# nikvaessen/w2v2-speaker

Measured on AMD Instinct MI355X. Metric: utterances/sec (w2v2-base + mean+std + AAM-softmax training step, 3 s clips), higher is better.
Workload: dtype f16; 1 GPU; wav2vec2-base + AAM-softmax(5994), mean+std pooling, 3 s synthetic audio, bs=66 per GPU, CNN frozen, fwd+bwd+all-reduce+Adam (BASELINE configs[1]); global_batch=66, samples_per_utt=48000, parallelism=dp1, regularisation=True

## Files before the change

### include/w2v2_hip.h

```cpp
#ifndef W2V2_HIP_H
#define W2V2_HIP_H

#include <stddef.h>
#include <stdint.h>

#ifdef __cplusplus
extern "C" {
#endif

#define W2V2_F32 0
#define W2V2_BF16 1
#define W2V2_F16 2

int w2v2_version(void);
const char* w2v2_last_error(void);

typedef struct {
  const void* ptr;
  int64_t ld;
  int64_t seg_len, seg_stride;
  int64_t stride0, stride1;
  int32_t trans;
  int32_t _pad;
} w2v2_operand;

enum {
  W2V2_EPI_NONE = 0,
  W2V2_EPI_BIAS = 1,
  W2V2_EPI_BIAS_GELU = 2,
  W2V2_EPI_GELU_BWD = 3,
  W2V2_EPI_ADD = 4,
  W2V2_EPI_SCALE_RC = 5,
  W2V2_EPI_BIAS_GELU_GRAD = 6,
  W2V2_EPI_MUL = 7
};

typedef struct {
  int32_t M, N, K;
  int32_t batch, batch_inner;
  int32_t dtype_ab;
  int32_t dtype_c;
  int32_t epilogue;
  w2v2_operand A, B;
  void* C;
  int64_t ldc, c_stride0, c_stride1;
  void* aux;
  int64_t ldaux, aux_stride0, aux_stride1;
  const float* bias;
  int64_t bias_stride1;
  const float* row_scale;
  const float* col_scale;
  float alpha;
  int32_t split_k;
  int32_t accumulate;
  int32_t _pad;
  int32_t k_ext, n_ext_from;
  int64_t b_lo_offset;
} w2v2_gemm_desc;

int w2v2_gemm(const w2v2_gemm_desc* d, void* stream);
int w2v2_gemm_timed(const w2v2_gemm_desc* d, void* stream, int slot);
int w2v2_timer_read(int first_slot, int n, float* ms_out);
int w2v2_gemm_kernel_of(const w2v2_gemm_desc* d);
int w2v2_tune_gemm_kernel(int family);
int w2v2_tune_gemm_debug(int bits);
int w2v2_tune_gemm_f32_tile(int tile);
int w2v2_tune_gemm_ring_debug(int bits);
int w2v2_gemm_f32_last_kernel(void);

typedef struct {
  const void* dY; int64_t ld_dy;
  const void* X;  int64_t ld_x;
  float* dW;      int64_t ld_dw;
  float* dbias;
  int32_t n_out, n_in;
} w2v2_wgrad_problem;
int w2v2_wgrad_grouped(const w2v2_wgrad_problem* problems, int n, int tokens, int tokens_padded,
                       int dtype , void* stream);
int w2v2_wgrad_kernel_of(const w2v2_wgrad_problem* problems, int n);
int w2v2_tune_wgrad_kernel(int family);

int w2v2_conv0_workspace_floats(int N, int C, int k, int stride);
int w2v2_conv0_stats(const float* wav, const float* w , float* partial, float* mean_rstd,
                     int B, int N, int C, int k, int stride, float eps, void* stream);
int w2v2_conv0_stats_mfma(const float* wav, const float* w, float* partial, float* mean_rstd,
                          int B, int N, int C, int k, int stride, float eps, void* stream);
int w2v2_conv0_stats_len(const float* wav, const float* w, float* partial, float* mean_rstd, const int* frames,
                         int B, int N, int C, int k, int stride, float eps, void* stream);
int w2v2_conv0_stats_mfma_len(const float* wav, const float* w, float* partial, float* mean_rstd, const int* frames,
                              int B, int N, int C, int k, int stride, float eps, void* stream);
int w2v2_conv0_apply(const float* wav, const float* w, const float* mean_rstd, const float* gamma,
                     const float* beta, void* y, int dtype, int B, int N, int C, int k, int stride,
                     void* stream);
int w2v2_conv0_layernorm_gelu(const float* wav, const float* w, const float* bias, const float* gamma, const float* beta,
                              void* out, int B, int N, int C, int k, int stride, float eps, int dtype, void* stream);
int w2v2_conv0_layernorm_gelu_bwd_workspace_floats(int B, int N, int C, int k, int stride);
int w2v2_conv0_layernorm_gelu_bwd(const float* wav, const float* w, const float* bias, const float* gamma, const float* beta,
                                  const void* dy, float* dw, float* dbias, float* dgamma, float* dbeta, float* workspace,
                                  int B, int N, int C, int k, int stride, float eps, int dtype, void* stream);
int w2v2_conv0_bwd(const float* wav, const float* w, const float* mean_rstd, const float* gamma,
                   const float* beta, const void* dz, float* sums, float* dw, float* dgamma, float* dbeta,
                   int dtype, int B, int N, int C, int k, int stride, void* stream);
int w2v2_col2im(const void* col, void* dx, int B, int Lin, int Lout, int Cin, int k, int stride, int dtype,
                void* stream);
int w2v2_unpack_conv_grad(const float* gp, float* g, int Cout, int Cin, int k, void* stream);
int w2v2_pack_conv_weight(const float* w, void* out, int dtype, int Cout, int Cin, int k, void* stream);

int w2v2_layernorm_fwd(const void* x, void* r_inout, const float* gamma, const float* beta, void* y,
                       float* mean, float* rstd, int M, int H, float eps, float drop_p,
                       uint64_t seed, int dtype, void* stream);
int w2v2_layernorm_gelu_fwd(const void* x, const float* gamma, const float* beta, void* y, int M, int H, float eps,
                            int dtype, void* stream);
int w2v2_layernorm_gelu_bwd_workspace_floats(int M, int H);
int w2v2_layernorm_gelu_bwd(const void* dy, const void* z, const float* gamma, const float* beta, void* dz, float* dgamma,
                            float* dbeta, float* dbias, float* workspace, int M, int H, float eps, int dtype, void* stream);
int w2v2_layernorm_bwd_workspace_floats(int H);
int w2v2_layernorm_bwd(const void* dy, const void* s, const float* mean, const float* rstd,
                       const float* gamma, void* ds, void* d_r, float* dgamma, float* dbeta,
                       float* workspace, int M, int H, float drop_p, uint64_t seed, int dtype,
                       void* stream);
typedef struct {
  const float* partial;
  float* dgamma;
  float* dbeta;
} w2v2_ln_fold;
int w2v2_layernorm_bwd_fold(const w2v2_ln_fold* entries, int n, int M, int H, void* stream);

int w2v2_dropout(const void* x, void* y, int64_t n, float p, uint64_t seed, int dtype, void* stream);
int w2v2_gelu_bwd(const void* dy, const void* pre, void* dx, int64_t n, int dtype, void* stream);
#define W2V2_PARTIAL_ROWS 256
int w2v2_gelu_bwd_colsum(const void* dy, const void* pre, void* dx, float* colsum, float* partial, int M, int N, int dtype,
                         void* stream);
int w2v2_add(const void* x, const void* a, void* y, int64_t n, int dtype, void* stream);
int w2v2_colsum(const void* x, int64_t ld, float* out, int M, int N, int dtype, void* stream);
int w2v2_zero_ranges(float* base, const int64_t* table, int n_ranges, int blocks_per_range, void* stream);
int w2v2_mean(const float* x, float* out, int n, void* stream);
int w2v2_cast(const float* x, void* y, int64_t n, int dtype, void* stream);
int w2v2_transpose_many(const void* src, void* dst, const int64_t* table, int n, int blocks_per_matrix,
                        int dtype, void* stream);
int w2v2_mask_fill(void* h, const uint8_t* mask, const float* embed, int M, int H, int dtype,
                   void* stream);
int w2v2_mask_feature(void* h, const uint8_t* mask, int B, int T, int H, int dtype, void* stream);
int w2v2_mask_fill_bwd(void* dh, const uint8_t* mask, float* d_embed, float* partial, int M, int H, int dtype,
                       void* stream);
int w2v2_prepend_token(const void* x, void* y, float c, int B, int T, int H, int dtype, void* stream);
int w2v2_pair_assemble(const void* feat, void* y, const int* left_row, const int* left_frames, const int* right_row,
                       const int* right_frames, float cls_c, float sep_c, int B, int T, int H, int dtype, void* stream);

int w2v2_posconv_regroup(const void* x, void* xg, int B, int T, int H, int G, int K, int pad_left,
                         int dtype, void* stream);
int w2v2_posconv_regroup_len(const void* x, void* xg, const int* lens, int B, int T, int H, int G, int K, int pad_left,
                             int dtype, void* stream);
int w2v2_posconv_wgrad(const void* dY, const void* xg, float* dwf, int B, int T, int H, int G, int K,
                       int dtype , void* stream);
int w2v2_posconv_direct(const void* xg, const void* w, void* out, void* aux, const float* bias, int B, int T, int G,
                        int Cg, int K, int64_t ldc, int mode, int dtype, void* stream);
int64_t w2v2_weightnorm_scratch_floats(int H, int G, int K);
int w2v2_weightnorm_pack(const float* g, const float* v, float* sumsq , void* wf,
                         void* wb, int H, int G, int K, int dtype, void* stream);
int w2v2_weightnorm_bwd(const float* g, const float* v, const float* sumsq, const float* dwf,
                        float* dot , float* dg, float* dv, int H, int G, int K,
                        void* stream);

int w2v2_softmax_fwd(const float* s, void* p, void* p_drop, int64_t rows, int T, int64_t ld,
                     float drop_p, uint64_t seed, int dtype, void* stream);
int w2v2_softmax_bwd(const float* dp_drop, const void* p, void* ds, int64_t rows, int T, int64_t ld,
                     float drop_p, uint64_t seed, int dtype, void* stream);
int w2v2_softmax_fwd_len(const float* s, void* p, const int* lens, int B, int heads, int T, int64_t ld, int dtype,
                         void* stream);
int w2v2_attention_fwd(const void* qkv, void* ctx, float* lse, int B, int T, int heads, int d,
                       float scale, float drop_p, uint64_t seed, int dtype, void* stream);
int w2v2_attention_bwd(const void* qkv, const void* ctx, const void* dctx, const float* lse,
                       void* dqkv, float* delta , int B, int T, int heads,
                       int d, float scale, float drop_p, uint64_t seed, int dtype, void* stream);
int w2v2_attention_fwd_len(const void* qkv, void* ctx, float* lse, const int* lens, int B, int T, int heads, int d,
                           float scale, int dtype, void* stream);

int w2v2_pool_fwd(const void* x, float* out, int B, int T, int H, int mode, int dtype, void* stream);
int w2v2_pool_fwd_len(const void* x, float* out, const int* lens, int B, int T, int H, int mode, int dtype,
                      void* stream);
int w2v2_pool_bwd(const void* x, const float* out, const float* dout, void* dx, int B, int T, int H,
                  int mode, int dtype, void* stream);

int w2v2_asp_context(const void* x, float* ctx, int B, int T, int C, int dtype, void* stream);
int w2v2_asp_context_len(const void* x, float* ctx, const int* lens, int B, int T, int C, int dtype, void* stream);
int w2v2_asp_context_bias(const float* ctx, const float* w1 , const float* b1, float* cb ,
                          int B, int A, int C, void* stream);
int w2v2_asp_bn_workspace_floats(int M, int A);
int w2v2_asp_bn_stats(const void* a_pre, float* workspace, float* mean_rstd, float* running, int M, int A,
                      float eps, float momentum, int dtype, void* stream);
int w2v2_asp_bn_eval_stats(const float* running, float* mean_rstd, int A, float eps, void* stream);
int w2v2_asp_bn_tanh(const void* a_pre, const float* mean_rstd, const float* gamma, const float* beta, void* h,
                     int M, int A, int dtype, void* stream);
int w2v2_asp_bn_bwd(const void* dh, const void* a_pre, const float* mean_rstd, const float* gamma,
                    const float* beta, float* workspace, float* dgamma, float* dbeta, void* da, int M, int A,
                    int dtype, void* stream);
int w2v2_asp_pool_fwd(const void* x, const void* s, float* out, float* stats, int B, int T, int C, int dtype,
                      void* stream);
int w2v2_asp_pool_fwd_len(const void* x, const void* s, float* out, float* stats, const int* lens, int B, int T, int C,
                          int dtype, void* stream);
int w2v2_asp_pool_bwd(const void* x, const void* s, const float* out, const float* stats, const float* dout,
                      void* ds, void* dx, int B, int T, int C, int dtype, void* stream);
int w2v2_asp_context_bwd(const void* x, const float* ctx, const void* da, const float* w1, float* dw1, void* dx,
                         float* scratch, int B, int T, int C, int A, int dtype, void* stream);

int w2v2_bce_head_fwd_bwd(const float* emb, const float* w, const float* b, const int64_t* label, float* prob,
                          float* loss_rows, float* dlogit, float* demb, float* dw, float* db, int B, int H,
                          const float* loss_scale, void* stream);

int w2v2_bn_workspace_floats(int M, int C);
int w2v2_bn_fwd(const void* a, int64_t lda, float* workspace, float* mean_rstd, float* running, const float* gamma,
                const float* beta, void* y, int64_t ldy, int M, int C, float eps, float momentum, int relu, int train,
                int dtype, void* stream);
int w2v2_bn_colsum_rows(int M, int C);
int w2v2_bn_bwd(const void* dy, int64_t lddy, const void* a, int64_t lda, const float* mean_rstd, const float* gamma,
                float* workspace, float* dgamma, float* dbeta, void* da, int64_t ldda, int M, int C, int relu,
                float* colsum_partial, int dtype, void* stream);
int w2v2_bn_bwd_sum(const void* dy, int64_t lddy, const void* dy2, int64_t lddy2, const void* a, int64_t lda,
                    const float* mean_rstd, const float* gamma, float* workspace, float* dgamma, float* dbeta, void* da,
                    int64_t ldda, int M, int C, int relu, float* colsum_partial, int dtype, void* stream);
int w2v2_im2col_reflect(const void* x, int64_t ldx, void* col, int B, int T, int Cin, int k, int dilation, int dtype,
                        void* stream);
int w2v2_im2col_reflect_sum(const void* x, int64_t ldx, const void* x2, int64_t ldx2, void* col, int B, int T, int Cin,
                            int k, int dilation, int dtype, void* stream);
int w2v2_im2col_reflect_len(const void* x, int64_t ldx, void* col, const int* lens, int B, int T, int Cin, int k,
                            int dilation, int dtype, void* stream);
int w2v2_im2col_reflect_sum_len(const void* x, int64_t ldx, const void* x2, int64_t ldx2, void* col, const int* lens,
                                int B, int T, int Cin, int k, int dilation, int dtype, void* stream);
int w2v2_col2im_reflect(const void* dcol, void* dx, int64_t lddx, int B, int T, int Cin, int k, int dilation,
                        int accumulate, int dtype, void* stream);
int w2v2_add_strided(const void* a, int64_t lda, const void* b, int64_t ldb, void* y, int64_t ldy, int M, int C,
                     int dtype, void* stream);
int w2v2_se_scale(const void* x, const float* g, void* y, int B, int T, int C, int dtype, void* stream);
int w2v2_se_bwd_gate(const void* dout, const void* x, float* dg, int B, int T, int C, int dtype, void* stream);
int w2v2_se_bwd_x(const void* dout, const float* g, const float* ds, void* dx, int B, int T, int C, int dtype,
                  void* stream);
int w2v2_act_fwd(const float* x, float* y, int64_t n, int mode, void* stream);
int w2v2_act_bwd(const float* dy, const float* y, float* dx, int64_t n, int mode, void* stream);

#define W2V2_FBANK_TILE_FRAMES 16
int w2v2_fbank_db(const float* wav, const int* lens, const float* window, const float* fbank, float* db_out,
                  float* partial_max, int B, int N, int T, int n_mels, void* stream);
int w2v2_fbank_normalize(const float* db, const float* partial_max, const int* lens, void* out, int64_t ldo, int dtype,
                         int B, int T, int n_mels, void* stream);

int w2v2_skinny_linear_fwd(const float* x, const float* W, const float* bias, float* y, int B, int N, int K, int act,
                           void* stream);
int w2v2_skinny_linear_bwd_x(const float* dy, const float* y, const float* W, float* dx, int B, int N, int K, int act,
                             void* stream);
int w2v2_skinny_linear_bwd_w(const float* dy, const float* y, const float* x, float* dW, float* dbias, int B, int N,
                             int K, int act, int accumulate, void* stream);

int w2v2_row_invnorm(const void* x, int64_t ld, float* inv, int rows, int cols, int dtype,
                     void* stream);
int w2v2_aam_softmax_fwd_bwd(const float* cos, const int64_t* label, float* softmax,
                             float* loss_rows, void* dcos_w, void* dcos_x, const float* inv_x,
                             const float* inv_w, float* rowdot, float* colprod, int B, int C,
                             int64_t ldc, float margin, float scale, const float* loss_scale,
                             float* correct_rows, int easy_margin , int dtype, void* stream);
int w2v2_normalize_bwd(const float* g, const void* x, int64_t ldx, const float* inv,
                       const float* dot, float* dx, int rows, int cols, int x_dtype, int add,
                       void* stream);
int w2v2_aam_dw(const void* dcos_x, int64_t ldc, const void* emb, const float* colprod, const float* W,
                const float* inv_w, float* dW, int B, int C, int E, int dtype, void* stream);

int w2v2_adam_step(float* p, const float* g, float* m, float* v, void* pb, int pb_dtype, int64_t n, float lr,
                   float beta1, float beta2, float eps, float bias_corr1, float bias_corr2,
                   float grad_scale, const float* scaler_state, int step, int skip_slot, void* stream);

#define W2V2_OPTIM_ADAM 0
#define W2V2_OPTIM_SGD 1
int w2v2_optim_step(int algo, float* p, const float* g, float* m, float* v, void* pb, int pb_dtype, int64_t n, float lr,
                    float beta1, float beta2, float eps, float bias_corr1, float bias_corr2, float grad_scale,
                    float weight_decay, float momentum, float dampening, int nesterov, const float* norm_state,
                    const float* scaler_state, int step, int skip_slot, void* stream);

int w2v2_grad_norm_partials(int64_t n);
int w2v2_grad_norm(const float* g, int64_t n, float grad_scale, float* scaler_state, float max_norm, double* partials,
                   int n_partials, float* norm_state, void* stream);

int w2v2_grad_accumulate(float* acc, const float* g, int64_t n, int first, void* stream);

int w2v2_weight_residual(const float* p, void* lo, const int64_t* table, int n_ranges, int dtype, void* stream);
int w2v2_grad_scaler_check(const float* g, int64_t n, float* state, void* stream);
int w2v2_grad_scaler_update(float* state, float growth, float backoff, int growth_interval, int skipped_ranges,
                            void* stream);

typedef struct w2v2_comm w2v2_comm;
int w2v2_comm_unique_id(void* id_host_128);
int w2v2_comm_init(w2v2_comm** comm, const void* id_host_128, int rank, int world, int device);
int w2v2_comm_init_loopback(w2v2_comm** comm, int world, int device);
int w2v2_allreduce_async(w2v2_comm* comm, float* buf, int64_t n, void* stream);
int w2v2_broadcast_async(w2v2_comm* comm, void* buf, int64_t nbytes, int root, void* stream);
int w2v2_comm_destroy(w2v2_comm* comm);
int w2v2_traffic_probe(float* buf, int64_t n, int channels, int lds_bytes, float gbps, void* stream);

#ifdef __cplusplus
}
#endif
#endif
```

### w2v2_speaker_amd/_lib.py

```python
from __future__ import annotations

import ctypes as C
import os

from . import _build

F32, BF16, F16 = 0, 1, 2
EPI_NONE, EPI_BIAS, EPI_BIAS_GELU, EPI_GELU_BWD, EPI_ADD, EPI_SCALE_RC, EPI_BIAS_GELU_GRAD, EPI_MUL = range(8)
OPTIM_ADAM, OPTIM_SGD = 0, 1

c_i32, c_i64, c_u64, c_f32, c_vp = C.c_int32, C.c_int64, C.c_uint64, C.c_float, C.c_void_p


class Operand(C.Structure):
    _fields_ = [("ptr", c_vp), ("ld", c_i64), ("seg_len", c_i64), ("seg_stride", c_i64),
                ("stride0", c_i64), ("stride1", c_i64), ("trans", c_i32), ("_pad", c_i32)]


class GemmDesc(C.Structure):
    _fields_ = [("M", c_i32), ("N", c_i32), ("K", c_i32), ("batch", c_i32), ("batch_inner", c_i32),
                ("dtype_ab", c_i32), ("dtype_c", c_i32), ("epilogue", c_i32),
                ("A", Operand), ("B", Operand),
                ("C", c_vp), ("ldc", c_i64), ("c_stride0", c_i64), ("c_stride1", c_i64),
                ("aux", c_vp), ("ldaux", c_i64), ("aux_stride0", c_i64), ("aux_stride1", c_i64),
                ("bias", c_vp), ("bias_stride1", c_i64), ("row_scale", c_vp), ("col_scale", c_vp),
                ("alpha", c_f32), ("split_k", c_i32), ("accumulate", c_i32), ("_pad", c_i32),
                ("k_ext", c_i32), ("n_ext_from", c_i32), ("b_lo_offset", c_i64)]


class LnFold(C.Structure):
    _fields_ = [("partial", c_vp), ("dgamma", c_vp), ("dbeta", c_vp)]


class WgradProblem(C.Structure):
    _fields_ = [("dY", c_vp), ("ld_dy", c_i64), ("X", c_vp), ("ld_x", c_i64), ("dW", c_vp), ("ld_dw", c_i64),
                ("dbias", c_vp), ("n_out", c_i32), ("n_in", c_i32)]


_SIGS = {
    "w2v2_version": (c_i32, []),
    "w2v2_last_error": (C.c_char_p, []),
    "w2v2_gemm": (c_i32, [C.POINTER(GemmDesc), c_vp]),
    "w2v2_gemm_kernel_of": (c_i32, [c_vp]),
    "w2v2_gemm_timed": (c_i32, [C.POINTER(GemmDesc), c_vp, c_i32]),
    "w2v2_timer_read": (c_i32, [c_i32, c_i32, c_vp]),
    "w2v2_tune_gemm_kernel": (c_i32, [c_i32]),
    "w2v2_tune_gemm_debug": (c_i32, [c_i32]),
    "w2v2_tune_gemm_f32_tile": (c_i32, [c_i32]),
    "w2v2_tune_gemm_ring_debug": (c_i32, [c_i32]),
    "w2v2_gemm_f32_last_kernel": (c_i32, []),
    "w2v2_zero_ranges": (c_i32, [c_vp, c_vp, c_i32, c_i32, c_vp]),
    "w2v2_mean": (c_i32, [c_vp, c_vp, c_i32, c_vp]),
    "w2v2_wgrad_grouped": (c_i32, [C.POINTER(WgradProblem), c_i32, c_i32, c_i32, c_i32, c_vp]),
    "w2v2_wgrad_kernel_of": (c_i32, [C.POINTER(WgradProblem), c_i32]),
    "w2v2_tune_wgrad_kernel": (c_i32, [c_i32]),
    "w2v2_conv0_workspace_floats": (c_i32, [c_i32, c_i32, c_i32, c_i32]),
    "w2v2_conv0_stats": (c_i32, [c_vp, c_vp, c_vp, c_vp, c_i32, c_i32, c_i32, c_i32, c_i32, c_f32, c_vp]),
    "w2v2_conv0_stats_mfma": (c_i32, [c_vp, c_vp, c_vp, c_vp, c_i32, c_i32, c_i32, c_i32, c_i32, c_f32, c_vp]),
    "w2v2_conv0_stats_len": (c_i32, [c_vp, c_vp, c_vp, c_vp, c_vp, c_i32, c_i32, c_i32, c_i32, c_i32, c_f32, c_vp]),
    "w2v2_conv0_stats_mfma_len": (c_i32, [c_vp, c_vp, c_vp, c_vp, c_vp, c_i32, c_i32, c_i32, c_i32, c_i32, c_f32,
                                          c_vp]),
    "w2v2_conv0_apply": (c_i32, [c_vp, c_vp, c_vp, c_vp, c_vp, c_vp, c_i32, c_i32, c_i32, c_i32, c_i32,
                                 c_i32, c_vp]),
    "w2v2_pack_conv_weight": (c_i32, [c_vp, c_vp, c_i32, c_i32, c_i32, c_i32, c_vp]),
    "w2v2_conv0_bwd": (c_i32, [c_vp] * 10 + [c_i32] * 6 + [c_vp]),
    "w2v2_col2im": (c_i32, [c_vp, c_vp, c_i32, c_i32, c_i32, c_i32, c_i32, c_i32, c_i32, c_vp]),
    "w2v2_unpack_conv_grad": (c_i32, [c_vp, c_vp, c_i32, c_i32, c_i32, c_vp]),
    "w2v2_conv0_layernorm_gelu": (c_i32, [c_vp, c_vp, c_vp, c_vp, c_vp, c_vp, c_i32, c_i32, c_i32, c_i32, c_i32, c_f32, c_i32, c_vp]),
    "w2v2_layernorm_gelu_fwd": (c_i32, [c_vp, c_vp, c_vp, c_vp, c_i32, c_i32, c_f32, c_i32, c_vp]),
    "w2v2_layernorm_gelu_bwd_workspace_floats": (c_i32, [c_i32, c_i32]),
    "w2v2_layernorm_gelu_bwd": (c_i32, [c_vp] * 9 + [c_i32, c_i32, c_f32, c_i32, c_vp]),
    "w2v2_conv0_layernorm_gelu_bwd_workspace_floats": (c_i32, [c_i32] * 5),
    "w2v2_conv0_layernorm_gelu_bwd": (c_i32, [c_vp] * 11 + [c_i32] * 5 + [c_f32, c_i32, c_vp]),
    "w2v2_layernorm_fwd": (c_i32, [c_vp, c_vp, c_vp, c_vp, c_vp, c_vp, c_vp, c_i32, c_i32, c_f32, c_f32,
                                   c_u64, c_i32, c_vp]),
    "w2v2_layernorm_bwd_workspace_floats": (c_i32, [c_i32]),
    "w2v2_layernorm_bwd": (c_i32, [c_vp, c_vp, c_vp, c_vp, c_vp, c_vp, c_vp, c_vp, c_vp, c_vp, c_i32, c_i32,
                                   c_f32, c_u64, c_i32, c_vp]),
    "w2v2_layernorm_bwd_fold": (c_i32, [C.POINTER(LnFold), c_i32, c_i32, c_i32, c_vp]),
    "w2v2_dropout": (c_i32, [c_vp, c_vp, c_i64, c_f32, c_u64, c_i32, c_vp]),
    "w2v2_gelu_bwd_colsum": (c_i32, [c_vp, c_vp, c_vp, c_vp, c_vp, c_i32, c_i32, c_i32, c_vp]),
    "w2v2_gelu_bwd": (c_i32, [c_vp, c_vp, c_vp, c_i64, c_i32, c_vp]),
    "w2v2_add": (c_i32, [c_vp, c_vp, c_vp, c_i64, c_i32, c_vp]),
    "w2v2_colsum": (c_i32, [c_vp, c_i64, c_vp, c_i32, c_i32, c_i32, c_vp]),
    "w2v2_cast": (c_i32, [c_vp, c_vp, c_i64, c_i32, c_vp]),
    "w2v2_transpose_many": (c_i32, [c_vp, c_vp, c_vp, c_i32, c_i32, c_i32, c_vp]),
    "w2v2_mask_feature": (c_i32, [c_vp, c_vp, c_i32, c_i32, c_i32, c_i32, c_vp]),
    "w2v2_mask_fill": (c_i32, [c_vp, c_vp, c_vp, c_i32, c_i32, c_i32, c_vp]),
    "w2v2_mask_fill_bwd": (c_i32, [c_vp, c_vp, c_vp, c_vp, c_i32, c_i32, c_i32, c_vp]),
    "w2v2_prepend_token": (c_i32, [c_vp, c_vp, c_f32, c_i32, c_i32, c_i32, c_i32, c_vp]),
    "w2v2_pair_assemble": (c_i32, [c_vp, c_vp, c_vp, c_vp, c_vp, c_vp, c_f32, c_f32, c_i32, c_i32, c_i32, c_i32, c_vp]),
    "w2v2_posconv_regroup": (c_i32, [c_vp, c_vp, c_i32, c_i32, c_i32, c_i32, c_i32, c_i32, c_i32, c_vp]),
    "w2v2_posconv_regroup_len": (c_i32, [c_vp, c_vp, c_vp, c_i32, c_i32, c_i32, c_i32, c_i32, c_i32, c_i32, c_vp]),
    "w2v2_posconv_direct": (c_i32, [c_vp, c_vp, c_vp, c_vp, c_vp, c_i32, c_i32, c_i32, c_i32, c_i32, c_i64, c_i32, c_i32, c_vp]),
    "w2v2_posconv_wgrad": (c_i32, [c_vp, c_vp, c_vp, c_i32, c_i32, c_i32, c_i32, c_i32, c_i32, c_vp]),
    "w2v2_weightnorm_scratch_floats": (c_i64, [c_i32, c_i32, c_i32]),
    "w2v2_weightnorm_pack": (c_i32, [c_vp, c_vp, c_vp, c_vp, c_vp, c_i32, c_i32, c_i32, c_i32, c_vp]),
    "w2v2_weightnorm_bwd": (c_i32, [c_vp, c_vp, c_vp, c_vp, c_vp, c_vp, c_vp, c_i32, c_i32, c_i32, c_vp]),
    "w2v2_softmax_fwd": (c_i32, [c_vp, c_vp, c_vp, c_i64, c_i32, c_i64, c_f32, c_u64, c_i32, c_vp]),
    "w2v2_softmax_bwd": (c_i32, [c_vp, c_vp, c_vp, c_i64, c_i32, c_i64, c_f32, c_u64, c_i32, c_vp]),
    "w2v2_softmax_fwd_len": (c_i32, [c_vp, c_vp, c_vp, c_i32, c_i32, c_i32, c_i64, c_i32, c_vp]),
    "w2v2_attention_fwd": (c_i32, [c_vp, c_vp, c_vp, c_i32, c_i32, c_i32, c_i32, c_f32, c_f32, c_u64,
                                   c_i32, c_vp]),
    "w2v2_attention_fwd_len": (c_i32, [c_vp, c_vp, c_vp, c_vp, c_i32, c_i32, c_i32, c_i32, c_f32, c_i32, c_vp]),
    "w2v2_attention_bwd": (c_i32, [c_vp, c_vp, c_vp, c_vp, c_vp, c_vp, c_i32, c_i32, c_i32, c_i32, c_f32,
                                   c_f32, c_u64, c_i32, c_vp]),
    "w2v2_pool_fwd": (c_i32, [c_vp, c_vp, c_i32, c_i32, c_i32, c_i32, c_i32, c_vp]),
    "w2v2_pool_fwd_len": (c_i32, [c_vp, c_vp, c_vp, c_i32, c_i32, c_i32, c_i32, c_i32, c_vp]),
    "w2v2_pool_bwd": (c_i32, [c_vp, c_vp, c_vp, c_vp, c_i32, c_i32, c_i32, c_i32, c_i32, c_vp]),
    "w2v2_bce_head_fwd_bwd": (c_i32, [c_vp] * 10 + [c_i32, c_i32, c_vp, c_vp]),
    "w2v2_bn_workspace_floats": (c_i32, [c_i32, c_i32]),
    "w2v2_bn_fwd": (c_i32, [c_vp, c_i64, c_vp, c_vp, c_vp, c_vp, c_vp, c_vp, c_i64, c_i32, c_i32, c_f32, c_f32, c_i32,
                            c_i32, c_i32, c_vp]),
    "w2v2_skinny_linear_fwd": (c_i32, [c_vp, c_vp, c_vp, c_vp, c_i32, c_i32, c_i32, c_i32, c_vp]),
    "w2v2_skinny_linear_bwd_x": (c_i32, [c_vp, c_vp, c_vp, c_vp, c_i32, c_i32, c_i32, c_i32, c_vp]),
    "w2v2_skinny_linear_bwd_w": (c_i32, [c_vp, c_vp, c_vp, c_vp, c_vp, c_i32, c_i32, c_i32, c_i32, c_i32, c_vp]),
    "w2v2_bn_bwd": (c_i32, [c_vp, c_i64, c_vp, c_i64, c_vp, c_vp, c_vp, c_vp, c_vp, c_vp, c_i64, c_i32, c_i32, c_i32,
                            c_vp, c_i32, c_vp]),
    "w2v2_bn_bwd_sum": (c_i32, [c_vp, c_i64, c_vp, c_i64, c_vp, c_i64, c_vp, c_vp, c_vp, c_vp, c_vp, c_vp, c_i64, c_i32,
                                c_i32, c_i32, c_vp, c_i32, c_vp]),
    "w2v2_bn_colsum_rows": (c_i32, [c_i32, c_i32]),
    "w2v2_im2col_reflect": (c_i32, [c_vp, c_i64, c_vp, c_i32, c_i32, c_i32, c_i32, c_i32, c_i32, c_vp]),
    "w2v2_im2col_reflect_sum": (c_i32, [c_vp, c_i64, c_vp, c_i64, c_vp, c_i32, c_i32, c_i32, c_i32, c_i32, c_i32, c_vp]),
    "w2v2_im2col_reflect_len": (c_i32, [c_vp, c_i64, c_vp, c_vp, c_i32, c_i32, c_i32, c_i32, c_i32, c_i32, c_vp]),
    "w2v2_im2col_reflect_sum_len": (c_i32, [c_vp, c_i64, c_vp, c_i64, c_vp, c_vp, c_i32, c_i32, c_i32, c_i32, c_i32, c_i32,
                                            c_vp]),
    "w2v2_col2im_reflect": (c_i32, [c_vp, c_vp, c_i64, c_i32, c_i32, c_i32, c_i32, c_i32, c_i32, c_i32, c_vp]),
    "w2v2_add_strided": (c_i32, [c_vp, c_i64, c_vp, c_i64, c_vp, c_i64, c_i32, c_i32, c_i32, c_vp]),
    "w2v2_se_scale": (c_i32, [c_vp, c_vp, c_vp, c_i32, c_i32, c_i32, c_i32, c_vp]),
    "w2v2_se_bwd_gate": (c_i32, [c_vp, c_vp, c_vp, c_i32, c_i32, c_i32, c_i32, c_vp]),
    "w2v2_se_bwd_x": (c_i32, [c_vp, c_vp, c_vp, c_vp, c_i32, c_i32, c_i32, c_i32, c_vp]),
    "w2v2_act_fwd": (c_i32, [c_vp, c_vp, c_i64, c_i32, c_vp]),
    "w2v2_act_bwd": (c_i32, [c_vp, c_vp, c_vp, c_i64, c_i32, c_vp]),
    "w2v2_fbank_db": (c_i32, [c_vp, c_vp, c_vp, c_vp, c_vp, c_vp, c_i32, c_i32, c_i32, c_i32, c_vp]),
    "w2v2_fbank_normalize": (c_i32, [c_vp, c_vp, c_vp, c_vp, c_i64, c_i32, c_i32, c_i32, c_i32, c_vp]),
    "w2v2_asp_context": (c_i32, [c_vp, c_vp, c_i32, c_i32, c_i32, c_i32, c_vp]),
    "w2v2_asp_context_len": (c_i32, [c_vp, c_vp, c_vp, c_i32, c_i32, c_i32, c_i32, c_vp]),
    "w2v2_asp_context_bias": (c_i32, [c_vp, c_vp, c_vp, c_vp, c_i32, c_i32, c_i32, c_vp]),
    "w2v2_asp_bn_workspace_floats": (c_i32, [c_i32, c_i32]),
    "w2v2_asp_bn_stats": (c_i32, [c_vp, c_vp, c_vp, c_vp, c_i32, c_i32, c_f32, c_f32, c_i32, c_vp]),
    "w2v2_asp_bn_eval_stats": (c_i32, [c_vp, c_vp, c_i32, c_f32, c_vp]),
    "w2v2_asp_bn_tanh": (c_i32, [c_vp, c_vp, c_vp, c_vp, c_vp, c_i32, c_i32, c_i32, c_vp]),
    "w2v2_asp_bn_bwd": (c_i32, [c_vp] * 9 + [c_i32, c_i32, c_i32, c_vp]),
    "w2v2_asp_pool_fwd": (c_i32, [c_vp, c_vp, c_vp, c_vp, c_i32, c_i32, c_i32, c_i32, c_vp]),
    "w2v2_asp_pool_fwd_len": (c_i32, [c_vp, c_vp, c_vp, c_vp, c_vp, c_i32, c_i32, c_i32, c_i32, c_vp]),
    "w2v2_asp_pool_bwd": (c_i32, [c_vp] * 7 + [c_i32, c_i32, c_i32, c_i32, c_vp]),
    "w2v2_asp_context_bwd": (c_i32, [c_vp] * 7 + [c_i32, c_i32, c_i32, c_i32, c_i32, c_vp]),
    "w2v2_row_invnorm": (c_i32, [c_vp, c_i64, c_vp, c_i32, c_i32, c_i32, c_vp]),
    "w2v2_aam_softmax_fwd_bwd": (c_i32, [c_vp, c_vp, c_vp, c_vp, c_vp, c_vp, c_vp, c_vp, c_vp, c_vp, c_i32,
                                         c_i32, c_i64, c_f32, c_f32, c_vp, c_vp, c_i32, c_i32, c_vp]),
    "w2v2_aam_dw": (c_i32, [c_vp, c_i64, c_vp, c_vp, c_vp, c_vp, c_vp, c_i32, c_i32, c_i32, c_i32, c_vp]),
    "w2v2_normalize_bwd": (c_i32, [c_vp, c_vp, c_i64, c_vp, c_vp, c_vp, c_i32, c_i32, c_i32, c_i32, c_vp]),
    "w2v2_adam_step": (c_i32, [c_vp, c_vp, c_vp, c_vp, c_vp, c_i32, c_i64, c_f32, c_f32, c_f32, c_f32, c_f32,
                               c_f32, c_f32, c_vp, c_i32, c_i32, c_vp]),
    "w2v2_optim_step": (c_i32, [c_i32, c_vp, c_vp, c_vp, c_vp, c_vp, c_i32, c_i64, c_f32, c_f32, c_f32, c_f32, c_f32,
                                c_f32, c_f32, c_f32, c_f32, c_f32, c_i32, c_vp, c_vp, c_i32, c_i32, c_vp]),
    "w2v2_grad_norm_partials": (c_i32, [c_i64]),
    "w2v2_grad_norm": (c_i32, [c_vp, c_i64, c_f32, c_vp, c_f32, c_vp, c_i32, c_vp, c_vp]),
    "w2v2_grad_accumulate": (c_i32, [c_vp, c_vp, c_i64, c_i32, c_vp]),
    "w2v2_weight_residual": (c_i32, [c_vp, c_vp, c_vp, c_i32, c_i32, c_vp]),
    "w2v2_comm_unique_id": (c_i32, [c_vp]),
    "w2v2_comm_init": (c_i32, [C.POINTER(c_vp), c_vp, c_i32, c_i32, c_i32]),
    "w2v2_comm_init_loopback": (c_i32, [C.POINTER(c_vp), c_i32, c_i32]),
    "w2v2_allreduce_async": (c_i32, [c_vp, c_vp, c_i64, c_vp]),
    "w2v2_broadcast_async": (c_i32, [c_vp, c_vp, c_i64, c_i32, c_vp]),
    "w2v2_comm_destroy": (c_i32, [c_vp]),
    "w2v2_traffic_probe": (c_i32, [c_vp, c_i64, c_i32, c_i32, c_f32, c_vp]),
    "w2v2_grad_scaler_check": (c_i32, [c_vp, c_i64, c_vp, c_vp]),
    "w2v2_grad_scaler_update": (c_i32, [c_vp, c_f32, c_f32, c_i32, c_i32, c_vp]),
}

EXPORTS = tuple(_SIGS)
_lib = None


def library_path() -> str:
    return _build.LIB


def load():
    global _lib
    if _lib is not None:
        return _lib
    path = _build.LIB
    alt = os.environ.get("W2V2_LIB_AB")
    if alt and os.path.exists(alt):
        path = alt
    elif _build.needs_build():
        try:
            _build.build_locked()
        except Exception as e:
            raise RuntimeError(f"libw2v2hip.so is missing or older than its sources and could not be built: {e}") from e
    lib = C.CDLL(path)
    for name, (res, args) in _SIGS.items():
        if path == alt and not hasattr(lib, name):
            continue
        fn = getattr(lib, name)
        fn.restype, fn.argtypes = res, args
    _lib = lib
    return lib


def check(rc: int, what: str = "") -> None:
    if rc != 0:
        msg = load().w2v2_last_error()
        raise RuntimeError(f"libw2v2hip {what} failed: {msg.decode() if msg else rc}")
```

### w2v2_speaker_amd/csrc/attention.hip

```cpp
#include "common.h"
#include <stdlib.h>
#include <type_traits>

typedef __attribute__((ext_vector_type(4))) float f32x4;

constexpr int HD = 64;

__device__ __forceinline__ uint64_t attn_drop_idx(int64_t bh, int q, int key, int Tn) {
  return (uint64_t)(bh * Tn + q) * (uint64_t)((Tn + 1) & ~1) + (uint64_t)key;
}
__device__ __forceinline__ uint64_t attn_row_pair0(int64_t bh, int q, int Tn) {
  return (uint64_t)(bh * Tn + q) * (uint64_t)(((Tn + 1) & ~1) >> 1);
}
__device__ __forceinline__ uint32_t rng_pair_i(uint32_t key, uint64_t pair_idx) { return rng_pair(key, pair_idx); }
__device__ __forceinline__ uint32_t rng_pair_i(uint32_t key, uint32_t pair_idx) {
  uint32_t x = pair_idx ^ key;
  x ^= x >> 16; x *= 0x85EBCA6Bu;
  x ^= x >> 13; x *= 0xC2B2AE35u;
  x ^= x >> 16;
  return x;
}
template <typename IDX>
__device__ __forceinline__ void attn_drop4_keys(uint32_t k, uint32_t thr, IDX row0, int key0_rel, float inv_keep,
                                                float (&ms)[4]) {
  const IDX pi = row0 + (IDX)(uint32_t)(key0_rel >> 1);
  const uint32_t h0 = rng_pair_i(k, pi), h1 = rng_pair_i(k, (IDX)(pi + 1));
  ms[0] = (h0 & 0xffffu) >= thr ? inv_keep : 0.f;
  ms[1] = (h0 >> 16) >= thr ? inv_keep : 0.f;
  ms[2] = (h1 & 0xffffu) >= thr ? inv_keep : 0.f;
  ms[3] = (h1 >> 16) >= thr ? inv_keep : 0.f;
}
template <typename IDX>
__device__ __forceinline__ void attn_drop4_rows(uint32_t k, uint32_t thr, IDX col0, uint32_t Tp2, int q0, int odd,
                                                float inv_keep, float (&ms)[4]) {
  const uint32_t qa = (uint32_t)(q0 + 2 * odd);
  const uint32_t h0 = rng_pair_i(k, (IDX)(col0 + (IDX)__umul24(qa, Tp2)));
  const uint32_t h1 = rng_pair_i(k, (IDX)(col0 + (IDX)__umul24(qa + 1u, Tp2)));
  const uint32_t p0 = __shfl_xor(h0, 1, 64), p1 = __shfl_xor(h1, 1, 64);
  const uint32_t r0 = odd ? p0 : h0, r1 = odd ? p1 : h1, r2 = odd ? h0 : p0, r3 = odd ? h1 : p1;
  const int sh = odd * 16;
  ms[0] = ((r0 >> sh) & 0xffffu) >= thr ? inv_keep : 0.f;
  ms[1] = ((r1 >> sh) & 0xffffu) >= thr ? inv_keep : 0.f;
  ms[2] = ((r2 >> sh) & 0xffffu) >= thr ? inv_keep : 0.f;
  ms[3] = ((r3 >> sh) & 0xffffu) >= thr ? inv_keep : 0.f;
}
__device__ __forceinline__ int aswz(int row) { return ((row ^ (row >> 1)) & 3) | (row & 4); }

__device__ __forceinline__ frag8_t as_frag(uint4 v) {
  union { uint4 u; frag8_t f; } c;
  c.u = v;
  return c.f;
}
template <typename TE>
__device__ __forceinline__ frag8_t pack_frag(const float a[4], const float b[4]) {
  uint4 v;
  v.x = pack2<TE>(a[0], a[1]);
  v.y = pack2<TE>(a[2], a[3]);
  v.z = pack2<TE>(b[0], b[1]);
  v.w = pack2<TE>(b[2], b[3]);
  return as_frag(v);
}
template <typename TE>
__device__ __forceinline__ float frag_dot(frag8_t a, frag8_t b) {
  union { frag8_t f; uint32_t w[4]; } ua, ub;
  ua.f = a;
  ub.f = b;
  float s = 0.f;
#pragma unroll
  for (int i = 0; i < 4; ++i) {
    float a0, a1, b0, b1;
    unpack2<TE>(ua.w[i], a0, a1);
    unpack2<TE>(ub.w[i], b0, b1);
    s = fmaf(a0, b0, s);
    s = fmaf(a1, b1, s);
  }
  return s;
}

__device__ __forceinline__ frag8_t lds_frag(const bf16_t* lds, int row0, int kk, int lane) {
  const int fr = lane & 15;
  const int lane_off = fr * 64 + (((kk * 4 + (lane >> 4)) ^ aswz(fr)) << 3);
  return as_frag(*reinterpret_cast<const uint4*>(lds + lane_off + row0 * 64));
}
__device__ __forceinline__ void reg_frag(frag8_t f[2], const bf16_t* g, int64_t gs, int row, int n_valid, int lane) {
#pragma unroll
  for (int kk = 0; kk < 2; ++kk) {
    uint4 v = make_uint4(0, 0, 0, 0);
    if (row < n_valid) v = *reinterpret_cast<const uint4*>(g + (int64_t)row * gs + kk * 32 + (lane >> 4) * 8);
    f[kk] = as_frag(v);
  }
}
__device__ __forceinline__ float quad_max(float v) {
  const uint32_t u = __float_as_uint(v);
  auto a = __builtin_amdgcn_permlane16_swap(u, u, false, false);
  v = fmaxf(__uint_as_float(a[0]), __uint_as_float(a[1]));
  const uint32_t w = __float_as_uint(v);
  auto b = __builtin_amdgcn_permlane32_swap(w, w, false, false);
  return fmaxf(__uint_as_float(b[0]), __uint_as_float(b[1]));
}
__device__ __forceinline__ float quad_sum(float v) {
  const uint32_t u = __float_as_uint(v);
  auto a = __builtin_amdgcn_permlane16_swap(u, u, false, false);
  v = __uint_as_float(a[0]) + __uint_as_float(a[1]);
  const uint32_t w = __float_as_uint(v);
  auto b = __builtin_amdgcn_permlane32_swap(w, w, false, false);
  return __uint_as_float(b[0]) + __uint_as_float(b[1]);
}

template <typename TE>
__device__ __forceinline__ void store_row4x4(bf16_t* row, int g, bool valid, const f32x4 (&o)[4]) {
  const bool odd = (g & 1) != 0;
#pragma unroll
  for (int p = 0; p < 2; ++p) {
    const uint32_t ax = pack2<TE>(o[2 * p][0], o[2 * p][1]), ay = pack2<TE>(o[2 * p][2], o[2 * p][3]);
    const uint32_t bx = pack2<TE>(o[2 * p + 1][0], o[2 * p + 1][1]), by = pack2<TE>(o[2 * p + 1][2], o[2 * p + 1][3]);
    const auto sx = __builtin_amdgcn_permlane16_swap(ax, bx, false, false);
    const auto sy = __builtin_amdgcn_permlane16_swap(ay, by, false, false);
    const uint4 w = make_uint4(sx[0], sy[0], sx[1], sy[1]);
    if (valid) store16_wt(row + (2 * p + (odd ? 1 : 0)) * 16 + (g & 2) * 4, w);
  }
}

typedef __attribute__((ext_vector_type(4))) short short4v_t;
typedef __attribute__((address_space(3))) short4v_t lds_s4v_t;

struct TrOff { int o[4]; };
__device__ __forceinline__ TrOff tr_offsets(int lane) {
  const int i = lane & 15, g = lane >> 4;
  const int r = g * 4 + (i >> 2);
  const int sw = aswz(r);
  TrOff t;
#pragma unroll
  for (int df = 0; df < 4; ++df) t.o[df] = r * 64 + (((2 * df + ((i & 3) >> 1)) ^ sw) << 3) + ((i & 1) << 2);
  return t;
}
__device__ __forceinline__ frag8_t lds_frag_tr(const bf16_t* img, const TrOff& t, int df, int blk) {
  const bf16_t* p0 = img + t.o[df] + blk * 2048;
  const short4v_t lo = __builtin_amdgcn_ds_read_tr16_b64_v4i16((lds_s4v_t*)p0);
  const short4v_t hi = __builtin_amdgcn_ds_read_tr16_b64_v4i16((lds_s4v_t*)(p0 + 1024));
  union { struct { short4v_t a, b; } s; frag8_t v; } u;
  u.s.a = lo;
  u.s.b = hi;
  return u.v;
}

struct TileRegs { uint4 v[2]; };
template <int NT>
__device__ __forceinline__ void tile_load(TileRegs& r, const bf16_t* g, int64_t gs, int row0, int n_valid) {
#pragma unroll
  for (int i = 0; i < 2; ++i) {
    const int c = threadIdx.x + NT * i;
    const int row = row0 + (c >> 3), ch = c & 7;
    r.v[i] = make_uint4(0, 0, 0, 0);
    if (row < n_valid) r.v[i] = *reinterpret_cast<const uint4*>(g + (int64_t)row * gs + ch * 8);
  }
}
template <int NT>
__device__ __forceinline__ void tile_store(const TileRegs& r, bf16_t* lds) {
#pragma unroll
  for (int i = 0; i < 2; ++i) {
    const int c = threadIdx.x + NT * i;
    const int row = c >> 3, ch = c & 7;
    *reinterpret_cast<uint4*>(lds + row * 64 + ((ch ^ aswz(row)) << 3)) = r.v[i];
  }
}

typedef __attribute__((address_space(1))) const void attn_gvoid_t;
typedef __attribute__((address_space(3))) void attn_lvoid_t;
template <int NW, int KT>
__device__ __forceinline__ void tile_dma(const bf16_t* g, int64_t gs, int row0, int n_valid, bf16_t* lds, int wave, int lane) {
#pragma unroll
  for (int i = 0; i < KT / (8 * NW); ++i) {
    const int piece = wave * (KT / (8 * NW)) + i;
    const int row = piece * 8 + (lane >> 3);
    const int src_row = min(row0 + row, n_valid - 1);
    const int ch = (lane & 7) ^ aswz(row);
    __builtin_amdgcn_global_load_lds((attn_gvoid_t*)(g + (int64_t)src_row * gs + ch * 8), (attn_lvoid_t*)(lds + piece * 8 * 64), 16, 0, 0);
  }
}

struct AttnBlock { int tile, h, b; };
__device__ __forceinline__ AttnBlock attn_block(int ntile_rows, int heads) {
  const int nwg = gridDim.x, bid = blockIdx.x;
  const int q = nwg >> 3, r = nwg & 7, xcd = bid & 7, loc = bid >> 3;
  int logical = (xcd < r ? xcd * (q + 1) : r * (q + 1) + (xcd - r) * q) + loc;
  if (heads < 0) { logical = bid; heads = -heads; }
  AttnBlock o;
  o.tile = logical % ntile_rows;
  const int bh = logical / ntile_rows;
  o.h = bh % heads;
  o.b = bh / heads;
  return o;
}

template <typename TE, int NW, int KT, typename IDX, bool LEN>
__global__ __launch_bounds__(64 * NW, 4) void attn_fwd_tiled_kernel(const bf16_t* __restrict__ qkv, bf16_t* __restrict__ ctx,
                                                             float* __restrict__ lse, int Tn, int heads_s, float scale,
                                                             float dp, float inv_keep, uint64_t seed,
                                                             LensArg<LEN> lens) {
  static_assert(KT * 8 == 2 * 64 * NW, "a tile is staged as two 16-byte chunks per thread");
  constexpr int NT = 64 * NW, RW = 16 * NW, AT_TILE = KT;
  __shared__ __attribute__((aligned(16))) bf16_t Ks[2][AT_TILE * 64];
  __shared__ __attribute__((aligned(16))) bf16_t Vs[2][AT_TILE * 64];
  const AttnBlock blk = attn_block((Tn + RW - 1) / RW, heads_s);
  const int heads = heads_s < 0 ? -heads_s : heads_s;
  const int b = blk.b, h = blk.h, row_tile = blk.tile;
  const int H = heads * HD;
  const int64_t gs = 3 * (int64_t)H;
  const bf16_t* qb = qkv + (int64_t)b * Tn * gs + h * HD;
  const int lane = threadIdx.x & 63, wave = threadIdx.x >> 6, g = lane >> 4;
  const int q = row_tile * RW + wave * 16 + (lane & 15);
  const int64_t bh = (int64_t)b * heads + h;
  int Lv = Tn;
  if constexpr (LEN) {
    Lv = lens[b];
    if (row_tile * RW >= Lv) {
      const f32x4 z[4] = {};
      store_row4x4<TE>(ctx + ((int64_t)b * Tn + q) * H + h * HD, g, q < Tn, z);
      return;
    }
  }
  frag8_t qf[2];
  reg_frag(qf, qb, gs, q, Lv, lane);
  const TrOff troff = tr_offsets(lane);
  const int ntile = (Lv + AT_TILE - 1) / AT_TILE;
  TileRegs rk, rv;
  tile_load<NT>(rk, qb + H, gs, 0, Lv);
  tile_load<NT>(rv, qb + 2 * H, gs, 0, Lv);
  tile_store<NT>(rk, Ks[0]);
  tile_store<NT>(rv, Vs[0]);
  __syncthreads();
  float m = -INFINITY, l = 0.f;
  const float scale2 = scale * 1.4426950408889634f;
  const uint32_t thr = drop_thr16(dp);
  const uint32_t rkey = rng_key(seed);
  const IDX row0 = (IDX)(attn_row_pair0(bh, q, Tn) + (uint64_t)(g * 2));
  f32x4 o[4];
#pragma unroll
  for (int df = 0; df < 4; ++df) o[df] = f32x4{0.f, 0.f, 0.f, 0.f};
  const bool active = row_tile * RW + wave * 16 < Lv;
#pragma unroll 1
  for (int t = 0; t < ntile; ++t) {
    const int cur = t & 1;
    if (t + 1 < ntile) {
      tile_load<NT>(rk, qb + H, gs, (t + 1) * AT_TILE, Lv);
      tile_load<NT>(rv, qb + 2 * H, gs, (t + 1) * AT_TILE, Lv);
    }
    const int nfj = min(AT_TILE / 16, (Lv - t * AT_TILE + 15) >> 4);
    if (active) {
      auto body = [&](auto full_c, auto drop_c) {
        constexpr bool FULL = decltype(full_c)::value, DROP = decltype(drop_c)::value;
        float s[AT_TILE / 16][4];
        float tmax = -INFINITY;
#pragma unroll
        for (int fj = 0; fj < AT_TILE / 16; ++fj) {
          if (FULL || fj < nfj) {
            f32x4 acc = mfma16<TE>(lds_frag(Ks[cur], fj * 16, 0, lane), qf[0], f32x4{0.f, 0.f, 0.f, 0.f});
            acc = mfma16<TE>(lds_frag(Ks[cur], fj * 16, 1, lane), qf[1], acc);
#pragma unroll
            for (int j = 0; j < 4; ++j) {
              float v = acc[j] * scale2;
              if constexpr (!FULL) v = (t * AT_TILE + fj * 16 + g * 4 + j < Lv) ? v : -INFINITY;
              s[fj][j] = v;
              tmax = fmaxf(tmax, v);
            }
          }
        }
        tmax = quad_max(tmax);
        const float mn = fmaxf(m, tmax);
        const float alpha = __builtin_amdgcn_exp2f(m - mn);
        m = mn;
        float psum = 0.f;
#pragma unroll
        for (int fj = 0; fj < AT_TILE / 16; ++fj) {
          if (FULL || fj < nfj) {
            float ms[4];
            if constexpr (DROP) attn_drop4_keys(rkey, thr, row0, t * AT_TILE + fj * 16, inv_keep, ms);
#pragma unroll
            for (int j = 0; j < 4; ++j) {
              const float p = __builtin_amdgcn_exp2f(s[fj][j] - mn);
              psum += p;
              s[fj][j] = DROP ? p * ms[j] : p;
            }
          } else {
#pragma unroll
            for (int j = 0; j < 4; ++j) s[fj][j] = 0.f;
          }
        }
        l = l * alpha + quad_sum(psum);
#pragma unroll
        for (int df = 0; df < 4; ++df) o[df] *= alpha;
#pragma unroll
        for (int kb = 0; kb < AT_TILE / 32; ++kb) {
          if (FULL || 2 * kb < nfj) {
            const frag8_t pf = pack_frag<TE>(s[2 * kb], s[2 * kb + 1]);
#pragma unroll
            for (int df = 0; df < 4; ++df) o[df] = mfma16<TE>(lds_frag_tr(Vs[cur], troff, df, kb), pf, o[df]);
          }
        }
      };
      const bool full = (t + 1) * AT_TILE <= Lv;
      if (!LEN && dp > 0.f) {
        if (full) body(std::true_type{}, std::true_type{}); else body(std::false_type{}, std::true_type{});
      } else {
        if (full) body(std::true_type{}, std::false_type{}); else body(std::false_type{}, std::false_type{});
      }
    }
    if (t + 1 < ntile) {
      tile_store<NT>(rk, Ks[cur ^ 1]);
      tile_store<NT>(rv, Vs[cur ^ 1]);
    }
    __syncthreads();
  }
  if constexpr (LEN) {
    const float inv = 1.0f / l;
#pragma unroll
    for (int df = 0; df < 4; ++df) o[df] = q < Lv ? o[df] * inv : f32x4{0.f, 0.f, 0.f, 0.f};
  } else {
    const float inv = q < Tn ? 1.0f / l : 0.f;
#pragma unroll
    for (int df = 0; df < 4; ++df) o[df] *= inv;
  }
  store_row4x4<TE>(ctx + ((int64_t)b * Tn + q) * H + h * HD, g, q < Tn, o);
  if (q < Lv && g == 0) lse[bh * Tn + q] = m * 0.6931471805599453f + __logf(l);
}

template <typename TE, int NW, int KT, typename IDX>
__global__ __launch_bounds__(64 * NW, 4) void attn_bwd_dq_tiled_kernel(const bf16_t* __restrict__ qkv,
                                                                const bf16_t* __restrict__ ctx,
                                                                const bf16_t* __restrict__ dctx,
                                                                const float* __restrict__ lse,
                                                                bf16_t* __restrict__ dqkv, float* __restrict__ delta,
                                                                int Tn, int heads_s, float scale, float dp,
                                                                float inv_keep, uint64_t seed) {
  static_assert(KT * 8 == 2 * 64 * NW, "a tile is staged as two 16-byte chunks per thread");
  constexpr int NT = 64 * NW, RW = 16 * NW, AT_TILE = KT;
  __shared__ __attribute__((aligned(16))) bf16_t Ks[2][AT_TILE * 64];
  __shared__ __attribute__((aligned(16))) bf16_t Vs[2][AT_TILE * 64];
  const AttnBlock blk = attn_block((Tn + RW - 1) / RW, heads_s);
  const int heads = heads_s < 0 ? -heads_s : heads_s;
  const int b = blk.b, h = blk.h, row_tile = blk.tile;
  const int H = heads * HD;
  const int64_t gs = 3 * (int64_t)H;
  const bf16_t* qb = qkv + (int64_t)b * Tn * gs + h * HD;
  const bf16_t* dob = dctx + (int64_t)b * Tn * H + h * HD;
  const bf16_t* ob = ctx + (int64_t)b * Tn * H + h * HD;
  const int lane = threadIdx.x & 63, wave = threadIdx.x >> 6, g = lane >> 4;
  const int q = row_tile * RW + wave * 16 + (lane & 15);
  const int64_t bh = (int64_t)b * heads + h;
  frag8_t qf[2], dof[2], of[2];
  reg_frag(qf, qb, gs, q, Tn, lane);
  reg_frag(dof, dob, H, q, Tn, lane);
  reg_frag(of, ob, H, q, Tn, lane);
  float dl = 0.f;
#pragma unroll
  for (int kk = 0; kk < 2; ++kk) dl += frag_dot<TE>(dof[kk], of[kk]);
  dl = quad_sum(dl);
  if (g == 0 && q < Tn) delta[bh * Tn + q] = dl;
  const uint32_t thr = drop_thr16(dp);
  const uint32_t rkey = rng_key(seed);
  const IDX row0 = (IDX)(attn_row_pair0(bh, q, Tn) + (uint64_t)(g * 2));
  const float l2 = q < Tn ? lse[bh * Tn + q] * 1.4426950408889634f : 0.f;
  const float scale2 = scale * 1.4426950408889634f;
  const TrOff troff = tr_offsets(lane);
  const int ntile = (Tn + AT_TILE - 1) / AT_TILE;
  TileRegs rk, rv;
  tile_load<NT>(rk, qb + H, gs, 0, Tn);
  tile_load<NT>(rv, qb + 2 * H, gs, 0, Tn);
  tile_store<NT>(rk, Ks[0]);
  tile_store<NT>(rv, Vs[0]);
  __syncthreads();
  f32x4 o[4];
#pragma unroll
  for (int df = 0; df < 4; ++df) o[df] = f32x4{0.f, 0.f, 0.f, 0.f};
  const bool active = row_tile * RW + wave * 16 < Tn;
#pragma unroll 1
  for (int t = 0; t < ntile; ++t) {
    const int cur = t & 1;
    if (t + 1 < ntile) {
      tile_load<NT>(rk, qb + H, gs, (t + 1) * AT_TILE, Tn);
      tile_load<NT>(rv, qb + 2 * H, gs, (t + 1) * AT_TILE, Tn);
    }
    const int nfj = min(AT_TILE / 16, (Tn - t * AT_TILE + 15) >> 4);
    if (active)
#pragma unroll
    for (int kb = 0; kb < AT_TILE / 32; ++kb) {
      if (2 * kb < nfj) {
      float ds2[2][4];
#pragma unroll
      for (int hf = 0; hf < 2; ++hf) {
        const int fj = 2 * kb + hf;
        if (fj < nfj) {
          f32x4 sa = {0.f, 0.f, 0.f, 0.f}, pa = {0.f, 0.f, 0.f, 0.f};
#pragma unroll
          for (int kk = 0; kk < 2; ++kk) {
            sa = mfma16<TE>(lds_frag(Ks[cur], fj * 16, kk, lane), qf[kk], sa);
            pa = mfma16<TE>(lds_frag(Vs[cur], fj * 16, kk, lane), dof[kk], pa);
          }
          const int key0 = t * AT_TILE + fj * 16 + g * 4;
          float ms[4] = {1.f, 1.f, 1.f, 1.f};
          if (dp > 0.f) attn_drop4_keys(rkey, thr, row0, t * AT_TILE + fj * 16, inv_keep, ms);
          if ((t + 1) * AT_TILE > Tn) {
#pragma unroll
            for (int j = 0; j < 4; ++j) {
              const float p = key0 + j < Tn ? __builtin_amdgcn_exp2f(fmaf(sa[j], scale2, -l2)) : 0.f;
              ds2[hf][j] = p * (pa[j] * ms[j] - dl) * scale;
            }
          } else {
#pragma unroll
            for (int j = 0; j < 4; ++j) {
              const float p = __builtin_amdgcn_exp2f(fmaf(sa[j], scale2, -l2));
              ds2[hf][j] = p * (pa[j] * ms[j] - dl) * scale;
            }
          }
        } else {
#pragma unroll
          for (int j = 0; j < 4; ++j) ds2[hf][j] = 0.f;
        }
      }
      const frag8_t pf = pack_frag<TE>(ds2[0], ds2[1]);
#pragma unroll
      for (int df = 0; df < 4; ++df) o[df] = mfma16<TE>(lds_frag_tr(Ks[cur], troff, df, kb), pf, o[df]);
      }
    }
    if (t + 1 < ntile) {
      tile_store<NT>(rk, Ks[cur ^ 1]);
      tile_store<NT>(rv, Vs[cur ^ 1]);
    }
    __syncthreads();
  }
  store_row4x4<TE>(dqkv + ((int64_t)b * Tn + q) * gs + h * HD, g, q < Tn, o);
}

template <typename TE, int NW, int KT, typename IDX, bool DMA>
__global__ __launch_bounds__(64 * NW, DMA ? 4 : 3) void attn_bwd_kv_tiled_kernel(const bf16_t* __restrict__ qkv,
                                                                const bf16_t* __restrict__ dctx,
                                                                const float* __restrict__ lse,
                                                                const float* __restrict__ delta,
                                                                bf16_t* __restrict__ dqkv, int Tn, int heads_s,
                                                                float scale, float dp, float inv_keep, uint64_t seed) {
  static_assert(KT * 8 == 2 * 64 * NW, "a tile is staged as two 16-byte chunks per thread");
  constexpr int NT = 64 * NW, RW = 16 * NW, AT_TILE = KT;
  __shared__ __attribute__((aligned(16))) bf16_t Qs[2][AT_TILE * 64];
  __shared__ __attribute__((aligned(16))) bf16_t Os[2][AT_TILE * 64];
  __shared__ __attribute__((aligned(16))) float lse_s[2][AT_TILE];
  __shared__ __attribute__((aligned(16))) float del_s[2][AT_TILE];
  const AttnBlock blk = attn_block((Tn + RW - 1) / RW, heads_s);
  const int heads = heads_s < 0 ? -heads_s : heads_s;
  const int b = blk.b, h = blk.h, row_tile = blk.tile;
  const int H = heads * HD;
  const int64_t gs = 3 * (int64_t)H;
  const bf16_t* qb = qkv + (int64_t)b * Tn * gs + h * HD;
  const bf16_t* dob = dctx + (int64_t)b * Tn * H + h * HD;
  const int lane = threadIdx.x & 63, wave = threadIdx.x >> 6, g = lane >> 4;
  const int key = row_tile * RW + wave * 16 + (lane & 15);
  const int64_t bh = (int64_t)b * heads + h;
  frag8_t kf[2], vf[2];
  reg_frag(kf, qb + H, gs, key, Tn, lane);
  reg_frag(vf, qb + 2 * H, gs, key, Tn, lane);
  const TrOff troff = tr_offsets(lane);
  const int ntile = (Tn + AT_TILE - 1) / AT_TILE;
  TileRegs rq, ro;
  float rl = 0.f, rd = 0.f;
  auto row_load = [&](int t) {
    if (threadIdx.x < AT_TILE) {
      const int r = t * AT_TILE + threadIdx.x;
      rl = r < Tn ? lse[bh * Tn + r] * 1.4426950408889634f : (DMA ? INFINITY : 0.f);
      rd = r < Tn ? delta[bh * Tn + r] : 0.f;
    }
  };
  auto row_store = [&](int buf) {
    if (threadIdx.x < AT_TILE) { lse_s[buf][threadIdx.x] = rl; del_s[buf][threadIdx.x] = rd; }
  };
  if constexpr (DMA) {
    tile_dma<NW, KT>(qb, gs, 0, Tn, Qs[0], wave, lane);
    tile_dma<NW, KT>(dob, H, 0, Tn, Os[0], wave, lane);
    row_load(0);
    row_store(0);
    asm volatile("s_waitcnt vmcnt(0)" ::: "memory");
  } else {
    tile_load<NT>(rq, qb, gs, 0, Tn);
    tile_load<NT>(ro, dob, H, 0, Tn);
    row_load(0);
    tile_store<NT>(rq, Qs[0]);
    tile_store<NT>(ro, Os[0]);
    row_store(0);
  }
  __syncthreads();
  f32x4 dv[4], dk[4];
#pragma unroll
  for (int df = 0; df < 4; ++df) { dv[df] = f32x4{0.f, 0.f, 0.f, 0.f}; dk[df] = f32x4{0.f, 0.f, 0.f, 0.f}; }
  const bool active = row_tile * RW + wave * 16 < Tn;
  const uint32_t rkey = rng_key(seed), thr = drop_thr16(dp);
  const IDX col0 = (IDX)(attn_drop_idx(bh, 0, key, Tn) >> 1);
  const uint32_t Tp2 = (uint32_t)(((Tn + 1) & ~1) >> 1);
  const float scale2 = scale * 1.4426950408889634f;
#pragma unroll 1
  for (int t = 0; t < ntile; ++t) {
    const int cur = t & 1;
    if (t + 1 < ntile) {
      if constexpr (DMA) {
        tile_dma<NW, KT>(qb, gs, (t + 1) * AT_TILE, Tn, Qs[cur ^ 1], wave, lane);
        tile_dma<NW, KT>(dob, H, (t + 1) * AT_TILE, Tn, Os[cur ^ 1], wave, lane);
      } else {
        tile_load<NT>(rq, qb, gs, (t + 1) * AT_TILE, Tn);
        tile_load<NT>(ro, dob, H, (t + 1) * AT_TILE, Tn);
      }
      row_load(t + 1);
    }
    const int nfq = min(AT_TILE / 16, (Tn - t * AT_TILE + 15) >> 4);
    if (active)
#pragma unroll
    for (int qb2 = 0; qb2 < AT_TILE / 32; ++qb2) {
      if (2 * qb2 < nfq) {
      float pt2[2][4], ds2[2][4];
#pragma unroll
      for (int hf = 0; hf < 2; ++hf) {
        const int fq = 2 * qb2 + hf;
        if (fq < nfq) {
          f32x4 sa = {0.f, 0.f, 0.f, 0.f}, pa = {0.f, 0.f, 0.f, 0.f};
#pragma unroll
          for (int kk = 0; kk < 2; ++kk) {
            sa = mfma16<TE>(lds_frag(Qs[cur], fq * 16, kk, lane), kf[kk], sa);
            pa = mfma16<TE>(lds_frag(Os[cur], fq * 16, kk, lane), vf[kk], pa);
          }
          const float4 l4 = *reinterpret_cast<const float4*>(&lse_s[cur][fq * 16 + g * 4]);
          const float4 d4 = *reinterpret_cast<const float4*>(&del_s[cur][fq * 16 + g * 4]);
          const float la[4] = {l4.x, l4.y, l4.z, l4.w}, da[4] = {d4.x, d4.y, d4.z, d4.w};
          const int q0 = t * AT_TILE + fq * 16 + g * 4;
          float ms[4] = {1.f, 1.f, 1.f, 1.f};
          if (dp > 0.f) attn_drop4_rows(rkey, thr, col0, Tp2, q0, key & 1, inv_keep, ms);
#pragma unroll
          for (int j = 0; j < 4; ++j) {
            const float p = key < Tn ? __builtin_amdgcn_exp2f(fmaf(sa[j], scale2, -la[j])) : 0.f;
            pt2[hf][j] = p * ms[j];
            ds2[hf][j] = p * (pa[j] * ms[j] - da[j]) * scale;
          }
        } else {
#pragma unroll
          for (int j = 0; j < 4; ++j) { pt2[hf][j] = 0.f; ds2[hf][j] = 0.f; }
        }
      }
      const frag8_t pf = pack_frag<TE>(pt2[0], pt2[1]);
      const frag8_t sf = pack_frag<TE>(ds2[0], ds2[1]);
#pragma unroll
      for (int df = 0; df < 4; ++df) {
        dv[df] = mfma16<TE>(lds_frag_tr(Os[cur], troff, df, qb2), pf, dv[df]);
        dk[df] = mfma16<TE>(lds_frag_tr(Qs[cur], troff, df, qb2), sf, dk[df]);
      }
      }
    }
    if (t + 1 < ntile) {
      if constexpr (!DMA) {
        tile_store<NT>(rq, Qs[cur ^ 1]);
        tile_store<NT>(ro, Os[cur ^ 1]);
      }
      row_store(cur ^ 1);
      if constexpr (DMA) asm volatile("s_waitcnt vmcnt(0)" ::: "memory");
    }
    __syncthreads();
  }
  bf16_t* dstk = dqkv + ((int64_t)b * Tn + key) * gs + H + h * HD;
  store_row4x4<TE>(dstk, g, key < Tn, dk);
  store_row4x4<TE>(dstk + H, g, key < Tn, dv);
}

static int attn_check(const char* nm, int B, int T, int heads, int d, int dtype, float drop_p) {
  W2V2_REQUIRE(B > 0 && T > 0 && heads > 0, "%s: bad shape", nm);
  W2V2_REQUIRE(d == HD, "%s: fused attention needs head dim 64 (got %d); use the unfused path", nm, d);
  W2V2_REQUIRE(dtype == W2V2_BF16 || dtype == W2V2_F16,
               "%s: fused attention needs 16-bit activations; the f32 parity mode uses the unfused path", nm);
  W2V2_REQUIRE(drop_p >= 0.f && drop_p < 1.f, "%s: bad dropout p", nm);
  return 0;
}

static const bool g_attn_no_remap = getenv("W2V2_ATTN_NO_XCD_REMAP") != nullptr;
static int attn_geom_env() { const char* e = getenv("W2V2_ATTN_GEOM"); return e ? atoi(e) : 0; }
constexpr int ATTN_SMALL_GEOM_MAX_T = 512;
static bool attn_small_geom(int T) {
  const int g = attn_geom_env();
  return g == 32 || (g != 64 && T <= ATTN_SMALL_GEOM_MAX_T && ((T + 31) & ~31) < ((T + 63) & ~63));
}

static bool attn_idx32(int B, int T, int heads) {
  if (getenv("W2V2_ATTN_IDX64")) return false;
  return (uint64_t)B * heads * T * (uint64_t)(((T + 1) & ~1) >> 1) < (1ull << 32);
}

template <typename TE, int NW, int KT, typename IDX>
static int attention_fwd_g(const char* name, const void* qkv, void* ctx, float* lse, const int* lens, int B, int T,
                           int heads, float scale, float drop_p, uint64_t seed, void* stream) {
  const float ik = 1.0f / (1.0f - drop_p);
  hipStream_t st = as_stream(stream);
  dim3 grid((unsigned)(cdiv(T, 16 * NW) * heads * B));
  W2V2_DISPATCH_LEN(lens,
    hipLaunchKernelGGL((attn_fwd_tiled_kernel<TE, NW, KT, IDX, LEN>), grid, dim3(64 * NW), 0, st, (const bf16_t*)qkv,
                       (bf16_t*)ctx, lse, T, g_attn_no_remap ? -heads : heads, scale, drop_p, ik, seed, lens));
  W2V2_CHECK_LAUNCH(name);
  return 0;
}
template <typename TE>
static int attention_fwd_t(const char* name, const void* qkv, void* ctx, float* lse, const int* lens, int B, int T,
                           int heads, float scale, float drop_p, uint64_t seed, void* stream) {
  const bool i32 = attn_idx32(B, T, heads);
  if (attn_small_geom(T))
    return i32 ? attention_fwd_g<TE, 2, 32, uint32_t>(name, qkv, ctx, lse, lens, B, T, heads, scale, drop_p, seed, stream)
               : attention_fwd_g<TE, 2, 32, uint64_t>(name, qkv, ctx, lse, lens, B, T, heads, scale, drop_p, seed, stream);
  return i32 ? attention_fwd_g<TE, 4, 64, uint32_t>(name, qkv, ctx, lse, lens, B, T, heads, scale, drop_p, seed, stream)
             : attention_fwd_g<TE, 4, 64, uint64_t>(name, qkv, ctx, lse, lens, B, T, heads, scale, drop_p, seed, stream);
}

extern "C" int w2v2_attention_fwd(const void* qkv, void* ctx, float* lse, int B, int T, int heads, int d, float scale,
                                  float drop_p, uint64_t seed, int dtype, void* stream) {
  if (attn_check("attention_fwd", B, T, heads, d, dtype, drop_p)) return -1;
  W2V2_REQUIRE(qkv && ctx && lse, "attention_fwd: null pointer");
  W2V2_DISPATCH_16(dtype, "attention_fwd",
                   return attention_fwd_t<AT>("attention_fwd", qkv, ctx, lse, nullptr, B, T, heads, scale, drop_p, seed,
                                              stream););
  return 0;
}

extern "C" int w2v2_attention_fwd_len(const void* qkv, void* ctx, float* lse, const int* lens, int B, int T, int heads,
                                      int d, float scale, int dtype, void* stream) {
  if (attn_check("attention_fwd_len", B, T, heads, d, dtype, 0.f)) return -1;
  W2V2_REQUIRE(qkv && ctx && lse && lens, "attention_fwd_len: null pointer");
  W2V2_DISPATCH_16(dtype, "attention_fwd_len",
                   return attention_fwd_t<AT>("attention_fwd_len", qkv, ctx, lse, lens, B, T, heads, scale, 0.f, 0,
                                              stream););
  return 0;
}

template <typename TE, int NW, int KT, typename IDX>
static int attention_bwd_g(const void* qkv, const void* ctx, const void* dctx, const float* lse, void* dqkv,
                           float* delta, int B, int T, int heads, float scale, float drop_p, uint64_t seed,
                           void* stream) {
  const float ik = 1.0f / (1.0f - drop_p);
  hipStream_t st = as_stream(stream);
  dim3 grid((unsigned)(cdiv(T, 16 * NW) * heads * B));
  hipLaunchKernelGGL((attn_bwd_dq_tiled_kernel<TE, NW, KT, IDX>), grid, dim3(64 * NW), 0, st, (const bf16_t*)qkv, (const bf16_t*)ctx,
                     (const bf16_t*)dctx, lse, (bf16_t*)dqkv, delta, T, g_attn_no_remap ? -heads : heads, scale, drop_p, ik,
                     seed);
  if (NW == 2 && getenv("W2V2_ATTN_KV_NO_DMA") == nullptr)
    hipLaunchKernelGGL((attn_bwd_kv_tiled_kernel<TE, NW, KT, IDX, NW == 2>), grid, dim3(64 * NW), 0, st, (const bf16_t*)qkv,
                       (const bf16_t*)dctx, lse, (const float*)delta, (bf16_t*)dqkv, T, g_attn_no_remap ? -heads : heads, scale,
                       drop_p, ik, seed);
  else
    hipLaunchKernelGGL((attn_bwd_kv_tiled_kernel<TE, NW, KT, IDX, false>), grid, dim3(64 * NW), 0, st, (const bf16_t*)qkv,
                       (const bf16_t*)dctx, lse, (const float*)delta, (bf16_t*)dqkv, T, g_attn_no_remap ? -heads : heads, scale,
                       drop_p, ik, seed);
  W2V2_CHECK_LAUNCH("attention_bwd");
  return 0;
}
template <typename TE>
static int attention_bwd_t(const void* qkv, const void* ctx, const void* dctx, const float* lse, void* dqkv,
                           float* delta, int B, int T, int heads, float scale, float drop_p, uint64_t seed,
                           void* stream) {
  const bool i32 = attn_idx32(B, T, heads);
  if (attn_small_geom(T))
    return i32 ? attention_bwd_g<TE, 2, 32, uint32_t>(qkv, ctx, dctx, lse, dqkv, delta, B, T, heads, scale, drop_p, seed, stream)
               : attention_bwd_g<TE, 2, 32, uint64_t>(qkv, ctx, dctx, lse, dqkv, delta, B, T, heads, scale, drop_p, seed, stream);
  return i32 ? attention_bwd_g<TE, 4, 64, uint32_t>(qkv, ctx, dctx, lse, dqkv, delta, B, T, heads, scale, drop_p, seed, stream)
             : attention_bwd_g<TE, 4, 64, uint64_t>(qkv, ctx, dctx, lse, dqkv, delta, B, T, heads, scale, drop_p, seed, stream);
}

extern "C" int w2v2_attention_bwd(const void* qkv, const void* ctx, const void* dctx, const float* lse, void* dqkv,
                                  float* delta, int B, int T, int heads, int d, float scale, float drop_p,
                                  uint64_t seed, int dtype, void* stream) {
  if (attn_check("attention_bwd", B, T, heads, d, dtype, drop_p)) return -1;
  W2V2_REQUIRE(qkv && ctx && dctx && lse && dqkv && delta, "attention_bwd: null pointer");
  W2V2_DISPATCH_16(dtype, "attention_bwd",
                   return attention_bwd_t<AT>(qkv, ctx, dctx, lse, dqkv, delta, B, T, heads, scale, drop_p, seed, stream););
  return 0;
}
```

### w2v2_speaker_amd/engine.py

```python
from __future__ import annotations

import math
import os
from dataclasses import dataclass
from typing import Callable, Dict, List, Optional, Sequence

import torch

from . import ops
from .config import W2V2Config, Wav2Vec2RegularisationConfig
from .ops import (EPI_ADD, EPI_BIAS, EPI_BIAS_GELU, EPI_BIAS_GELU_GRAD, EPI_GELU_BWD, EPI_MUL, EPI_NONE, EPI_SCALE_RC, Gemm,
                  POOL_MODES,
                  WgradGroup)
from .params import W2V_PREFIX, ParamStore

_SITE = {"featproj": 1, "prologue": 2, "attn": 3, "post_attn": 4, "ffn": 5, "act": 6}


def _splitk(m_tiles: int, n_tiles: int, k: int, batch: int = 1) -> int:
    blocks = max(1, m_tiles * n_tiles * batch)
    s = max(1, min(16, 512 // blocks))
    while s > 1 and k // s < 256:
        s -= 1
    return s


def _tiles(n: int, t: int = 128) -> int:
    return (n + t - 1) // t


def _pad64(n: int) -> int:
    return (n + 63) // 64 * 64


def _wb(name: str):
    return name + ".weight", name + ".bias"


@dataclass(frozen=True)
class PlanSwitches:
    wgrad_group: int = 0
    no_wgrad_pairs: bool = False
    no_ln_fold: bool = False
    no_posconv_direct: bool = False
    pos_dw_gemm: bool = False

    @classmethod
    def from_env(cls) -> "PlanSwitches":
        env = os.environ.get
        group = env("W2V2_WGRAD_GROUP")
        return cls(max(1, min(4, int(group))) if group else 0, bool(env("W2V2_NO_WGRAD_PAIRS")),
                   bool(env("W2V2_NO_LN_FOLD")), bool(env("W2V2_NO_POSCONV_DIRECT")), bool(env("W2V2_POS_DW_GEMM")))


def encoder_backward_schedule(num_layers: int, skip: Sequence[int], pair_uppers: Sequence[int], grouped: bool = True,
                              group: int = 2):
    if grouped and group > 2:
        ev, held, skip, pending_top = [], [], set(skip), num_layers - 1

        def flush(down_to):
            nonlocal held, pending_top
            if held:
                ev.extend([("wgrad", tuple(held)), ("fold",)])
            ev.extend(("notify", h) for h in range(pending_top, down_to - 1, -1))
            held, pending_top = [], down_to - 1
        for l in reversed(range(num_layers)):
            if l in skip:
                if not held:
                    flush(l)
                continue
            ev.append(("body", l))
            held.append(l)
            ev.append(("dx", l))
            if len(held) == group:
                flush(l)
        flush(0)
        return ev
    ev, held, Ltop, skip, pair_uppers = [], None, num_layers - 1, set(skip), set(pair_uppers)
    for l in reversed(range(num_layers)):
        upper = grouped and (Ltop - l) % 2 == 0 and l > 0 and l in pair_uppers
        if l in skip:
            if held is not None:
                ev += [("wgrad", (held,)), ("fold",), ("notify", held)]
                held = None
            ev.append(("notify", l))
            continue
        ev.append(("body", l))
        if grouped:
            if held is not None:
                ev.append(("wgrad", (held, l)))
            elif not upper:
                ev.append(("wgrad", (l,)))
        ev.append(("dx", l))
        if grouped and held is None and upper:
            held = l
            continue
        ev.append(("fold",))
        if held is not None:
            ev.append(("notify", held))
            held = None
        ev.append(("notify", l))
    assert held is None
    return ev


def valid_lengths(cfg: W2V2Config, lengths, batch: int, n_samples: int) -> List[int]:
    if isinstance(lengths, torch.Tensor):
        if lengths.is_cuda or lengths.is_floating_point() or lengths.is_complex():
            raise ValueError("lengths must be Python ints or a CPU integer tensor")
        lengths = lengths.reshape(-1).tolist()
    lens = [int(n) for n in lengths]
    if len(lens) != batch:
        raise ValueError(f"lengths: {len(lens)} values for a batch of {batch}")
    for n in lens:
        if n > n_samples:
            raise ValueError(f"lengths: {n} samples is longer than the plan's {n_samples}")
        if min(cfg.conv_lengths(n)) < 1:
            raise ValueError(f"lengths: {n} samples is too short for one encoder frame")
    return lens


@dataclass
class LayerBufs:
    qkv: torch.Tensor
    ctx: torch.Tensor
    a: torch.Tensor
    x1: torch.Tensor
    hpre: torch.Tensor
    h: torch.Tensor
    f: torch.Tensor
    mean1: torch.Tensor
    rstd1: torch.Tensor
    mean2: torch.Tensor
    rstd2: torch.Tensor
    lse: Optional[torch.Tensor] = None
    p: Optional[torch.Tensor] = None
    pd: Optional[torch.Tensor] = None


class Plan:
    def __init__(self, store: ParamStore, batch: int, n_samples: int, *, train: bool,
                 reg: Optional[Wav2Vec2RegularisationConfig] = None, pooling: str = "mean+std",
                 insert_cls_token: bool = False, cls_token_constant: float = 1.0,
                 aam_margin: float = 0.2, aam_scale: float = 30.0, fused_attention: Optional[bool] = None,
                 seed: int = 7, keep_hidden_states: bool = False, paired: bool = False,
                 sep_token_constant: float = -1.0, encoder_frames: Optional[int] = None):
        cfg = store.cfg
        self.store, self.cfg, self.B, self.N, self.train = store, cfg, batch, n_samples, train
        self.paired, self.sep_c = paired, sep_token_constant
        self.Bc = 2 * batch if paired else batch
        assert not (paired and insert_cls_token)
        self.reg = reg if reg is not None else Wav2Vec2RegularisationConfig()
        pooling = pooling.lower() if pooling.lower() == "none" else pooling
        self.pooling, self.pool_mode = pooling, POOL_MODES.get(pooling, -1)
        assert pooling in ("attentive", "random", "none") or pooling in POOL_MODES, pooling
        self.no_pool = pooling == "none"
        self._rand_idx = 0
        self.cls, self.cls_c = insert_cls_token, cls_token_constant
        self.margin, self.scale = aam_margin, aam_scale
        self.seed = seed
        self.all_x = train or keep_hidden_states
        self.dev, self.adt = store.device, store.act_dtype
        self.enc_only = encoder_frames is not None
        if self.enc_only and (not paired or train or n_samples != 0 or encoder_frames < 5):
            raise ValueError("encoder_frames: an evaluation plan with paired=True, n_samples=0 and at least 5 frames "
                             "([CLS] l [SEP] r [SEP]); build it with Plan.pair_encoder")
        self.lens = [0] * len(cfg.conv_dim) if self.enc_only else cfg.conv_lengths(n_samples)
        self.T0 = self.lens[-1]
        if self.enc_only:
            self.T = int(encoder_frames)
        else:
            self.T = 2 * self.T0 + 3 if paired else self.T0 + (1 if insert_cls_token else 0)
        self.M0, self.M = self.Bc * self.T0, batch * self.T
        H, d = cfg.hidden_size, cfg.head_dim
        if fused_attention is None:
            fused_attention = ops.is16(self.adt) and d == 64
        self.fused = fused_attention
        self.stable = bool(cfg.do_stable_layer_norm)
        self.ln_conv = cfg.feat_extract_norm == "layer"
        if cfg.feat_extract_norm not in ("group", "layer"):
            raise ValueError(f"feat_extract_norm must be 'group' or 'layer', got {cfg.feat_extract_norm!r}")
        if not self.ln_conv and cfg.conv_bias and train and not store.freeze_cnn:
            raise NotImplementedError("feat_extract_norm='group' with conv_bias=True (no published checkpoint has it) has a "
                                      "forward path only: train it with the feature extractor frozen "
                                      "(completely_freeze_feature_extractor: true, the reference's default)")
        if self.stable and (insert_cls_token or paired or keep_hidden_states):
            raise NotImplementedError("do_stable_layer_norm: the CLS-token, paired-input and hidden-state-ensemble paths are "
                                      "built for the post-LN encoder only")
        self.embed_dim = H * (2 if pooling == "attentive" else ops.POOL_WIDTH.get(self.pool_mode, 1))
        self._pack_version = -1
        self._cnn_version = -1
        self._asp = {}
        self.sw = PlanSwitches.from_env()
        self.grouped = train and store.flat_lp_t is not None
        self.wg_group = self._wgrad_group_size() if train else 2
        self.g_wgrad_pair, self._wgrad_cache = {}, {}
        self.head, self.fc, self._lnfold = None, None, None
        self._len_dev, self._len = None, None
        self.frame_lengths: Optional[List[int]] = None
        self._pair_dev = None
        self._alloc()
        self._build_gemms()

    @classmethod
    def pair_encoder(cls, store: ParamStore, batch: int, frames: int, **kw) -> "Plan":
        return cls(store, batch, 0, train=False, pooling="first", paired=True, encoder_frames=frames, **kw)

    def _wgrad_group_size(self) -> int:
        if self.sw.wgrad_group:
            return self.sw.wgrad_group
        cfg = self.cfg
        H, I = cfg.hidden_size, cfg.intermediate_size
        c = lambda n: -(-n // 256)
        tiles = c(H) * c(I) * 2 + c(H) * c(H) + c(3 * H) * c(H)
        ncu = torch.cuda.get_device_properties(self.dev).multi_processor_count if self.dev.type == "cuda" else 256
        cost = {k: -(-k * tiles // ncu) / k for k in (2, 4)}
        return 4 if (cfg.num_hidden_layers >= 4 and cost[4] < cost[2] - 1e-9) else 2

    def _wgrad_for(self, layers):
        if len(layers) == 1:
            return self.g_layer[layers[0]]["wgrad"]
        if len(layers) == 2 and layers[0] in self.g_wgrad_pair and layers[1] == layers[0] - 1:
            return self.g_wgrad_pair[layers[0]]
        if layers not in self._wgrad_cache:
            if len(self._wgrad_cache) >= 256:
                self._wgrad_cache.clear()
            probs = []
            for l in layers:
                probs += self.g_layer[l]["wgrad_problems"]
            self._wgrad_cache[layers] = WgradGroup(probs, self.M, _pad64(self.M))
        return self._wgrad_cache[layers]

    def _x(self, l: int) -> torch.Tensor:
        return self.X[l if self.all_x else l % 2]

    def _e(self, *shape, dtype=None) -> torch.Tensor:
        return torch.empty(*shape, dtype=dtype or self.adt, device=self.dev)

    def _ep(self, rows: int, cols: int, pad_rows: int = 0) -> torch.Tensor:
        rp = max(_pad64(rows), pad_rows)
        full = torch.zeros(rp, cols, dtype=self.adt, device=self.dev)
        v = full[:rows]
        v._w2v2_padded = full
        return v

    def _alloc(self) -> None:
        cfg, B, T, M, H, I = self.cfg, self.B, self.T, self.M, self.cfg.hidden_size, self.cfg.intermediate_size
        f32 = torch.float32
        C = cfg.conv_dim
        Bc = self.Bc
        if self.enc_only:
            self.cnn_train = False
            self.hx = self._e(M, H)
            self._alloc_encoder()
            return
        self.stats0 = ops.conv0_workspace(Bc, self.N, C[0], cfg.conv_kernel[0], cfg.conv_stride[0], self.dev)
        self.conv = [self._e(Bc, L, c) for L, c in zip(self.lens, C)]
        cins = (1,) + tuple(C[:-1])
        self.convw = [None] + [self._e(C[i], cfg.conv_kernel[i] * cins[i]) for i in range(1, len(C))]
        self.zero_bias = torch.zeros(max(max(C), H), dtype=f32, device=self.dev)
        self.cnn_train = self.train and not self.store.freeze_cnn
        if self.cnn_train:
            self.conv_pre = [None] + [self._e(Bc, L, c) for L, c in zip(self.lens[1:], C[1:])]
            self.dconv = [self._e(Bc, L, c) for L, c in zip(self.lens[:-1], C[:-1])]
            self.col = self._e(max(Bc * self.lens[i] * cfg.conv_kernel[i] * cins[i] for i in range(1, len(C))))
            self.dwp = torch.zeros(max(C[i] * cfg.conv_kernel[i] * cins[i] for i in range(1, len(C))), dtype=f32,
                                   device=self.dev)
            self.sums0 = self._e(Bc, C[0], 2, dtype=f32)
            if self.ln_conv:
                self.lng_ws = self._e(max(ops.lib().w2v2_layernorm_gelu_bwd_workspace_floats(Bc * L, c)
                                          for L, c in zip(self.lens[1:], C[1:])), dtype=f32)
                self.c0l_ws = ops.conv0_layernorm_gelu_bwd_workspace(Bc, self.N, C[0], cfg.conv_kernel[0],
                                                                     cfg.conv_stride[0], self.dev)
        self.proj_slices = 8
        self.proj_slice_len = -(-self.M0 // (self.proj_slices * 64)) * 64
        proj_pad = self.proj_slices * self.proj_slice_len
        self.ln_feat = self._ep(self.M0, C[-1], proj_pad)
        self.mean_f, self.rstd_f = self._e(self.M0, dtype=f32), self._e(self.M0, dtype=f32)
        self.h0 = self._e(self.M0, H)
        self.hx = self._e(M, H) if (self.cls or self.paired) else self.h0
        self._alloc_encoder(proj_pad)

    def _alloc_encoder(self, proj_pad: int = 0) -> None:
        cfg, B, T, M, H, I = self.cfg, self.B, self.T, self.M, self.cfg.hidden_size, self.cfg.intermediate_size
        f32 = torch.float32
        C = cfg.conv_dim
        G, K = cfg.num_conv_pos_embedding_groups, cfg.num_conv_pos_embeddings
        self.Cg, self.Tp = H // G, T + K - 1
        self.pos_direct = (ops.is16(self.adt) and self.Cg in (48, 64) and K == 128 and not self.sw.no_posconv_direct)
        self.xg = self._e(B, G, self.Tp, self.Cg)
        self.posw_f, self.posw_b = self._e(G, self.Cg, K * self.Cg), self._e(G, self.Cg, K * self.Cg)
        self.pos_sumsq = ops.weightnorm_scratch(H, G, K, self.dev)
        self.pos = self._e(M, H)
        self.pos_pre = self._e(M, H) if self.train else None
        self.mean0, self.rstd0 = self._e(M, dtype=f32), self._e(M, dtype=f32)
        L = cfg.num_hidden_layers
        nset = L if self.train else 1
        self.X = [self._ep(M, H) for _ in range(L + 1 if self.all_x else 2)]
        heads = cfg.num_attention_heads
        self.Tl = (T + 7) // 8 * 8
        self.lb: List[LayerBufs] = []
        for _ in range(nset):
            lb = LayerBufs(qkv=self._e(M, 3 * H), ctx=self._ep(M, H), a=self._e(M, H), x1=self._ep(M, H),
                           hpre=self._e(M, I) if self.train else None, h=self._ep(M, I), f=self._e(M, H),
                           mean1=self._e(M, dtype=f32), rstd1=self._e(M, dtype=f32),
                           mean2=self._e(M, dtype=f32), rstd2=self._e(M, dtype=f32))
            if self.fused:
                lb.lse = self._e(B * heads * T, dtype=f32)
            else:
                lb.p = torch.zeros(B * heads * T, self.Tl, dtype=self.adt, device=self.dev)
                lb.pd = (torch.zeros(B * heads * T, self.Tl, dtype=self.adt, device=self.dev)
                         if (self.train and self.reg.attention_dropout > 0) else lb.p)
            self.lb.append(lb)
        if not self.fused:
            self.S = torch.zeros(B * heads * T, self.Tl, dtype=f32, device=self.dev)
        E = self.embed_dim
        self.head_rows = B * T if self.no_pool else B
        self.emb = self._e(self.head_rows, E, dtype=f32)
        st = self.store
        if st.head == "bce":
            from .heads import BceHead
            self.head = BceHead(self.head_rows, E, w=st.p("linear.weight"), b=st.p("linear.bias"),
                                w_grad=st.g("linear.weight") if self.train else None,
                                b_grad=st.g("linear.bias") if self.train else None, emb=self.emb, train=self.train,
                                loss_scale=st.scaler)
        elif st.head is not None:
            from .heads import ClassifierHead, FcStack
            aam = st.head == "aam"
            nh = len(st.hidden_fc)
            self.fc = FcStack(st, self.head_rows, E, st.hidden_fc, self.emb, self.train) if nh else None
            head_in = self.fc.x[-1] if self.fc is not None else self.emb
            wname = "loss_fn.fc_weights" if aam else f"fc_list.{nh}.0.weight"
            bname = f"fc_list.{nh}.0.bias"
            self.head = ClassifierHead(st.head, self.head_rows, st.head_in_dim, st.num_speakers, w_master=st.p(wname),
                                       w_operand=st.w(wname), w_grad=st.g(wname) if self.train else None,
                                       bias=None if aam else st.p(bname),
                                       bias_grad=None if (aam or not self.train) else st.g(bname),
                                       emb=head_in, act_dtype=self.adt, train=self.train, margin=self.margin,
                                       scale=self.scale, loss_scale=st.scaler)
        if self.train:
            self.demb = (self.head.demb if (self.head is not None and self.fc is None)
                         else self._e(self.head_rows, E, dtype=f32))
            self.G = self._ep(M, H, 0 if (self.cls or self.paired) else proj_pad)
            self._gsets = [dict(Gd=self._ep(M, H), Gd1=self._ep(M, H), DH=self._ep(M, I), DQKV=self._ep(M, 3 * H))
                           for _ in range(cfg.num_hidden_layers if self.wg_group > 2 else 2)]
            self.DC = self._e(M, H)
            self.P1 = self._e(M, H)
            self.GR = self._e(M, H) if self.stable else None
            self.dyg = self._e(B, G, self.Tp, self.Cg)
            self.dwf = self._e(G, K * self.Cg, self.Cg, dtype=f32)
            self.pos_dot = ops.weightnorm_scratch(H, G, K, self.dev)
            self.dn = self._e(self.M0, C[-1])
            self.G0 = self._ep(self.M0, H, proj_pad) if (self.cls or self.paired) else None
            if self.fused:
                self.delta = self._e(B * heads * T, dtype=f32)
            else:
                self.dS = torch.zeros(B * heads * T, self.Tl, dtype=self.adt, device=self.dev)
            self._lnfold = ops.LnFoldGroup(H, self.dev)

    def _build_gemms(self) -> None:
        cfg, st, B, T, M, H, I = self.cfg, self.store, self.B, self.T, self.M, self.cfg.hidden_size, self.cfg.intermediate_size
        C = cfg.conv_dim
        cins = (1,) + tuple(C[:-1])
        self.g_conv = []
        for i in range(1, len(C) if not self.enc_only else 0):
            k, s, ci, co = cfg.conv_kernel[i], cfg.conv_stride[i], cins[i], C[i]
            cbias = st.mp(f"feature_extractor.conv_layers.{i}.conv.bias") if cfg.conv_bias else self.zero_bias
            ln_train = self.ln_conv and self.cnn_train
            self.g_conv.append(Gemm(self.Bc * self.lens[i], co, k * ci, self.conv[i - 1], self.convw[i],
                                    self.conv_pre[i] if ln_train else self.conv[i],
                                    lda=s * ci, ldb=k * ci, ldc=co, a_seg=(self.lens[i], self.lens[i - 1] * ci),
                                    epilogue=EPI_BIAS if self.ln_conv else EPI_BIAS_GELU, bias=cbias,
                                    aux=self.conv_pre[i] if (self.cnn_train and not self.ln_conv) else None, ldaux=co))
        if self.cnn_train:
            self.g_conv_dw, self.g_conv_dx = [None], [None]
            for i in range(1, len(C)):
                k, sd, ci, co = cfg.conv_kernel[i], cfg.conv_stride[i], cins[i], C[i]
                Mi = self.Bc * self.lens[i]
                gout = self.dn if i == len(C) - 1 else self.dconv[i]
                self.g_conv_dw.append(Gemm(co, k * ci, Mi, gout, self.conv[i - 1], self.dwp, lda=co, ldb=sd * ci,
                                           ldc=k * ci, transA=True, transB=True,
                                           b_seg=(self.lens[i], self.lens[i - 1] * ci),
                                           split_k=_splitk(_tiles(co), _tiles(k * ci), Mi), accumulate=True))
                self.g_conv_dx.append(Gemm(Mi, k * ci, co, gout, self.convw[i], self.col, lda=co, ldb=k * ci,
                                           ldc=k * ci, transB=True))
        mw, mp = st.mw, st.mp
        self.g_proj = None if self.enc_only else Gemm(
            self.M0, H, C[-1], self.ln_feat, mw("feature_projection.projection.weight"), self.h0,
            lda=C[-1], ldb=C[-1], ldc=H, epilogue=EPI_BIAS, bias=mp("feature_projection.projection.bias"))
        G, K, Cg, Tp = cfg.num_conv_pos_embedding_groups, cfg.num_conv_pos_embeddings, self.Cg, self.Tp
        self.g_pos = Gemm(M, Cg, K * Cg, self.xg, self.posw_f, self.pos, lda=Cg, ldb=K * Cg, ldc=H,
                          a_seg=(T, G * Tp * Cg), batch=G, batch_inner=G, a_strides=(0, Tp * Cg),
                          b_strides=(0, Cg * K * Cg), c_strides=(0, Cg), epilogue=EPI_BIAS_GELU,
                          bias=mp("encoder.pos_conv_embed.conv.bias"), bias_stride1=Cg,
                          aux=self.pos_pre, ldaux=H, aux_strides=(0, Cg))
        heads, d = cfg.num_attention_heads, cfg.head_dim
        L = cfg.num_hidden_layers
        self.g_layer: List[Dict[str, Gemm]] = []
        for l in range(L):
            lb = self.lb[l if self.train else 0]
            xin = self._x(l)
            pre = f"encoder.layers.{l}."
            gl: Dict[str, Gemm] = {}
            two = st.two_term and H % 64 == 0
            gl["qkv"] = Gemm(M, 3 * H, H, xin, st.qkv(l, "w"), lb.qkv, lda=H, ldb=H, ldc=3 * H, epilogue=EPI_BIAS,
                             bias=st.qkv(l, "p", "bias"), b_lo=st.qkv_lo(l) if two else None, n_ext_from=2 * H)
            if not self.fused:
                qkv = lb.qkv.view(-1)
                sc = (heads * T * self.Tl, T * self.Tl)
                gl["scores"] = Gemm(T, T, d, qkv, qkv[H:], self.S, lda=3 * H, ldb=3 * H, ldc=self.Tl,
                                    batch=B * heads, batch_inner=heads, a_strides=(T * 3 * H, d),
                                    b_strides=(T * 3 * H, d), c_strides=sc, alpha=d ** -0.5)
                gl["ctx"] = Gemm(T, d, T, lb.pd, qkv[2 * H:], lb.ctx, lda=self.Tl, ldb=3 * H, ldc=H, transB=True,
                                 batch=B * heads, batch_inner=heads, a_strides=sc, b_strides=(T * 3 * H, d),
                                 c_strides=(T * H, d))
            gl["out"] = Gemm(M, H, H, lb.ctx, mw(pre + "attention.out_proj.weight"), lb.a, lda=H, ldb=H, ldc=H,
                             epilogue=EPI_BIAS, bias=mp(pre + "attention.out_proj.bias"),
                             b_lo=st.w_lo(W2V_PREFIX + pre + "attention.out_proj.weight") if two else None)
            gl["ffn1"] = Gemm(M, I, H, lb.x1, mw(pre + "feed_forward.intermediate_dense.weight"), lb.h, lda=H, ldb=H,
                              ldc=I, epilogue=EPI_BIAS_GELU_GRAD if lb.hpre is not None else EPI_BIAS_GELU,
                              bias=mp(pre + "feed_forward.intermediate_dense.bias"), aux=lb.hpre, ldaux=I)
            gl["ffn2"] = Gemm(M, H, I, lb.h, mw(pre + "feed_forward.output_dense.weight"), lb.f, lda=I, ldb=I, ldc=H,
                              epilogue=EPI_BIAS, bias=mp(pre + "feed_forward.output_dense.bias"))
            if self.train:
                mg = st.mg
                sk = lambda m, n: _splitk(_tiles(m), _tiles(n), M)
                W2, W1, Wo = (mw(pre + "feed_forward.output_dense.weight"), mw(pre + "feed_forward.intermediate_dense.weight"),
                              mw(pre + "attention.out_proj.weight"))
                Wqkv = st.qkv(l, "w")
                gs = self._gsets[l % len(self._gsets)]
                tb = st.flat_lp_t is None
                if not tb:
                    W2, W1, Wo = (st.wt("wav2vec.model." + pre + "feed_forward.output_dense.weight"),
                                  st.wt("wav2vec.model." + pre + "feed_forward.intermediate_dense.weight"),
                                  st.wt("wav2vec.model." + pre + "attention.out_proj.weight"))
                    Wqkv = st.qkv_t(l)
                if self.grouped:
                    pad = lambda t: t._w2v2_padded
                    gl["wgrad_problems"] = [
                        (pad(gs["Gd"]), pad(lb.h), mg(pre + "feed_forward.output_dense.weight"),
                         mg(pre + "feed_forward.output_dense.bias")),
                        (pad(gs["DH"]), pad(lb.x1), mg(pre + "feed_forward.intermediate_dense.weight"),
                         mg(pre + "feed_forward.intermediate_dense.bias")),
                        (pad(gs["Gd1"]), pad(lb.ctx), mg(pre + "attention.out_proj.weight"),
                         mg(pre + "attention.out_proj.bias")),
                        (pad(gs["DQKV"]), pad(xin), st.qkv(l, "g"), st.qkv(l, "g", "bias"))]
                    gl["wgrad"] = WgradGroup(gl["wgrad_problems"], M, _pad64(M))
                gl["dW2"] = Gemm(H, I, M, gs["Gd"], lb.h, mg(pre + "feed_forward.output_dense.weight"), lda=H, ldb=I,
                                 ldc=I, transA=True, transB=True, split_k=sk(H, I), accumulate=True)
                gl["dh"] = Gemm(M, I, H, gs["Gd"], W2, gs["DH"], lda=H, ldb=I if tb else H, ldc=I, transB=tb,
                                epilogue=EPI_MUL, aux=lb.hpre, ldaux=I)
                gl["dW1"] = Gemm(I, H, M, gs["DH"], lb.x1, mg(pre + "feed_forward.intermediate_dense.weight"), lda=I,
                                 ldb=H, ldc=H, transA=True, transB=True, split_k=sk(I, H), accumulate=True)
                into_g = {} if self.stable else dict(epilogue=EPI_ADD, aux=self.G, ldaux=H)
                gl["dx1"] = Gemm(M, H, I, gs["DH"], W1, self.G, lda=I, ldb=H if tb else I, ldc=H, transB=tb, **into_g)
                gl["dWo"] = Gemm(H, H, M, gs["Gd1"], lb.ctx, mg(pre + "attention.out_proj.weight"), lda=H, ldb=H, ldc=H,
                                 transA=True, transB=True, split_k=sk(H, H), accumulate=True)
                gl["dctx"] = Gemm(M, H, H, gs["Gd1"], Wo, self.DC, lda=H, ldb=H, ldc=H, transB=tb)
                if not self.fused:
                    qkv = lb.qkv.view(-1)
                    dq = gs["DQKV"].view(-1)
                    sc = (heads * T * self.Tl, T * self.Tl)
                    hs = (T * 3 * H, d)
                    gl["dP"] = Gemm(T, T, d, self.DC, qkv[2 * H:], self.S, lda=H, ldb=3 * H, ldc=self.Tl,
                                    batch=B * heads, batch_inner=heads, a_strides=(T * H, d), b_strides=hs, c_strides=sc)
                    gl["dq"] = Gemm(T, d, T, self.dS, qkv[H:], dq, lda=self.Tl, ldb=3 * H, ldc=3 * H, transB=True,
                                    batch=B * heads, batch_inner=heads, a_strides=sc, b_strides=hs, c_strides=hs,
                                    alpha=d ** -0.5)
                    gl["dk"] = Gemm(T, d, T, self.dS, qkv, dq[H:], lda=self.Tl, ldb=3 * H, ldc=3 * H, transA=True,
                                    transB=True, batch=B * heads, batch_inner=heads, a_strides=sc, b_strides=hs,
                                    c_strides=hs, alpha=d ** -0.5)
                    gl["dv"] = Gemm(T, d, T, lb.pd, self.DC, dq[2 * H:], lda=self.Tl, ldb=H, ldc=3 * H, transA=True,
                                    transB=True, batch=B * heads, batch_inner=heads, a_strides=sc,
                                    b_strides=(T * H, d), c_strides=hs)
                gl["dWqkv"] = Gemm(3 * H, H, M, gs["DQKV"], xin, st.qkv(l, "g"), lda=3 * H, ldb=H, ldc=H, transA=True,
                                   transB=True, split_k=sk(3 * H, H), accumulate=True)
                gl["dx"] = Gemm(M, H, 3 * H, gs["DQKV"], Wqkv, self.G, lda=3 * H, ldb=H if tb else 3 * H, ldc=H,
                                transB=tb, **into_g)
            self.g_layer.append(gl)
        if self.grouped and not self.sw.no_wgrad_pairs:
            for l in range(L - 1, 0, -2):
                self.g_wgrad_pair[l] = WgradGroup(self.g_layer[l]["wgrad_problems"] +
                                                  self.g_layer[l - 1]["wgrad_problems"], M, _pad64(M))
        if self.train:
            mg = st.mg
            self.g_pos_dw = Gemm(K * Cg, Cg, M, self.xg, self.P1, self.dwf, lda=Cg, ldb=H, ldc=Cg, transA=True,
                                 transB=True, a_seg=(T, G * Tp * Cg), batch=G, batch_inner=G, a_strides=(0, Tp * Cg),
                                 b_strides=(0, Cg), c_strides=(0, K * Cg * Cg))
            self.g_pos_dx = Gemm(M, Cg, K * Cg, self.dyg, self.posw_b, self.G, lda=Cg, ldb=K * Cg, ldc=H,
                                 a_seg=(T, G * Tp * Cg), batch=G, batch_inner=G, a_strides=(0, Tp * Cg),
                                 b_strides=(0, Cg * K * Cg), c_strides=(0, Cg), epilogue=EPI_ADD, aux=self.G, ldaux=H,
                                 aux_strides=(0, Cg))
            g0 = self.G0 if (self.cls or self.paired) else self.G
            if st.flat_lp_t is not None:
                S, Ls, Cf = self.proj_slices, self.proj_slice_len, C[-1]
                self.proj_parts = torch.zeros(S, H * Cf + H, dtype=torch.float32, device=self.dev)
                g0p, lnp = g0._w2v2_padded, self.ln_feat._w2v2_padded
                assert g0p.shape[0] >= S * Ls and lnp.shape[0] >= S * Ls
                self.g_proj_dw = WgradGroup([(g0p[i * Ls:], lnp[i * Ls:], self.proj_parts[i, :H * Cf].view(H, Cf),
                                              self.proj_parts[i, H * Cf:]) for i in range(S)], Ls, Ls)
            else:
                self.g_proj_dw = Gemm(H, C[-1], self.M0, g0, self.ln_feat, mg("feature_projection.projection.weight"),
                                      lda=H, ldb=C[-1], ldc=C[-1], transA=True, transB=True,
                                      split_k=_splitk(_tiles(H), _tiles(C[-1]), self.M0), accumulate=True)
            tbp = st.flat_lp_t is None
            Wp = (mw("feature_projection.projection.weight") if tbp
                  else st.wt("wav2vec.model.feature_projection.projection.weight"))
            self.g_proj_dn = Gemm(self.M0, C[-1], H, g0, Wp, self.dn, lda=H, ldb=C[-1] if tbp else H, ldc=C[-1],
                                  transB=tbp)

    def _refresh_packs(self) -> None:
        st, cfg = self.store, self.cfg
        if self._cnn_version != st.cnn_version and not self.enc_only:
            for i in range(1, len(cfg.conv_dim)):
                ops.pack_conv_weight(st.mp(f"feature_extractor.conv_layers.{i}.conv.weight"), self.convw[i])
            self._cnn_version = st.cnn_version
        if self._pack_version != st.version:
            ops.weightnorm_pack(st.mp("encoder.pos_conv_embed.conv.parametrizations.weight.original0"),
                                st.mp("encoder.pos_conv_embed.conv.parametrizations.weight.original1"),
                                self.pos_sumsq, self.posw_f, self.posw_b, cfg.hidden_size,
                                cfg.num_conv_pos_embedding_groups, cfg.num_conv_pos_embeddings)
            self._pack_version = st.version

    def _sd(self, site: str, layer: int, step: int) -> int:
        return (self.seed * 1000003 + step) * 4096 + layer * 8 + _SITE[site]

    def _set_lengths(self, lengths) -> None:
        if self.train:
            raise NotImplementedError("lengths: evaluation plans only (there is no backward for variable lengths)")
        if self.paired:
            raise NotImplementedError("lengths: a paired plan takes the two sides' sample counts as pair_lengths=(left, right)")
        if self.pooling in ("random", "none"):
            raise NotImplementedError(f"lengths: pooling {self.pooling!r} has no variable-length form "
                                      "(supported: mean+std, mean, max, first, first+cls, last, middle, quantile, attentive)")
        lens = valid_lengths(self.cfg, lengths, self.B, self.N)
        f0 = [self.cfg.conv_lengths(n)[0] for n in lens]
        te = [self.cfg.num_frames(n) + (1 if self.cls else 0) for n in lens]
        if self._len_dev is None:
            self._len_dev = torch.empty(2, self.B, dtype=torch.int32, device=self.dev)
        self._len_dev.copy_(torch.tensor([f0, te], dtype=torch.int32))
        self._len = self._len_dev
        self.frame_lengths = te

    def _set_pair_lengths(self, pair_lengths) -> None:
        if not self.paired or self.enc_only:
            raise ValueError("pair_lengths: a plan built with paired=True over waveforms (an encoder-only plan takes "
                             "embed_pairs; other plans take lengths=)")
        if self.train:
            raise NotImplementedError("pair_lengths: evaluation plans only (there is no backward for variable lengths)")
        if self.pooling != "first":
            raise NotImplementedError("pair_lengths: the paired model reads token 0 (pooling='first')")
        try:
            left, right = pair_lengths
        except (TypeError, ValueError):
            raise ValueError("pair_lengths: a pair (left, right) of per-pair sample counts") from None
        B, T0 = self.B, self.T0
        lens = valid_lengths(self.cfg, left, B, self.N) + valid_lengths(self.cfg, right, B, self.N)
        if self._len_dev is None:
            self._len_dev = torch.empty(3 * B, dtype=torch.int32, device=self.dev)
        self._len_dev[:2 * B].copy_(torch.tensor([self.cfg.conv_lengths(n)[0] for n in lens], dtype=torch.int32))
        self._len = (self._len_dev[:2 * B], self._len_dev[2 * B:])
        fr = [self.cfg.num_frames(n) for n in lens]
        self._pair_rows = ([b * T0 for b in range(B)], fr[:B], [(B + b) * T0 for b in range(B)], fr[B:])

    def _assemble_pairs(self, feat: torch.Tensor, left_row, left_frames, right_row, right_frames) -> None:
        B, T, H = self.B, self.T, self.cfg.hidden_size
        if self._pair_dev is None:
            self._pair_dev = torch.empty(4, B, dtype=torch.int32, device=self.dev)
        if self.enc_only:
            if self._len_dev is None:
                self._len_dev = torch.empty(B, dtype=torch.int32, device=self.dev)
            self._len = (None, self._len_dev)
        host = ops.pair_assemble(feat, self.hx.view(B, T, H), left_row, left_frames, right_row, right_frames, self.cls_c,
                                 self.sep_c, table=self._pair_dev)
        te = host[1] + host[3] + 3
        self._len[1].copy_(te)
        self.frame_lengths = te.tolist()

    def embed_pairs(self, feat: torch.Tensor, left_row, left_frames, right_row, right_frames) -> torch.Tensor:
        if not self.enc_only:
            raise ValueError("embed_pairs: an encoder-only paired plan (Plan.pair_encoder)")
        assert feat.is_cuda and feat.dtype == self.adt and feat.dim() == 2 and feat.is_contiguous()
        self._refresh_packs()
        self._step, self._skip, self._mask, self._fmask = 0, (), None, None
        self._assemble_pairs(feat, left_row, left_frames, right_row, right_frames)
        self._pool_fwd(self._encode(0))
        return self.emb

    def features(self, wav: torch.Tensor, lengths=None):
        if self.train or self.paired or self.cls:
            raise NotImplementedError("features: non-paired evaluation plans without a CLS token")
        cfg = self.cfg
        if wav.dim() == 3:
            wav = wav[:, 0, :]
        wav = wav.contiguous()
        assert wav.shape == (self.Bc, self.N) and wav.dtype == torch.float32 and wav.is_cuda
        self._len, self.frame_lengths = None, None
        frames = [self.T0] * self.B
        if lengths is not None:
            lens = valid_lengths(cfg, lengths, self.B, self.N)
            if self._len_dev is None:
                self._len_dev = torch.empty(2, self.B, dtype=torch.int32, device=self.dev)
            frames = [cfg.num_frames(n) for n in lens]
            self._len_dev.copy_(torch.tensor([[cfg.conv_lengths(n)[0] for n in lens], frames], dtype=torch.int32))
            self._len = self._len_dev
        self._refresh_packs()
        self._wav = wav
        self._project(wav)
        return self.h0.view(self.B, self.T0, cfg.hidden_size), frames

    def _project(self, wav: torch.Tensor) -> None:
        mp = self.store.mp
        self._cnn_forward(wav)
        ops.layernorm_fwd(self.conv[-1].view(self.M0, -1), None, mp("feature_projection.layer_norm.weight"),
                          mp("feature_projection.layer_norm.bias"), self.ln_feat, self.mean_f, self.rstd_f,
                          self.cfg.layer_norm_eps)
        self.g_proj()

    def forward(self, wav: torch.Tensor, mask: Optional[torch.Tensor] = None, skip_layers: Sequence[int] = (),
                step: int = 0, feature_mask: Optional[torch.Tensor] = None, lengths=None,
                pair_lengths=None) -> torch.Tensor:
        cfg, st, reg = self.cfg, self.store, self.reg
        if self.enc_only:
            raise ValueError("forward: an encoder-only plan has no conv stack (embed_pairs)")
        B, T, M, H = self.B, self.T, self.M, cfg.hidden_size
        if wav.dim() == 3:
            wav = wav[:, 0, :]
        wav = wav.contiguous()
        assert wav.shape == (self.Bc, self.N) and wav.dtype == torch.float32 and wav.is_cuda
        self._len, self.frame_lengths = None, None
        if lengths is not None:
            self._set_lengths(lengths)
        if pair_lengths is not None:
            self._set_pair_lengths(pair_lengths)
        self._refresh_packs()
        self._wav = wav
        tr = self.train
        self._step, self._skip, self._mask, self._fmask = step, tuple(skip_layers), None, None
        mp = st.mp
        self._project(wav)
        if tr and reg.feat_proj_dropout > 0:
            ops.dropout_(self.h0, reg.feat_proj_dropout, self._sd("featproj", 0, step))
        if self.cls:
            ops.prepend_token(self.h0.view(B, self.T0, H), self.hx.view(B, T, H), self.cls_c)
        elif pair_lengths is not None:
            assert mask is None and feature_mask is None
            self._assemble_pairs(self.h0, *self._pair_rows)
        elif self.paired:
            assert mask is None
            T0, hx, h0 = self.T0, self.hx.view(B, T, H), self.h0.view(2, B, self.T0, H)
            hx[:, 0].fill_(self.cls_c)
            hx[:, 1:1 + T0].copy_(h0[0])
            hx[:, 1 + T0].fill_(self.sep_c)
            hx[:, 2 + T0:2 + 2 * T0].copy_(h0[1])
            hx[:, 2 + 2 * T0].fill_(self.sep_c)
        elif mask is not None:
            self._mask = mask.to(torch.uint8).contiguous().view(-1)
            ops.mask_fill(self.h0, self._mask, mp("masked_spec_embed"))
        if feature_mask is not None:
            assert not (self.cls or self.paired)
            self._fmask = feature_mask.to(torch.uint8).contiguous().view(-1)
            ops.mask_feature(self.h0, self._fmask, B, self.T0)
        return self._encode(step)

    def _encode(self, step: int) -> torch.Tensor:
        cfg, mp = self.cfg, self.store.mp
        B, T, H = self.B, self.T, cfg.hidden_size
        G, K = cfg.num_conv_pos_embedding_groups, cfg.num_conv_pos_embeddings
        if self._len is not None:
            ops.posconv_regroup_len(self.hx, self.xg, self._len[1], B, T, H, G, K, K // 2)
        else:
            ops.posconv_regroup(self.hx, self.xg, B, T, H, G, K, K // 2)
        if self.pos_direct:
            ops.posconv_direct(self.xg, self.posw_f, self.pos, self.pos_pre, mp("encoder.pos_conv_embed.conv.bias"), B, T, G,
                               self.Cg, K, H, 0)
        else:
            self.g_pos()
        return self._encoder_forward(step)

    def _attention(self, l: int, lb: LayerBufs, gl, pa: float, step: int) -> None:
        B, T, heads, d = self.B, self.T, self.cfg.num_attention_heads, self.cfg.head_dim
        lens = None if self._len is None else self._len[1]
        if self.fused:
            if lens is not None:
                ops.attention_fwd_len(lb.qkv, lb.ctx, lb.lse, lens, B, T, heads, d, d ** -0.5)
            else:
                ops.attention_fwd(lb.qkv, lb.ctx, lb.lse, B, T, heads, d, d ** -0.5, pa, self._sd("attn", l, step))
            return
        gl["scores"]()
        if lens is not None:
            ops.softmax_fwd_len(self.S, lb.p, lens, B, heads, T, self.Tl)
        else:
            ops.softmax_fwd(self.S, lb.p, lb.pd if pa > 0 else None, B * heads * T, T, self.Tl, pa,
                            self._sd("attn", l, step))
        gl["ctx"]()

    def _ln_params_for_input_of(self, l: int):
        n = f"encoder.layers.{l}.layer_norm" if l < self.cfg.num_hidden_layers else "encoder.layer_norm"
        return _wb(n)

    def _encoder_forward(self, step: int) -> torch.Tensor:
        cfg, mp, eps = self.cfg, self.store.mp, self.cfg.layer_norm_eps
        H, L = cfg.hidden_size, cfg.num_hidden_layers
        ph = self.reg.hidden_dropout if self.train else 0.0
        if self.stable:
            ops.add(self.hx, self.pos, self.pos)
            if ph > 0:
                ops.dropout_(self.pos, ph, self._sd("prologue", 0, step))
            res = self.pos
            w0, b0 = self._ln_params_for_input_of(0)
            ops.layernorm_fwd(res, None, mp(w0), mp(b0), self._x(0), self.mean0, self.rstd0, eps)
            self._res_src = {}
        else:
            ops.layernorm_fwd(self.hx, self.pos, mp("encoder.layer_norm.weight"), mp("encoder.layer_norm.bias"), self._x(0),
                              self.mean0, self.rstd0, eps)
            if ph > 0:
                ops.dropout_(self._x(0), ph, self._sd("prologue", 0, step))
        for l in range(L):
            xin, xout, lb = self._x(l), self._x(l + 1), self.lb[l if self.train else 0]
            pre = f"encoder.layers.{l}."
            if self.stable:
                ln_next = self._ln_params_for_input_of(l + 1)
                if l in self._skip:
                    ops.layernorm_fwd(res, None, mp(ln_next[0]), mp(ln_next[1]), xout, lb.mean2, lb.rstd2, eps)
                    self._res_src[l] = res
                    continue
                self._block_forward(l, step, res, _wb(pre + "final_layer_norm"), lb.a, ln_next, xout)
                res = lb.f
            elif l in self._skip:
                ops.copy_strided(xin, H, xout, H, xin.shape[0], H)
            else:
                self._block_forward(l, step, xin, _wb(pre + "layer_norm"), lb.x1, _wb(pre + "final_layer_norm"), xout)
        self.out = self._x(L).view(self.B, self.T, H)
        return self.out

    def _block_forward(self, l: int, step: int, res1: torch.Tensor, ln1, res2: torch.Tensor, ln2, xout: torch.Tensor) -> None:
        reg, tr, mp, eps = self.reg, self.train, self.store.mp, self.cfg.layer_norm_eps
        lb, gl = self.lb[l if tr else 0], self.g_layer[l]
        ph = reg.hidden_dropout if tr else 0.0
        gl["qkv"]()
        self._attention(l, lb, gl, reg.attention_dropout if tr else 0.0, step)
        gl["out"]()
        ops.layernorm_fwd(res1, lb.a, mp(ln1[0]), mp(ln1[1]), lb.x1, lb.mean1, lb.rstd1, eps, ph,
                          self._sd("post_attn", l, step))
        gl["ffn1"]()
        if tr and reg.activation_dropout > 0:
            ops.dropout_(lb.h, reg.activation_dropout, self._sd("act", l, step))
            ops.dropout_(lb.hpre, reg.activation_dropout, self._sd("act", l, step))
        gl["ffn2"]()
        ops.layernorm_fwd(res2, lb.f, mp(ln2[0]), mp(ln2[1]), xout, lb.mean2, lb.rstd2, eps, ph, self._sd("ffn", l, step))

    def conv_features(self, wav: torch.Tensor) -> torch.Tensor:
        cfg, st = self.cfg, self.store
        if wav.dim() == 3:
            wav = wav[:, 0, :]
        wav = wav.contiguous()
        assert wav.shape == (self.Bc, self.N) and wav.dtype == torch.float32 and wav.is_cuda
        self._refresh_packs()
        self._wav = wav
        self._len = None
        self._cnn_forward(wav)
        return self.conv[-1]

    def _cnn_forward(self, wav: torch.Tensor) -> None:
        cfg, mp = self.cfg, self.store.mp
        fe = "feature_extractor.conv_layers."
        if not self.ln_conv and self._len is not None:
            ops.conv0_groupnorm_gelu_len(wav, mp(fe + "0.conv.weight"), mp(fe + "0.layer_norm.weight"),
                                         mp(fe + "0.layer_norm.bias"), self.conv[0], self.stats0, self._len[0],
                                         cfg.conv_kernel[0], cfg.conv_stride[0])
            for g in self.g_conv:
                g()
            return
        if not self.ln_conv:
            ops.conv0_groupnorm_gelu(wav, mp(fe + "0.conv.weight"), mp(fe + "0.layer_norm.weight"), mp(fe + "0.layer_norm.bias"),
                                     self.conv[0], self.stats0, cfg.conv_kernel[0], cfg.conv_stride[0])
            for g in self.g_conv:
                g()
            return
        ops.conv0_layernorm_gelu(wav, mp(fe + "0.conv.weight"), mp(fe + "0.conv.bias") if cfg.conv_bias else None,
                                 mp(fe + "0.layer_norm.weight"), mp(fe + "0.layer_norm.bias"), self.conv[0],
                                 cfg.conv_kernel[0], cfg.conv_stride[0])
        for i, g in enumerate(self.g_conv, start=1):
            g()
            y = self.conv[i].view(-1, cfg.conv_dim[i])
            z = self.conv_pre[i].view(-1, cfg.conv_dim[i]) if self.cnn_train else y
            ops.layernorm_gelu_fwd(z, mp(fe + f"{i}.layer_norm.weight"), mp(fe + f"{i}.layer_norm.bias"), y, 1e-5)

    def conv_backward(self, dfeat: torch.Tensor) -> None:
        if not self.train or self.store.freeze_cnn:
            raise RuntimeError("conv_backward needs Plan(train=True) over ParamStore(freeze_cnn=False)")
        self.dn.view(-1).copy_(dfeat.to(self.adt).contiguous().view(-1))
        self._backward_cnn()

    def embed(self, wav, mask=None, skip_layers=(), step: int = 0, feature_mask=None, lengths=None,
              pair_lengths=None) -> torch.Tensor:
        out = self.forward(wav, mask, skip_layers, step, feature_mask, lengths=lengths, pair_lengths=pair_lengths)
        if self.pooling == "attentive":
            return self._asp_for(out).forward(None if self._len is None else self._len[1])
        self._pool_fwd(out)
        return self.emb

    def _pool_fwd(self, out: torch.Tensor) -> None:
        B, T, H = out.shape
        if self._len is not None:
            ops.pool_fwd_len(out, self.emb, self._len[1], self.pool_mode)
        elif self.no_pool:
            ops.pool_fwd(out.view(B * T, 1, H), self.emb, POOL_MODES["first"])
        elif self.pooling == "random":
            import random
            self._rand_idx = random.randint(0, T - 1)
            ops.pool_fwd(out, self.emb, ops.POOL_INDEX_BASE + self._rand_idx)
        else:
            ops.pool_fwd(out, self.emb, self.pool_mode)

    def hidden_states(self) -> List[torch.Tensor]:
        assert self.all_x, "build the plan with keep_hidden_states=True"
        return [x.view(self.B, self.T, self.cfg.hidden_size) for x in self.X]

    def ensemble_embeddings(self, wav, num_ensembles: int) -> List[torch.Tensor]:
        assert self.pooling != "attentive", "ensemble pooling shares one stat-pooling layer: use a stateless pool"
        self.forward(wav, None, (), 0)
        hs = self.hidden_states()
        out = []
        for h in hs[len(hs) - num_ensembles:]:
            e = torch.empty_like(self.emb)
            ops.pool_fwd(h, e, self.pool_mode)
            out.append(e)
        return out

    def _asp_for(self, out: torch.Tensor):
        from .asp import AttentivePool
        key = out.data_ptr()
        if key not in self._asp:
            B, T, H = out.shape
            x2 = out.view(B * T, H)
            src = next((x for x in self.X if x.data_ptr() == key), None)
            if src is not None and hasattr(src, "_w2v2_padded"):
                x2._w2v2_padded = src._w2v2_padded
            self._asp[key] = AttentivePool(self.store, x2, self.emb, self.G if self.train else None, B, T, self.train)
        self._asp_cur = self._asp[key]
        return self._asp_cur

    def head_forward_backward(self, label: torch.Tensor):
        if self.no_pool:
            label = torch.repeat_interleave(label, self.T)
        if self.fc is not None:
            self.fc.forward()
        out = self.head.forward_backward(label)
        if self.fc is not None and self.train:
            self.demb.copy_(self.fc.backward(self.head.demb))
        return out

    def speaker_embedding(self, embedding_layer_idx: int = -1) -> torch.Tensor:
        if embedding_layer_idx < 0:
            return self.emb
        nh = len(self.store.hidden_fc)
        if embedding_layer_idx < nh:
            return self.fc.forward(upto=embedding_layer_idx)
        if embedding_layer_idx == nh and self.store.head == "ce":
            if self.fc is not None:
                self.fc.forward()
            h = self.head
            if h.emb_lp is not h.emb:
                ops.cast(h.emb, h.emb_lp)
            h.g_fwd()
            return h.logits[:, :h.C]
        raise ValueError("could not determine the speaker embedding layer")

    def backward(self, demb: Optional[torch.Tensor] = None,
                 on_bucket_ready: Optional[Callable[[str], None]] = None,
                 dhidden: Optional[torch.Tensor] = None) -> None:
        assert self.train, "backward needs a training plan"
        cfg, st, reg = self.cfg, self.store, self.reg
        B, T, M, H = self.B, self.T, self.M, cfg.hidden_size
        mp, mg = st.mp, st.mg
        step = self._step
        notify = on_bucket_ready or (lambda name: None)
        if dhidden is not None:
            self.G.view(B, T, H).copy_(dhidden)
        else:
            if demb is None:
                demb = self.demb
            if self.pooling == "attentive":
                self._asp_cur.backward(demb)
            elif self.no_pool:
                ops.pool_bwd(self.out.view(B * T, 1, H), self.emb, demb, self.G.view(B * T, 1, H), POOL_MODES["first"])
            elif self.pooling == "random":
                ops.pool_bwd(self.out, self.emb, demb, self.G.view(B, T, H), ops.POOL_INDEX_BASE + self._rand_idx)
            else:
                ops.pool_bwd(self.out, self.emb, demb, self.G.view(B, T, H), self.pool_mode)
        notify("head")
        lnfold = None if self.sw.no_ln_fold else self._lnfold
        if self.stable:
            self._backward_encoder_stable(notify)
        for ev in (() if self.stable else
                   encoder_backward_schedule(cfg.num_hidden_layers, self._skip, self.g_wgrad_pair, self.grouped,
                                             1 if self.sw.no_wgrad_pairs else self.wg_group)):
            kind = ev[0]
            if kind == "body":
                self._layer_backward_body(ev[1], lnfold)
            elif kind == "wgrad":
                layers = ev[1]
                self._wgrad_for(tuple(layers))()
            elif kind == "dx":
                self.g_layer[ev[1]]["dx"]()
            elif kind == "fold":
                if lnfold is not None:
                    lnfold.fold()
            else:
                notify(f"layer{ev[1]}")
        ph = reg.hidden_dropout
        if not self.stable:
            if ph > 0:
                ops.dropout_(self.G, ph, self._sd("prologue", 0, step))
            ops.layernorm_bwd(self.G, self.pos, self.mean0, self.rstd0, mp("encoder.layer_norm.weight"), self.G, None,
                              mg("encoder.layer_norm.weight"), mg("encoder.layer_norm.bias"))
        if H % 8 == 0:
            ops.gelu_bwd_colsum(self.G, self.pos_pre, self.P1, mg("encoder.pos_conv_embed.conv.bias"), M, H)
        else:
            ops.gelu_bwd(self.G, self.pos_pre, self.P1)
            ops.colsum(self.P1, mg("encoder.pos_conv_embed.conv.bias"), M, H)
        G_, K = cfg.num_conv_pos_embedding_groups, cfg.num_conv_pos_embeddings
        if ops.is16(self.P1.dtype) and not self.sw.pos_dw_gemm:
            ops.posconv_wgrad(self.P1, self.xg, self.dwf, B, T, H, G_, K)
        else:
            self.g_pos_dw()
        ops.weightnorm_bwd(mp("encoder.pos_conv_embed.conv.parametrizations.weight.original0"),
                           mp("encoder.pos_conv_embed.conv.parametrizations.weight.original1"), self.pos_sumsq,
                           self.dwf, self.pos_dot, mg("encoder.pos_conv_embed.conv.parametrizations.weight.original0"),
                           mg("encoder.pos_conv_embed.conv.parametrizations.weight.original1"), H, G_, K)
        notify("prologue")
        ops.posconv_regroup(self.P1, self.dyg, B, T, H, G_, K, K - 1 - K // 2)
        if self.pos_direct:
            ops.posconv_direct(self.dyg, self.posw_b, self.G, self.G, None, B, T, G_, self.Cg, K, H, 1)
        else:
            self.g_pos_dx()
        if self.cls:
            self.G0.view(B, self.T0, H).copy_(self.G.view(B, T, H)[:, 1:, :])
            g0 = self.G0
        elif self.paired:
            T0, G3, G0 = self.T0, self.G.view(B, T, H), self.G0.view(2, B, self.T0, H)
            G0[0].copy_(G3[:, 1:1 + T0])
            G0[1].copy_(G3[:, 2 + T0:2 + 2 * T0])
            g0 = self.G0
        else:
            g0 = self.G
            if self._fmask is not None:
                ops.mask_feature(g0, self._fmask, B, self.T0)
            if self._mask is not None:
                ops.mask_fill_bwd(g0, self._mask, mg("masked_spec_embed"))
        if reg.feat_proj_dropout > 0:
            ops.dropout_(g0, reg.feat_proj_dropout, self._sd("featproj", 0, step))
        self.g_proj_dw()
        if st.flat_lp_t is None:
            ops.colsum(g0, mg("feature_projection.projection.bias"), self.M0, H)
        else:
            S, Cf = self.proj_slices, cfg.conv_dim[-1]
            ld = H * Cf + H
            ops.colsum(self.proj_parts, mg("feature_projection.projection.weight").view(-1), S, H * Cf, ld)
            ops.colsum(self.proj_parts[:, H * Cf:], mg("feature_projection.projection.bias"), S, H, ld)
        self.g_proj_dn()
        ops.layernorm_bwd(self.dn, self.conv[-1].view(self.M0, -1), self.mean_f, self.rstd_f,
                          mp("feature_projection.layer_norm.weight"), self.dn, None,
                          mg("feature_projection.layer_norm.weight"), mg("feature_projection.layer_norm.bias"))
        notify("projection")
        if not st.freeze_cnn:
            if not st.cnn_runtime_frozen:
                self._backward_cnn()
            notify("cnn")

    def _backward_encoder_stable(self, notify) -> None:
        mp, mg = self.store.mp, self.store.mg
        step, ph, L = self._step, self.reg.hidden_dropout, self.cfg.num_hidden_layers
        G, GR = self.G, self.GR
        GR.zero_()
        for l in reversed(range(L)):
            lb, gs = self.lb[l], self._gsets[l % len(self._gsets)]
            wn, bn = self._ln_params_for_input_of(l + 1)
            if l in self._skip:
                ops.layernorm_bwd(G, self._res_src[l], lb.mean2, lb.rstd2, mp(wn), G, None, mg(wn), mg(bn))
                ops.add(GR, G, GR)
                G.zero_()
                continue
            w2, b2 = _wb(f"encoder.layers.{l}.final_layer_norm")
            ops.layernorm_bwd(G, lb.f, lb.mean2, lb.rstd2, mp(wn), G, None, mg(wn), mg(bn))
            ops.add(GR, G, GR)
            gs["Gd"].copy_(GR)
            if ph > 0:
                ops.dropout_(gs["Gd"], ph, self._sd("ffn", l, step))
            self._ffn_backward(l)
            ops.layernorm_bwd(G, lb.a, lb.mean1, lb.rstd1, mp(w2), G, None, mg(w2), mg(b2))
            ops.add(GR, G, GR)
            gs["Gd1"].copy_(GR)
            if ph > 0:
                ops.dropout_(gs["Gd1"], ph, self._sd("post_attn", l, step))
            self._attention_backward(l)
            if self.grouped:
                self.g_layer[l]["wgrad"]()
            else:
                self._qkv_wgrad_ungrouped(l)
            self.g_layer[l]["dx"]()
        w0, b0 = self._ln_params_for_input_of(0)
        ops.layernorm_bwd(G, self.pos, self.mean0, self.rstd0, mp(w0), G, None, mg(w0), mg(b0))
        ops.add(GR, G, GR)
        if ph > 0:
            ops.dropout_(GR, ph, self._sd("prologue", 0, step))
        G.copy_(GR)
        for l in reversed(range(L)):
            notify(f"layer{l}")

    def _layer_backward_body(self, l: int, lnfold) -> None:
        mp, mg = self.store.mp, self.store.mg
        step, ph = self._step, self.reg.hidden_dropout
        lb, gs = self.lb[l], self._gsets[l % len(self._gsets)]
        w1, b1 = _wb(f"encoder.layers.{l}.layer_norm")
        w2, b2 = _wb(f"encoder.layers.{l}.final_layer_norm")
        ops.layernorm_bwd(self.G, lb.f, lb.mean2, lb.rstd2, mp(w2), self.G, gs["Gd"], mg(w2), mg(b2), ph,
                          self._sd("ffn", l, step), defer_to=lnfold)
        self._ffn_backward(l)
        ops.layernorm_bwd(self.G, lb.a, lb.mean1, lb.rstd1, mp(w1), self.G, gs["Gd1"], mg(w1), mg(b1), ph,
                          self._sd("post_attn", l, step), defer_to=lnfold)
        self._attention_backward(l)
        if not self.grouped:
            self._qkv_wgrad_ungrouped(l)

    def _ffn_backward(self, l: int) -> None:
        mg, M, H, I = self.store.mg, self.M, self.cfg.hidden_size, self.cfg.intermediate_size
        gl, gs = self.g_layer[l], self._gsets[l % len(self._gsets)]
        pre = f"encoder.layers.{l}.feed_forward."
        if not self.grouped:
            gl["dW2"]()
            ops.colsum(gs["Gd"], mg(pre + "output_dense.bias"), M, H)
        gl["dh"]()
        if not self.grouped:
            gl["dW1"]()
            ops.colsum(gs["DH"], mg(pre + "intermediate_dense.bias"), M, I)
        gl["dx1"]()

    def _attention_backward(self, l: int) -> None:
        cfg, B, T = self.cfg, self.B, self.T
        heads, d, pa = cfg.num_attention_heads, cfg.head_dim, self.reg.attention_dropout
        lb, gl, gs = self.lb[l], self.g_layer[l], self._gsets[l % len(self._gsets)]
        if not self.grouped:
            gl["dWo"]()
            ops.colsum(gs["Gd1"], self.store.mg(f"encoder.layers.{l}.attention.out_proj.bias"), self.M, cfg.hidden_size)
        gl["dctx"]()
        if self.fused:
            ops.attention_bwd(lb.qkv, lb.ctx, self.DC, lb.lse, gs["DQKV"], self.delta, B, T, heads, d, d ** -0.5,
                              pa, self._sd("attn", l, self._step))
        else:
            gl["dP"]()
            ops.softmax_bwd(self.S, lb.p, self.dS, B * heads * T, T, self.Tl, pa, self._sd("attn", l, self._step))
            gl["dq"]()
            gl["dk"]()
            gl["dv"]()

    def _qkv_wgrad_ungrouped(self, l: int) -> None:
        self.g_layer[l]["dWqkv"]()
        ops.colsum(self._gsets[l % len(self._gsets)]["DQKV"], self.store.qkv(l, "g", "bias"), self.M, 3 * self.cfg.hidden_size)

    def _backward_cnn(self) -> None:
        cfg, st, B = self.cfg, self.store, self.Bc
        C = cfg.conv_dim
        cins = (1,) + tuple(C[:-1])
        mg = st.mg
        if self.ln_conv:
            self._backward_cnn_layer_norm()
            return
        for i in reversed(range(1, len(C))):
            k, sd, ci, co = cfg.conv_kernel[i], cfg.conv_stride[i], cins[i], C[i]
            gout = self.dn if i == len(C) - 1 else self.dconv[i]
            gv = gout.view(-1, co)
            ops.gelu_bwd(gv, self.conv_pre[i].view(-1, co), gv)
            self.dwp.zero_()
            self.g_conv_dw[i]()
            ops.unpack_conv_grad(self.dwp, mg(f"feature_extractor.conv_layers.{i}.conv.weight"))
            self.g_conv_dx[i]()
            ops.col2im(self.col, self.dconv[i - 1], B, self.lens[i - 1], self.lens[i], ci, k, sd)
        ops.conv0_bwd(self._wav, st.mp("feature_extractor.conv_layers.0.conv.weight"), self.stats0,
                      st.mp("feature_extractor.conv_layers.0.layer_norm.weight"),
                      st.mp("feature_extractor.conv_layers.0.layer_norm.bias"), self.dconv[0], self.sums0,
                      mg("feature_extractor.conv_layers.0.conv.weight"),
                      mg("feature_extractor.conv_layers.0.layer_norm.weight"),
                      mg("feature_extractor.conv_layers.0.layer_norm.bias"), cfg.conv_kernel[0], cfg.conv_stride[0])


    def _backward_cnn_layer_norm(self) -> None:
        cfg, st, B = self.cfg, self.store, self.Bc
        C = cfg.conv_dim
        cins = (1,) + tuple(C[:-1])
        mp, mg = st.mp, st.mg
        fe = "feature_extractor.conv_layers."
        for i in reversed(range(1, len(C))):
            k, sd, ci, co = cfg.conv_kernel[i], cfg.conv_stride[i], cins[i], C[i]
            gout = self.dn if i == len(C) - 1 else self.dconv[i]
            gv = gout.view(-1, co)
            ops.layernorm_gelu_bwd(gv, self.conv_pre[i].view(-1, co), mp(fe + f"{i}.layer_norm.weight"),
                                   mp(fe + f"{i}.layer_norm.bias"), gv, mg(fe + f"{i}.layer_norm.weight"),
                                   mg(fe + f"{i}.layer_norm.bias"), mg(fe + f"{i}.conv.bias") if cfg.conv_bias else None,
                                   self.lng_ws)
            self.dwp.zero_()
            self.g_conv_dw[i]()
            ops.unpack_conv_grad(self.dwp, mg(fe + f"{i}.conv.weight"))
            self.g_conv_dx[i]()
            ops.col2im(self.col, self.dconv[i - 1], B, self.lens[i - 1], self.lens[i], ci, k, sd)
        ops.conv0_layernorm_gelu_bwd(self._wav, mp(fe + "0.conv.weight"), mp(fe + "0.conv.bias") if cfg.conv_bias else None,
                                     mp(fe + "0.layer_norm.weight"), mp(fe + "0.layer_norm.bias"), self.dconv[0],
                                     mg(fe + "0.conv.weight"), mg(fe + "0.conv.bias") if cfg.conv_bias else None,
                                     mg(fe + "0.layer_norm.weight"), mg(fe + "0.layer_norm.bias"), self.c0l_ws,
                                     cfg.conv_kernel[0], cfg.conv_stride[0])
```

### w2v2_speaker_amd/ops.py

```python
from __future__ import annotations

import ctypes as C
from typing import Optional, Tuple

import torch

from . import _lib
from ._lib import (BF16, EPI_ADD, EPI_BIAS, EPI_BIAS_GELU, EPI_BIAS_GELU_GRAD, EPI_GELU_BWD, EPI_MUL, EPI_NONE, EPI_SCALE_RC, F16, F32,
                   GemmDesc)

POOL_MODES = {"mean+std": 0, "mean": 1, "max": 2, "first": 3, "first+cls": 3, "last": 4, "middle": 4, "quantile": 5}
POOL_WIDTH = {0: 2, 5: 5}
POOL_INDEX_BASE = 16


def lib():
    return _lib.load()


def dt(t: torch.Tensor) -> int:
    if t.dtype == torch.bfloat16:
        return BF16
    if t.dtype == torch.float16:
        return F16
# ... 250 lines not shown
    _dev(wav, w, work, gamma, beta, dz, sums, dw, dgamma, dbeta)
    B, N = wav.shape
    Cc = w.shape[0]
    mr = work[work.numel() - B * Cc * 2:]
    _lib.check(lib().w2v2_conv0_bwd(wav.data_ptr(), w.data_ptr(), mr.data_ptr(), gamma.data_ptr(), beta.data_ptr(),
                                    dz.data_ptr(), sums.data_ptr(), dw.data_ptr(), dgamma.data_ptr(), dbeta.data_ptr(),
                                    dt(dz), B, N, Cc, k, stride, stream()), "conv0_bwd")


def col2im(col, dx, B: int, Lin: int, Lout: int, Cin: int, k: int, stride: int) -> None:
    _dev(col, dx)
    _lib.check(lib().w2v2_col2im(col.data_ptr(), dx.data_ptr(), B, Lin, Lout, Cin, k, stride, dt(col), stream()),
               "col2im")


def unpack_conv_grad(gp, g) -> None:
    _dev(gp, g)
    co, ci, k = g.shape
    _lib.check(lib().w2v2_unpack_conv_grad(gp.data_ptr(), g.data_ptr(), co, ci, k, stream()), "unpack_conv_grad")


def pack_conv_weight(w: torch.Tensor, out: torch.Tensor) -> None:
    _dev(w, out)
    co, ci, k = w.shape
    _lib.check(lib().w2v2_pack_conv_weight(w.data_ptr(), out.data_ptr(), dt(out), co, ci, k, stream()), "pack_conv")


def layernorm_fwd(x, r, gamma, beta, y, mean, rstd, eps: float, drop_p: float = 0.0, seed: int = 0) -> None:
    _dev(x, r, gamma, beta, y, mean, rstd)
    H = x.shape[-1]
    M = x.numel() // H
    _lib.check(lib().w2v2_layernorm_fwd(x.data_ptr(), _p(r), gamma.data_ptr(), beta.data_ptr(), y.data_ptr(),
                                        mean.data_ptr(), rstd.data_ptr(), M, H, eps, drop_p, seed, dt(x), stream()),
               "layernorm_fwd")


def layernorm_gelu_fwd(x, gamma, beta, y, eps: float) -> None:
    _dev(x, gamma, beta, y)
    H = x.shape[-1]
    _lib.check(lib().w2v2_layernorm_gelu_fwd(x.data_ptr(), gamma.data_ptr(), beta.data_ptr(), y.data_ptr(), x.numel() // H, H,
                                             eps, dt(x), stream()), "layernorm_gelu_fwd")


def layernorm_gelu_bwd_workspace(M: int, H: int, device) -> torch.Tensor:
    return torch.empty(max(lib().w2v2_layernorm_gelu_bwd_workspace_floats(M, H), 1), dtype=torch.float32, device=device)


def layernorm_gelu_bwd(dy, z, gamma, beta, dz, dgamma, dbeta, dbias, work, eps: float = 1e-5) -> None:
    _dev(dy, z, gamma, beta, dz, dgamma, dbeta, dbias, work)
    H = dy.shape[-1]
    M = dy.numel() // H
    if work.numel() < lib().w2v2_layernorm_gelu_bwd_workspace_floats(M, H):
        raise ValueError("layernorm_gelu_bwd: workspace too small")
    _lib.check(lib().w2v2_layernorm_gelu_bwd(dy.data_ptr(), z.data_ptr(), gamma.data_ptr(), beta.data_ptr(), dz.data_ptr(),
                                             dgamma.data_ptr(), dbeta.data_ptr(), _p(dbias), work.data_ptr(), M, H, eps,
                                             dt(dy), stream()), "layernorm_gelu_bwd")


_LN_WS = {}


def _ln_workspace(H: int, device) -> torch.Tensor:
    key = (H, str(device))
    if key not in _LN_WS:
        _LN_WS[key] = torch.empty(lib().w2v2_layernorm_bwd_workspace_floats(H), dtype=torch.float32, device=device)
    return _LN_WS[key]


def layernorm_bwd(dy, s, mean, rstd, gamma, ds, d_r, dgamma, dbeta, drop_p: float = 0.0, seed: int = 0,
                  defer_to: Optional["LnFoldGroup"] = None) -> None:
    _dev(dy, s, mean, rstd, gamma, ds, d_r, dgamma, dbeta)
    H = dy.shape[-1]
    M = dy.numel() // H
    if defer_to is not None and dgamma is not None:
        ws = defer_to.add(dgamma, dbeta, M, H)
        _lib.check(lib().w2v2_layernorm_bwd(dy.data_ptr(), s.data_ptr(), mean.data_ptr(), rstd.data_ptr(),
                                            gamma.data_ptr(), ds.data_ptr(), _p(d_r), None, None, ws.data_ptr(), M, H,
                                            drop_p, seed, dt(dy), stream()), "layernorm_bwd")
        return
    ws = _ln_workspace(H, dy.device) if dgamma is not None else None
    _lib.check(lib().w2v2_layernorm_bwd(dy.data_ptr(), s.data_ptr(), mean.data_ptr(), rstd.data_ptr(),
                                        gamma.data_ptr(), ds.data_ptr(), _p(d_r), _p(dgamma), _p(dbeta), _p(ws), M, H,
                                        drop_p, seed, dt(dy), stream()), "layernorm_bwd")


class LnFoldGroup:

    def __init__(self, H: int, device, slots: int = 8):
        n = lib().w2v2_layernorm_bwd_workspace_floats(H)
        self._ws = torch.empty(slots, n, dtype=torch.float32, device=device)
        self._arr = (_lib.LnFold * slots)()
        self._n, self._M, self._H, self._keep = 0, 0, H, []

    def add(self, dgamma, dbeta, M: int, H: int) -> torch.Tensor:
        if self._n == len(self._arr):
            self.fold()
        assert H == self._H and (self._n == 0 or M == self._M)
        e = self._arr[self._n]
        e.partial, e.dgamma, e.dbeta = self._ws[self._n].data_ptr(), dgamma.data_ptr(), dbeta.data_ptr()
        self._keep.append((dgamma, dbeta))
        self._M = M
        self._n += 1
        return self._ws[self._n - 1]

    def fold(self) -> None:
        if self._n:
            _lib.check(lib().w2v2_layernorm_bwd_fold(self._arr, self._n, self._M, self._H, stream()),
                       "layernorm_bwd_fold")
        self._n, self._keep = 0, []


def dropout_(x: torch.Tensor, p: float, seed: int) -> None:
    _dev(x)
    _lib.check(lib().w2v2_dropout(x.data_ptr(), x.data_ptr(), x.numel(), p, seed, dt(x), stream()), "dropout")


def gelu_bwd(dy, pre, dx) -> None:
    _dev(dy, pre, dx)
    _lib.check(lib().w2v2_gelu_bwd(dy.data_ptr(), pre.data_ptr(), dx.data_ptr(), dy.numel(), dt(dy), stream()),
               "gelu_bwd")


PARTIAL_ROWS = 256
_PARTIAL_WS = {}


def _partial_workspace(N: int, device, st: int) -> torch.Tensor:
    key = (N, str(device), st)
    if key not in _PARTIAL_WS:
        _PARTIAL_WS[key] = torch.empty(PARTIAL_ROWS * N, dtype=torch.float32, device=device)
    return _PARTIAL_WS[key]


def gelu_bwd_colsum(dy, pre, dx, colsum_out, M: int, N: int) -> None:
    _dev(dy, pre, dx, colsum_out)
    st = stream()
    ws = _partial_workspace(N, dy.device, st)
    _lib.check(lib().w2v2_gelu_bwd_colsum(dy.data_ptr(), pre.data_ptr(), dx.data_ptr(), colsum_out.data_ptr(),
                                          ws.data_ptr(), M, N, dt(dy), st), "gelu_bwd_colsum")


def add(x, a, y) -> None:
    _dev(x, a, y)
    _lib.check(lib().w2v2_add(x.data_ptr(), a.data_ptr(), y.data_ptr(), x.numel(), dt(x), stream()), "add")


def colsum(x: torch.Tensor, out: torch.Tensor, M: int, N: int, ld: Optional[int] = None) -> None:
    _dev(x, out)
    _lib.check(lib().w2v2_colsum(x.data_ptr(), ld if ld is not None else N, out.data_ptr(), M, N, dt(x), stream()),
               "colsum")


def zero_ranges(base: torch.Tensor, table: torch.Tensor, blocks_per_range: int = 8) -> None:
    _dev(base, table)
    assert base.dtype == torch.float32 and table.dtype == torch.int64
    _lib.check(lib().w2v2_zero_ranges(base.data_ptr(), table.data_ptr(), table.shape[0], blocks_per_range, stream()),
               "zero_ranges")


def mean(x: torch.Tensor, out: torch.Tensor) -> None:
    _dev(x, out)
    assert x.dtype == torch.float32 and out.dtype == torch.float32
    _lib.check(lib().w2v2_mean(x.data_ptr(), out.data_ptr(), x.numel(), stream()), "mean")


def cast(x: torch.Tensor, y: torch.Tensor) -> None:
    _dev(x, y)
    _lib.check(lib().w2v2_cast(x.data_ptr(), y.data_ptr(), x.numel(), dt(y), stream()), "cast")


def transpose_many(src, dst, table, n: int, blocks_per_matrix: int = 64) -> None:
    _dev(src, dst, table)
    _lib.check(lib().w2v2_transpose_many(src.data_ptr(), dst.data_ptr(), table.data_ptr(), n, blocks_per_matrix,
                                         dt(src), stream()), "transpose_many")


def mask_fill(h, mask_u8, embed) -> None:
    _dev(h, mask_u8, embed)
    H = h.shape[-1]
    _lib.check(lib().w2v2_mask_fill(h.data_ptr(), mask_u8.data_ptr(), embed.data_ptr(), h.numel() // H, H, dt(h),
                                    stream()), "mask_fill")


def mask_feature(h, mask_u8, B: int, T: int) -> None:
    _dev(h, mask_u8)
    H = h.shape[-1]
    assert mask_u8.dtype == torch.uint8 and mask_u8.numel() == B * H
    _lib.check(lib().w2v2_mask_feature(h.data_ptr(), mask_u8.data_ptr(), B, T, H, dt(h), stream()), "mask_feature")


def mask_fill_bwd(dh, mask_u8, d_embed) -> None:
    _dev(dh, mask_u8, d_embed)
    H = dh.shape[-1]
    st = stream()
    ws = _partial_workspace(H, dh.device, st)
    _lib.check(lib().w2v2_mask_fill_bwd(dh.data_ptr(), mask_u8.data_ptr(), d_embed.data_ptr(), ws.data_ptr(),
                                        dh.numel() // H, H, dt(dh), st), "mask_fill_bwd")


def prepend_token(x, y, c: float) -> None:
    _dev(x, y)
    B, T, H = x.shape
    _lib.check(lib().w2v2_prepend_token(x.data_ptr(), y.data_ptr(), c, B, T, H, dt(x), stream()), "prepend_token")


def pair_tables(left_row, left_frames, right_row, right_frames, rows: int, T: int) -> torch.Tensor:
    as_list = lambda x: x.reshape(-1).tolist() if isinstance(x, torch.Tensor) else list(x)
    cols = [[int(v) for v in as_list(x)] for x in (left_row, left_frames, right_row, right_frames)]
    if len({len(c) for c in cols}) != 1 or not cols[0]:
        raise ValueError("pair_assemble: the four tables need one entry per pair (at least one pair)")
    for b, (lr, ta, rr, tb) in enumerate(zip(*cols)):
        if ta < 1 or tb < 1:
            raise ValueError(f"pair_assemble: pair {b} has an empty side ({ta} + {tb} frames)")
        if ta + tb + 3 > T:
            raise ValueError(f"pair_assemble: pair {b} needs {ta + tb + 3} frames, the sequence has {T}")
        if lr < 0 or rr < 0 or lr + ta > rows or rr + tb > rows:
            raise ValueError(f"pair_assemble: pair {b} reads rows [{lr}, {lr + ta}) and [{rr}, {rr + tb}) of a feature "
                             f"matrix of {rows}")
    return torch.tensor(cols, dtype=torch.int32)


def pair_assemble(feat, y, left_row, left_frames, right_row, right_frames, cls_c: float, sep_c: float,
                  table: Optional[torch.Tensor] = None) -> torch.Tensor:
    _dev(feat, y)
    B, T, H = y.shape
    assert feat.dim() == 2 and feat.shape[1] == H and feat.dtype == y.dtype and feat.is_contiguous() and y.is_contiguous()
    host = pair_tables(left_row, left_frames, right_row, right_frames, feat.shape[0], T)
    if host.shape[1] != B:
        raise ValueError(f"pair_assemble: {host.shape[1]} pairs for a batch of {B}")
    if table is None:
        table = torch.empty(4, B, dtype=torch.int32, device=y.device)
    assert table.shape == (4, B) and table.dtype == torch.int32 and table.is_cuda and table.is_contiguous()
    table.copy_(host)
    _lib.check(lib().w2v2_pair_assemble(feat.data_ptr(), y.data_ptr(), table[0].data_ptr(), table[1].data_ptr(),
                                        table[2].data_ptr(), table[3].data_ptr(), cls_c, sep_c, B, T, H, dt(y), stream()),
               "pair_assemble")
    return host


def posconv_wgrad(dY, xg, dwf, B: int, T: int, H: int, G: int, K: int) -> None:
    _dev(dY, xg, dwf)
    assert is16(dY.dtype) and xg.dtype == dY.dtype and dwf.dtype == torch.float32
    _lib.check(lib().w2v2_posconv_wgrad(dY.data_ptr(), xg.data_ptr(), dwf.data_ptr(), B, T, H, G, K, dt(dY), stream()),
               "posconv_wgrad")


def posconv_direct(xg, w, out, aux, bias, B: int, T: int, G: int, Cg: int, K: int, ldc: int, mode: int) -> None:
    _dev(xg, w, out, aux, bias)
    assert is16(xg.dtype) and w.dtype == xg.dtype and out.dtype == xg.dtype
    _lib.check(lib().w2v2_posconv_direct(xg.data_ptr(), w.data_ptr(), out.data_ptr(), _p(aux), _p(bias), B, T, G, Cg, K,
                                         ldc, mode, dt(xg), stream()), "posconv_direct")
    if Gemm._log is not None:
        Gemm._log.append({"kind": "posconv", "flops": 2.0 * B * T * G * Cg * K * Cg, "alg_flops": 2.0 * B * T * G * Cg * K * Cg,
                          "kernel": "posconv_direct_kernel", "M": B * T, "N": Cg, "K": K * Cg, "mode": mode})


def posconv_regroup(x, xg, B: int, T: int, H: int, G: int, K: int, pad_left: int) -> None:
    _dev(x, xg)
    _lib.check(lib().w2v2_posconv_regroup(x.data_ptr(), xg.data_ptr(), B, T, H, G, K, pad_left, dt(x), stream()),
               "posconv_regroup")


def posconv_regroup_len(x, xg, lens, B: int, T: int, H: int, G: int, K: int, pad_left: int) -> None:
    _dev(x, xg, lens)
    _lib.check(lib().w2v2_posconv_regroup_len(x.data_ptr(), xg.data_ptr(), lens.data_ptr(), B, T, H, G, K, pad_left,
                                              dt(x), stream()), "posconv_regroup_len")


def weightnorm_scratch(H: int, G: int, K: int, device) -> torch.Tensor:
    return torch.empty(int(lib().w2v2_weightnorm_scratch_floats(H, G, K)), dtype=torch.float32, device=device)


def weightnorm_pack(g, v, sumsq, wf, wb, H: int, G: int, K: int) -> None:
    _dev(g, v, sumsq, wf, wb)
    _lib.check(lib().w2v2_weightnorm_pack(g.data_ptr(), v.data_ptr(), sumsq.data_ptr(), wf.data_ptr(),
                                          wb.data_ptr(), H, G, K, dt(wf), stream()), "weightnorm_pack")


def weightnorm_bwd(g, v, sumsq, dwf, dot, dg, dv, H: int, G: int, K: int) -> None:
    _dev(g, v, sumsq, dwf, dot, dg, dv)
    _lib.check(lib().w2v2_weightnorm_bwd(g.data_ptr(), v.data_ptr(), sumsq.data_ptr(), dwf.data_ptr(),
                                         dot.data_ptr(), dg.data_ptr(), dv.data_ptr(), H, G, K, stream()),
               "weightnorm_bwd")


def softmax_fwd(s, p, p_drop, rows: int, T: int, ld: int, drop_p: float, seed: int) -> None:
    _dev(s, p, p_drop)
    _lib.check(lib().w2v2_softmax_fwd(s.data_ptr(), p.data_ptr(), _p(p_drop), rows, T, ld, drop_p, seed, dt(p),
                                      stream()), "softmax_fwd")


def softmax_fwd_len(s, p, lens, B: int, heads: int, T: int, ld: int) -> None:
    _dev(s, p, lens)
    _lib.check(lib().w2v2_softmax_fwd_len(s.data_ptr(), p.data_ptr(), lens.data_ptr(), B, heads, T, ld, dt(p),
                                          stream()), "softmax_fwd_len")


def softmax_bwd(dp_drop, p, ds, rows: int, T: int, ld: int, drop_p: float, seed: int) -> None:
    _dev(dp_drop, p, ds)
    _lib.check(lib().w2v2_softmax_bwd(dp_drop.data_ptr(), p.data_ptr(), ds.data_ptr(), rows, T, ld, drop_p, seed,
                                      dt(p), stream()), "softmax_bwd")


def attention_fwd(qkv, ctx, lse, B: int, T: int, heads: int, d: int, scale: float, drop_p: float, seed: int) -> None:
    _dev(qkv, ctx, lse)
    _lib.check(lib().w2v2_attention_fwd(qkv.data_ptr(), ctx.data_ptr(), lse.data_ptr(), B, T, heads, d, scale,
                                        drop_p, seed, dt(qkv), stream()), "attention_fwd")


def attention_fwd_len(qkv, ctx, lse, lens, B: int, T: int, heads: int, d: int, scale: float) -> None:
    _dev(qkv, ctx, lse, lens)
    _lib.check(lib().w2v2_attention_fwd_len(qkv.data_ptr(), ctx.data_ptr(), lse.data_ptr(), lens.data_ptr(), B, T, heads,
                                            d, scale, dt(qkv), stream()), "attention_fwd_len")


def attention_bwd(qkv, ctx, dctx, lse, dqkv, delta, B: int, T: int, heads: int, d: int, scale: float,
                  drop_p: float, seed: int) -> None:
    _dev(qkv, ctx, dctx, lse, dqkv, delta)
    _lib.check(lib().w2v2_attention_bwd(qkv.data_ptr(), ctx.data_ptr(), dctx.data_ptr(), lse.data_ptr(),
                                        dqkv.data_ptr(), delta.data_ptr(), B, T, heads, d, scale, drop_p, seed,
                                        dt(qkv), stream()), "attention_bwd")


def pool_fwd(x, out, mode: int) -> None:
    _dev(x, out)
    B, T, H = x.shape
    _lib.check(lib().w2v2_pool_fwd(x.data_ptr(), out.data_ptr(), B, T, H, mode, dt(x), stream()), "pool_fwd")


def pool_fwd_len(x, out, lens, mode: int) -> None:
    _dev(x, out, lens)
    B, T, H = x.shape
    _lib.check(lib().w2v2_pool_fwd_len(x.data_ptr(), out.data_ptr(), lens.data_ptr(), B, T, H, mode, dt(x), stream()),
               "pool_fwd_len")


def pool_bwd(x, out, dout, dx, mode: int) -> None:
    _dev(x, out, dout, dx)
    B, T, H = x.shape
    _lib.check(lib().w2v2_pool_bwd(x.data_ptr(), out.data_ptr(), dout.data_ptr(), dx.data_ptr(), B, T, H, mode,
                                   dt(x), stream()), "pool_bwd")


def row_invnorm(x, inv, rows: int, cols: int, ld: Optional[int] = None) -> None:
    _dev(x, inv)
    _lib.check(lib().w2v2_row_invnorm(x.data_ptr(), ld if ld is not None else cols, inv.data_ptr(), rows, cols,
                                      dt(x), stream()), "row_invnorm")


def aam_softmax_fwd_bwd(cos, label, softmax, loss_rows, dcos_w, dcos_x, inv_x, inv_w, rowdot, colprod, B: int,
                        Cn: int, ldc: int, margin: float, scale: float, loss_scale=None, correct_rows=None,
                        easy_margin: bool = False) -> None:
    _dev(cos, label, softmax, loss_rows, dcos_w, dcos_x, inv_x, inv_w, rowdot, colprod, loss_scale, correct_rows)
    dty = dt(dcos_w) if dcos_w is not None else F32
    _lib.check(lib().w2v2_aam_softmax_fwd_bwd(cos.data_ptr(), label.data_ptr(), softmax.data_ptr(),
                                              loss_rows.data_ptr(), _p(dcos_w), _p(dcos_x), _p(inv_x), _p(inv_w),
                                              _p(rowdot), _p(colprod), B, Cn, ldc, margin, scale, _p(loss_scale),
                                              _p(correct_rows), int(easy_margin), dty, stream()),
               "aam_softmax")


def normalize_bwd(g, x, inv, dot, dx, rows: int, cols: int, ldx: Optional[int] = None, add_to: bool = False) -> None:
    _dev(g, x, inv, dot, dx)
    _lib.check(lib().w2v2_normalize_bwd(g.data_ptr(), x.data_ptr(), ldx if ldx is not None else cols, inv.data_ptr(),
                                        dot.data_ptr(), dx.data_ptr(), rows, cols, dt(x), int(add_to), stream()),
               "normalize_bwd")


def aam_dw(dcos_x, emb, colprod, w_master, inv_w, dw, B: int, Cn: int, E: int, ldc: int) -> None:
    _dev(dcos_x, emb, colprod, w_master, inv_w, dw)
    assert emb.dtype == dcos_x.dtype and dw.dtype == torch.float32 and w_master.dtype == torch.float32
    _lib.check(lib().w2v2_aam_dw(dcos_x.data_ptr(), ldc, emb.data_ptr(), colprod.data_ptr(), w_master.data_ptr(),
                                 inv_w.data_ptr(), dw.data_ptr(), B, Cn, E, dt(emb), stream()), "aam_dw")


def adam_step(p, g, m, v, pb, n: int, lr: float, beta1: float, beta2: float, eps: float, step: int,
              grad_scale: float = 1.0, scaler=None, skip_slot: int = 0) -> None:
    _dev(p, g, m, v, pb, scaler)
    bc1 = 1.0 - beta1 ** step
    bc2 = 1.0 - beta2 ** step
    _lib.check(lib().w2v2_adam_step(p.data_ptr(), g.data_ptr(), m.data_ptr(), v.data_ptr(), _p(pb),
                                    dt(pb) if pb is not None else BF16, n, lr, beta1, beta2, eps, bc1, bc2, grad_scale,
                                    _p(scaler), step, skip_slot, stream()), "adam_step")


def optim_step(algo: str, p, g, m, v, pb, n: int, lr: float, beta1: float = 0.9, beta2: float = 0.999, eps: float = 1e-8,
               step: int = 1, grad_scale: float = 1.0, scaler=None, skip_slot: int = 0, weight_decay: float = 0.0,
               momentum: float = 0.0, dampening: float = 0.0, nesterov: bool = False, norm_state=None) -> None:
    if algo not in ("adam", "sgd"):
        raise ValueError(f"optim_step: algo must be 'adam' or 'sgd', got {algo!r}")
    _dev(p, g, m, v, pb, scaler, norm_state)
    adam = algo == "adam"
    bc1 = 1.0 - beta1 ** step if adam else 1.0
    bc2 = 1.0 - beta2 ** step if adam else 1.0
    _lib.check(lib().w2v2_optim_step(_lib.OPTIM_ADAM if adam else _lib.OPTIM_SGD, p.data_ptr(), g.data_ptr(), _p(m), _p(v),
                                     _p(pb), dt(pb) if pb is not None else BF16, n, lr, beta1, beta2, eps, bc1, bc2,
                                     grad_scale, weight_decay, momentum, dampening, int(bool(nesterov)), _p(norm_state),
                                     _p(scaler), step, skip_slot, stream()), "optim_step")


def grad_norm_partials(n: int) -> int:
    return int(lib().w2v2_grad_norm_partials(n))


def grad_norm(g, n: int, norm_state, partials, grad_scale: float = 1.0, scaler=None, max_norm: float = 0.0) -> None:
    _dev(g, norm_state, partials, scaler)
    assert partials.dtype == torch.float64 and norm_state.dtype == torch.float32 and norm_state.numel() >= 2
    _lib.check(lib().w2v2_grad_norm(g.data_ptr(), n, grad_scale, _p(scaler), max_norm, partials.data_ptr(),
                                    partials.numel(), norm_state.data_ptr(), stream()), "grad_norm")


def grad_accumulate(acc, g, n: int, first: bool) -> None:
    _dev(acc, g)
    assert acc.dtype == torch.float32 and g.dtype == torch.float32 and acc.numel() >= n and g.numel() >= n
    _lib.check(lib().w2v2_grad_accumulate(acc.data_ptr(), g.data_ptr(), n, int(bool(first)), stream()), "grad_accumulate")


def weight_residual(p, lo, table) -> None:
    _dev(p, lo, table)
    _lib.check(lib().w2v2_weight_residual(p.data_ptr(), lo.data_ptr(), table.data_ptr(), table.shape[0], dt(lo), stream()),
               "weight_residual")


def grad_scaler_check(g, n: int, state) -> None:
    _dev(g, state)
    _lib.check(lib().w2v2_grad_scaler_check(g.data_ptr(), n, state.data_ptr(), stream()), "grad_scaler_check")


def grad_scaler_update(state, growth: float = 2.0, backoff: float = 0.5, growth_interval: int = 2000,
                       skipped_ranges: int = 0) -> None:
    _dev(state)
    assert skipped_ranges == 0 or state.numel() >= 8
    _lib.check(lib().w2v2_grad_scaler_update(state.data_ptr(), growth, backoff, growth_interval, skipped_ranges, stream()),
               "grad_scaler_update")


def asp_context(x, ctx, B: int, T: int, C: int) -> None:
    _dev(x, ctx)
    _lib.check(lib().w2v2_asp_context(x.data_ptr(), ctx.data_ptr(), B, T, C, dt(x), stream()), "asp_context")


def asp_context_len(x, ctx, lens, B: int, T: int, C: int) -> None:
    _dev(x, ctx, lens)
    _lib.check(lib().w2v2_asp_context_len(x.data_ptr(), ctx.data_ptr(), lens.data_ptr(), B, T, C, dt(x), stream()),
               "asp_context_len")


def asp_context_bias(ctx, w1, b1, cb, B: int, A: int, C: int) -> None:
    _dev(ctx, w1, b1, cb)
    _lib.check(lib().w2v2_asp_context_bias(ctx.data_ptr(), w1.data_ptr(), b1.data_ptr(), cb.data_ptr(), B, A, C,
                                           stream()), "asp_context_bias")


def asp_bn_workspace(M: int, A: int, device) -> torch.Tensor:
    return torch.empty(lib().w2v2_asp_bn_workspace_floats(M, A), dtype=torch.float32, device=device)


def asp_bn_stats(a_pre, work, mean_rstd, running, M: int, A: int, eps: float, momentum: float) -> None:
    _dev(a_pre, work, mean_rstd, running)
    _lib.check(lib().w2v2_asp_bn_stats(a_pre.data_ptr(), work.data_ptr(), mean_rstd.data_ptr(), _p(running), M, A, eps,
                                       momentum, dt(a_pre), stream()), "asp_bn_stats")


def asp_bn_eval_stats(running, mean_rstd, A: int, eps: float) -> None:
    _dev(running, mean_rstd)
    _lib.check(lib().w2v2_asp_bn_eval_stats(running.data_ptr(), mean_rstd.data_ptr(), A, eps, stream()),
               "asp_bn_eval_stats")


def asp_bn_tanh(a_pre, mean_rstd, gamma, beta, h, M: int, A: int) -> None:
    _dev(a_pre, mean_rstd, gamma, beta, h)
    _lib.check(lib().w2v2_asp_bn_tanh(a_pre.data_ptr(), mean_rstd.data_ptr(), gamma.data_ptr(), beta.data_ptr(),
                                      h.data_ptr(), M, A, dt(a_pre), stream()), "asp_bn_tanh")


def asp_bn_bwd(dh, a_pre, mean_rstd, gamma, beta, work, dgamma, dbeta, da, M: int, A: int) -> None:
    _dev(dh, a_pre, mean_rstd, gamma, beta, work, dgamma, dbeta, da)
    _lib.check(lib().w2v2_asp_bn_bwd(dh.data_ptr(), a_pre.data_ptr(), mean_rstd.data_ptr(),
                                     gamma.data_ptr(), beta.data_ptr(), work.data_ptr(), dgamma.data_ptr(), dbeta.data_ptr(),
                                     da.data_ptr(), M, A, dt(dh), stream()), "asp_bn_bwd")


def asp_pool_fwd(x, s, out, stats, B: int, T: int, C: int) -> None:
    _dev(x, s, out, stats)
    _lib.check(lib().w2v2_asp_pool_fwd(x.data_ptr(), s.data_ptr(), out.data_ptr(), stats.data_ptr(), B, T, C, dt(x),
                                       stream()), "asp_pool_fwd")


def asp_pool_fwd_len(x, s, out, stats, lens, B: int, T: int, C: int) -> None:
    _dev(x, s, out, stats, lens)
    _lib.check(lib().w2v2_asp_pool_fwd_len(x.data_ptr(), s.data_ptr(), out.data_ptr(), stats.data_ptr(), lens.data_ptr(),
                                           B, T, C, dt(x), stream()), "asp_pool_fwd_len")


def asp_pool_bwd(x, s, out, stats, dout, ds, dx, B: int, T: int, C: int) -> None:
    _dev(x, s, out, stats, dout, ds, dx)
    _lib.check(lib().w2v2_asp_pool_bwd(x.data_ptr(), s.data_ptr(), out.data_ptr(), stats.data_ptr(), dout.data_ptr(),
                                       ds.data_ptr(), dx.data_ptr(), B, T, C, dt(x), stream()), "asp_pool_bwd")


def asp_context_bwd(x, ctx, da, w1, dw1, dx, scratch, B: int, T: int, C: int, A: int) -> None:
    _dev(x, ctx, da, w1, dw1, dx, scratch)
    _lib.check(lib().w2v2_asp_context_bwd(x.data_ptr(), ctx.data_ptr(), da.data_ptr(), w1.data_ptr(), dw1.data_ptr(),
                                          dx.data_ptr(), scratch.data_ptr(), B, T, C, A, dt(x), stream()),
               "asp_context_bwd")


def bn_workspace(M: int, C: int, device) -> torch.Tensor:
    return torch.empty(lib().w2v2_bn_workspace_floats(M, C), dtype=torch.float32, device=device)


def bn_fwd(a, lda: int, work, mean_rstd, running, gamma, beta, y, ldy: int, M: int, C: int, eps: float,
           momentum: float, relu: bool, train: bool) -> None:
    _dev(a, work, mean_rstd, running, gamma, beta, y)
    _lib.check(lib().w2v2_bn_fwd(a.data_ptr(), lda, _p(work), mean_rstd.data_ptr(), _p(running), gamma.data_ptr(),
                                 beta.data_ptr(), y.data_ptr(), ldy, M, C, eps, momentum, int(relu), int(train), dt(a),
                                 stream()), "bn_fwd")


def bn_colsum_rows(M: int, C: int) -> int:
    return int(lib().w2v2_bn_colsum_rows(M, C))


def bn_bwd(dy, lddy: int, a, lda: int, mean_rstd, gamma, work, dgamma, dbeta, da, ldda: int, M: int, C: int,
           relu: bool, colsum_partial=None, dy2=None, lddy2: int = 0) -> None:
    _dev(dy, a, mean_rstd, gamma, work, dgamma, dbeta, da, colsum_partial, dy2)
    if dy2 is None:
        _lib.check(lib().w2v2_bn_bwd(dy.data_ptr(), lddy, a.data_ptr(), lda, mean_rstd.data_ptr(), gamma.data_ptr(),
                                     work.data_ptr(), dgamma.data_ptr(), dbeta.data_ptr(), da.data_ptr(), ldda, M, C,
                                     int(relu), _p(colsum_partial), dt(a), stream()), "bn_bwd")
    else:
        _lib.check(lib().w2v2_bn_bwd_sum(dy.data_ptr(), lddy, dy2.data_ptr(), lddy2, a.data_ptr(), lda,
                                         mean_rstd.data_ptr(), gamma.data_ptr(), work.data_ptr(), dgamma.data_ptr(),
                                         dbeta.data_ptr(), da.data_ptr(), ldda, M, C, int(relu), _p(colsum_partial),
                                         dt(a), stream()), "bn_bwd_sum")


def im2col_reflect(x, ldx: int, col, B: int, T: int, Cin: int, k: int, dilation: int, x2=None, ldx2: int = 0) -> None:
    _dev(x, col, x2)
    if x2 is None:
        _lib.check(lib().w2v2_im2col_reflect(x.data_ptr(), ldx, col.data_ptr(), B, T, Cin, k, dilation, dt(x), stream()),
                   "im2col_reflect")
    else:
        _lib.check(lib().w2v2_im2col_reflect_sum(x.data_ptr(), ldx, x2.data_ptr(), ldx2, col.data_ptr(), B, T, Cin, k,
                                                 dilation, dt(x), stream()), "im2col_reflect_sum")


def im2col_reflect_len(x, ldx: int, col, lens, B: int, T: int, Cin: int, k: int, dilation: int, x2=None,
                       ldx2: int = 0) -> None:
    _dev(x, col, lens, x2)
    if x2 is None:
        _lib.check(lib().w2v2_im2col_reflect_len(x.data_ptr(), ldx, col.data_ptr(), lens.data_ptr(), B, T, Cin, k,
                                                 dilation, dt(x), stream()), "im2col_reflect_len")
    else:
        _lib.check(lib().w2v2_im2col_reflect_sum_len(x.data_ptr(), ldx, x2.data_ptr(), ldx2, col.data_ptr(),
                                                     lens.data_ptr(), B, T, Cin, k, dilation, dt(x), stream()),
                   "im2col_reflect_sum_len")


def col2im_reflect(dcol, dx, lddx: int, B: int, T: int, Cin: int, k: int, dilation: int, accumulate: bool) -> None:
    _dev(dcol, dx)
    _lib.check(lib().w2v2_col2im_reflect(dcol.data_ptr(), dx.data_ptr(), lddx, B, T, Cin, k, dilation,
                                         int(accumulate), dt(dcol), stream()), "col2im_reflect")


def add_strided(a, lda: int, b, ldb: int, y, ldy: int, M: int, C: int) -> None:
    _dev(a, b, y)
    _lib.check(lib().w2v2_add_strided(a.data_ptr(), lda, _p(b), ldb, y.data_ptr(), ldy, M, C, dt(a), stream()),
               "add_strided")


def copy_strided(a, lda: int, y, ldy: int, M: int, C: int) -> None:
    add_strided(a, lda, None, 0, y, ldy, M, C)


FBANK_HOP, FBANK_WIN, FBANK_TILE_FRAMES = 160, 400, 16


def fbank_partial_max(B: int, T: int, device) -> torch.Tensor:
    return torch.empty(B, -(-T // FBANK_TILE_FRAMES), dtype=torch.float32, device=device)


def _fbank_f32(*ts) -> None:
    for t in ts:
        if t.dtype != torch.float32 or not t.is_contiguous():
            raise ValueError("fbank: wav, window, fbank, db and partial_max are contiguous f32 tensors")


def fbank_db(wav, lens, window, fbank, db, partial_max) -> None:
    _dev(wav, lens, window, fbank, db, partial_max)
    _fbank_f32(wav, window, fbank, db, partial_max)
    B, N = wav.shape
    T, n_mels = 1 + N // FBANK_HOP, fbank.shape[1]
    if (window.numel() != FBANK_WIN or fbank.shape[0] != FBANK_WIN // 2 + 1 or tuple(db.shape) != (B, T, n_mels)
            or partial_max.numel() < B * -(-T // FBANK_TILE_FRAMES)
            or (lens is not None and (lens.dtype != torch.int32 or lens.numel() != B))):
        raise ValueError(f"fbank_db: shapes wav {tuple(wav.shape)}, window {tuple(window.shape)}, fbank "
                         f"{tuple(fbank.shape)}, db {tuple(db.shape)}, partial_max {tuple(partial_max.shape)}")
    _lib.check(lib().w2v2_fbank_db(wav.data_ptr(), _p(lens), window.data_ptr(), fbank.data_ptr(), db.data_ptr(),
                                   partial_max.data_ptr(), B, N, T, n_mels, stream()), "fbank_db")


def fbank_normalize(db, partial_max, lens, out, ldo: int) -> None:
    _dev(db, partial_max, lens, out)
    _fbank_f32(db, partial_max)
    B, T, n_mels = db.shape
    if (out.dtype not in (torch.float32, torch.bfloat16) or ldo < n_mels or out.stride(-1) != 1
            or partial_max.numel() < B * -(-T // FBANK_TILE_FRAMES)
            or out.untyped_storage().nbytes() // out.element_size() - out.storage_offset() < (B * T - 1) * ldo + n_mels
            or (lens is not None and (lens.dtype != torch.int32 or lens.numel() != B))):
        raise ValueError(f"fbank_normalize: db {tuple(db.shape)}, out {tuple(out.shape)} {out.dtype} with row stride {ldo}")
    _lib.check(lib().w2v2_fbank_normalize(db.data_ptr(), partial_max.data_ptr(), _p(lens), out.data_ptr(), ldo, dt(out),
                                          B, T, n_mels, stream()), "fbank_normalize")


def se_scale(x, g, y, B: int, T: int, C: int) -> None:
    _dev(x, g, y)
    _lib.check(lib().w2v2_se_scale(x.data_ptr(), g.data_ptr(), y.data_ptr(), B, T, C, dt(x), stream()), "se_scale")


def se_bwd_gate(dout, x, dg, B: int, T: int, C: int) -> None:
    _dev(dout, x, dg)
    _lib.check(lib().w2v2_se_bwd_gate(dout.data_ptr(), x.data_ptr(), dg.data_ptr(), B, T, C, dt(x), stream()),
               "se_bwd_gate")
# ... 56 lines not shown
```

Before: 6313 utterances/sec.

## Store attention dropout keep-mask as bitmask in forward, reuse in backward

```diff
diff --git a/include/w2v2_hip.h b/include/w2v2_hip.h
--- a/include/w2v2_hip.h
+++ b/include/w2v2_hip.h
@@ -173,6 +173,12 @@
 int w2v2_attention_bwd(const void* qkv, const void* ctx, const void* dctx, const float* lse,
                        void* dqkv, float* delta , int B, int T, int heads,
                        int d, float scale, float drop_p, uint64_t seed, int dtype, void* stream);
+int64_t w2v2_attention_keep_words(int B, int T, int heads);
+int w2v2_attention_fwd_keep(const void* qkv, void* ctx, float* lse, uint64_t* keep , int B, int T,
+                            int heads, int d, float scale, float drop_p, uint64_t seed, int dtype, void* stream);
+int w2v2_attention_bwd_keep(const void* qkv, const void* ctx, const void* dctx, const float* lse,
+                            const uint64_t* keep , void* dqkv, float* delta, int B, int T,
+                            int heads, int d, float scale, float drop_p, uint64_t seed, int dtype, void* stream);
 int w2v2_attention_fwd_len(const void* qkv, void* ctx, float* lse, const int* lens, int B, int T, int heads, int d,
                            float scale, int dtype, void* stream);
 
diff --git a/w2v2_speaker_amd/_lib.py b/w2v2_speaker_amd/_lib.py
--- a/w2v2_speaker_amd/_lib.py
+++ b/w2v2_speaker_amd/_lib.py
@@ -102,6 +102,11 @@
     "w2v2_softmax_fwd_len": (c_i32, [c_vp, c_vp, c_vp, c_i32, c_i32, c_i32, c_i64, c_i32, c_vp]),
     "w2v2_attention_fwd": (c_i32, [c_vp, c_vp, c_vp, c_i32, c_i32, c_i32, c_i32, c_f32, c_f32, c_u64,
                                    c_i32, c_vp]),
+    "w2v2_attention_keep_words": (c_i64, [c_i32, c_i32, c_i32]),
+    "w2v2_attention_fwd_keep": (c_i32, [c_vp, c_vp, c_vp, c_vp, c_i32, c_i32, c_i32, c_i32, c_f32, c_f32, c_u64,
+                                        c_i32, c_vp]),
+    "w2v2_attention_bwd_keep": (c_i32, [c_vp, c_vp, c_vp, c_vp, c_vp, c_vp, c_vp, c_i32, c_i32, c_i32, c_i32, c_f32,
+                                        c_f32, c_u64, c_i32, c_vp]),
     "w2v2_attention_fwd_len": (c_i32, [c_vp, c_vp, c_vp, c_vp, c_i32, c_i32, c_i32, c_i32, c_f32, c_i32, c_vp]),
     "w2v2_attention_bwd": (c_i32, [c_vp, c_vp, c_vp, c_vp, c_vp, c_vp, c_i32, c_i32, c_i32, c_i32, c_f32,
                                    c_f32, c_u64, c_i32, c_vp]),
diff --git a/w2v2_speaker_amd/csrc/attention.hip b/w2v2_speaker_amd/csrc/attention.hip
--- a/w2v2_speaker_amd/csrc/attention.hip
+++ b/w2v2_speaker_amd/csrc/attention.hip
@@ -21,14 +21,21 @@
   return x;
 }
 template <typename IDX>
+__device__ __forceinline__ void attn_keep4_keys(uint32_t k, uint32_t thr, IDX row0, int key0_rel, bool (&kp)[4]) {
+  const IDX pi = row0 + (IDX)(uint32_t)(key0_rel >> 1);
+  const uint32_t h0 = rng_pair_i(k, pi), h1 = rng_pair_i(k, (IDX)(pi + 1));
+  kp[0] = (h0 & 0xffffu) >= thr;
+  kp[1] = (h0 >> 16) >= thr;
+  kp[2] = (h1 & 0xffffu) >= thr;
+  kp[3] = (h1 >> 16) >= thr;
+}
+template <typename IDX>
 __device__ __forceinline__ void attn_drop4_keys(uint32_t k, uint32_t thr, IDX row0, int key0_rel, float inv_keep,
                                                 float (&ms)[4]) {
-  const IDX pi = row0 + (IDX)(uint32_t)(key0_rel >> 1);
-  const uint32_t h0 = rng_pair_i(k, pi), h1 = rng_pair_i(k, (IDX)(pi + 1));
-  ms[0] = (h0 & 0xffffu) >= thr ? inv_keep : 0.f;
-  ms[1] = (h0 >> 16) >= thr ? inv_keep : 0.f;
-  ms[2] = (h1 & 0xffffu) >= thr ? inv_keep : 0.f;
-  ms[3] = (h1 >> 16) >= thr ? inv_keep : 0.f;
+  bool kp[4];
+  attn_keep4_keys(k, thr, row0, key0_rel, kp);
+#pragma unroll
+  for (int j = 0; j < 4; ++j) ms[j] = kp[j] ? inv_keep : 0.f;
 }
 template <typename IDX>
 __device__ __forceinline__ void attn_drop4_rows(uint32_t k, uint32_t thr, IDX col0, uint32_t Tp2, int q0, int odd,
@@ -44,6 +51,28 @@
   ms[2] = ((r2 >> sh) & 0xffffu) >= thr ? inv_keep : 0.f;
   ms[3] = ((r3 >> sh) & 0xffffu) >= thr ? inv_keep : 0.f;
 }
+
+struct AttnKeep {};
+template <typename IDX> struct attn_idx_of { typedef IDX type; };
+template <> struct attn_idx_of<AttnKeep> { typedef uint32_t type; };
+struct KeepFrag { uint64_t w[4]; };
+__device__ __forceinline__ KeepFrag attn_keep_frag(const uint64_t* __restrict__ kbh, int NB, int qblk, int kblk) {
+  const uint64_t* p = kbh + ((int64_t)min(qblk, NB - 1) * NB + min(kblk, NB - 1)) * 4;
+  KeepFrag f;
+#pragma unroll
+  for (int j = 0; j < 4; ++j) f.w[j] = p[j];
+  return f;
+}
+__device__ __forceinline__ void attn_keep4_words(const KeepFrag& f, float inv_keep, float (&ms)[4]) {
+#pragma unroll
+  for (int j = 0; j < 4; ++j) ms[j] = __builtin_amdgcn_inverse_ballot_w64(f.w[j]) ? inv_keep : 0.f;
+}
+__device__ __forceinline__ void attn_keep4_bits(uint32_t half, int sh, float inv_keep, float (&ms)[4]) {
+  const uint32_t x = half >> sh, ik = __float_as_uint(inv_keep);
+#pragma unroll
+  for (int j = 0; j < 4; ++j) ms[j] = __uint_as_float((0u - ((x >> j) & 1u)) & ik);
+}
+
 __device__ __forceinline__ int aswz(int row) { return ((row ^ (row >> 1)) & 3) | (row & 4); }
 
 __device__ __forceinline__ frag8_t as_frag(uint4 v) {
@@ -197,7 +226,7 @@
 __global__ __launch_bounds__(64 * NW, 4) void attn_fwd_tiled_kernel(const bf16_t* __restrict__ qkv, bf16_t* __restrict__ ctx,
                                                              float* __restrict__ lse, int Tn, int heads_s, float scale,
                                                              float dp, float inv_keep, uint64_t seed,
-                                                             LensArg<LEN> lens) {
+                                                             LensArg<LEN> lens, uint64_t* __restrict__ keep) {
   static_assert(KT * 8 == 2 * 64 * NW, "a tile is staged as two 16-byte chunks per thread");
   constexpr int NT = 64 * NW, RW = 16 * NW, AT_TILE = KT;
   __shared__ __attribute__((aligned(16))) bf16_t Ks[2][AT_TILE * 64];
@@ -239,6 +268,9 @@
 #pragma unroll
   for (int df = 0; df < 4; ++df) o[df] = f32x4{0.f, 0.f, 0.f, 0.f};
   const bool active = row_tile * RW + wave * 16 < Lv;
+  const int NB = (Tn + 15) >> 4;
+  uint64_t* keep_q = nullptr;
+  if (!LEN && keep) keep_q = keep + (bh * NB + (row_tile * NW + __builtin_amdgcn_readfirstlane(wave))) * NB * 4;
 #pragma unroll 1
   for (int t = 0; t < ntile; ++t) {
     const int cur = t & 1;
@@ -271,11 +303,19 @@
         const float alpha = __builtin_amdgcn_exp2f(m - mn);
         m = mn;
         float psum = 0.f;
+        uint64_t kwd[AT_TILE / 16][4];
 #pragma unroll
         for (int fj = 0; fj < AT_TILE / 16; ++fj) {
           if (FULL || fj < nfj) {
             float ms[4];
-            if constexpr (DROP) attn_drop4_keys(rkey, thr, row0, t * AT_TILE + fj * 16, inv_keep, ms);
+            if constexpr (DROP) {
+              bool kp[4];
+              attn_keep4_keys(rkey, thr, row0, t * AT_TILE + fj * 16, kp);
+#pragma unroll
+              for (int j = 0; j < 4; ++j) ms[j] = kp[j] ? inv_keep : 0.f;
+#pragma unroll
+              for (int j = 0; j < 4; ++j) kwd[fj][j] = __builtin_amdgcn_ballot_w64(kp[j]);
+            }
 #pragma unroll
             for (int j = 0; j < 4; ++j) {
               const float p = __builtin_amdgcn_exp2f(s[fj][j] - mn);
@@ -296,6 +336,19 @@
             const frag8_t pf = pack_frag<TE>(s[2 * kb], s[2 * kb + 1]);
 #pragma unroll
             for (int df = 0; df < 4; ++df) o[df] = mfma16<TE>(lds_frag_tr(Vs[cur], troff, df, kb), pf, o[df]);
+          }
+        }
+        if constexpr (DROP) {
+          if (keep_q && lane == 0) {
+#pragma unroll
+            for (int fj = 0; fj < AT_TILE / 16; ++fj) {
+              if (FULL || fj < nfj) {
+                uint4* dst = reinterpret_cast<uint4*>(keep_q + (t * (AT_TILE / 16) + fj) * 4);
+                const uint64_t* w = kwd[fj];
+                dst[0] = make_uint4((uint32_t)w[0], (uint32_t)(w[0] >> 32), (uint32_t)w[1], (uint32_t)(w[1] >> 32));
+                dst[1] = make_uint4((uint32_t)w[2], (uint32_t)(w[2] >> 32), (uint32_t)w[3], (uint32_t)(w[3] >> 32));
+              }
+            }
           }
         }
       };
@@ -332,9 +385,12 @@
                                                                 const float* __restrict__ lse,
                                                                 bf16_t* __restrict__ dqkv, float* __restrict__ delta,
                                                                 int Tn, int heads_s, float scale, float dp,
-                                                                float inv_keep, uint64_t seed) {
+                                                                float inv_keep, uint64_t seed,
+                                                                const uint64_t* __restrict__ keep) {
   static_assert(KT * 8 == 2 * 64 * NW, "a tile is staged as two 16-byte chunks per thread");
-  constexpr int NT = 64 * NW, RW = 16 * NW, AT_TILE = KT;
+  constexpr int NT = 64 * NW, RW = 16 * NW, AT_TILE = KT, NF = KT / 16;
+  constexpr bool KEEP = std::is_same<IDX, AttnKeep>::value;
+  typedef typename attn_idx_of<IDX>::type HIDX;
   __shared__ __attribute__((aligned(16))) bf16_t Ks[2][AT_TILE * 64];
   __shared__ __attribute__((aligned(16))) bf16_t Vs[2][AT_TILE * 64];
   const AttnBlock blk = attn_block((Tn + RW - 1) / RW, heads_s);
@@ -359,7 +415,7 @@
   if (g == 0 && q < Tn) delta[bh * Tn + q] = dl;
   const uint32_t thr = drop_thr16(dp);
   const uint32_t rkey = rng_key(seed);
-  const IDX row0 = (IDX)(attn_row_pair0(bh, q, Tn) + (uint64_t)(g * 2));
+  const HIDX row0 = (HIDX)(attn_row_pair0(bh, q, Tn) + (uint64_t)(g * 2));
   const float l2 = q < Tn ? lse[bh * Tn + q] * 1.4426950408889634f : 0.f;
   const float scale2 = scale * 1.4426950408889634f;
   const TrOff troff = tr_offsets(lane);
@@ -374,12 +430,24 @@
 #pragma unroll
   for (int df = 0; df < 4; ++df) o[df] = f32x4{0.f, 0.f, 0.f, 0.f};
   const bool active = row_tile * RW + wave * 16 < Tn;
+  const int NB = (Tn + 15) >> 4;
+  const int qblk = row_tile * NW + __builtin_amdgcn_readfirstlane(wave);
+  const uint64_t* kbh = KEEP ? keep + bh * NB * NB * 4 : nullptr;
+  KeepFrag kw[NF], kn[NF];
+  if constexpr (KEEP) {
+#pragma unroll
+    for (int fj = 0; fj < NF; ++fj) kw[fj] = attn_keep_frag(kbh, NB, qblk, fj);
+  }
 #pragma unroll 1
   for (int t = 0; t < ntile; ++t) {
     const int cur = t & 1;
     if (t + 1 < ntile) {
       tile_load<NT>(rk, qb + H, gs, (t + 1) * AT_TILE, Tn);
       tile_load<NT>(rv, qb + 2 * H, gs, (t + 1) * AT_TILE, Tn);
+      if constexpr (KEEP) {
+#pragma unroll
+        for (int fj = 0; fj < NF; ++fj) kn[fj] = attn_keep_frag(kbh, NB, qblk, (t + 1) * NF + fj);
+      }
     }
     const int nfj = min(AT_TILE / 16, (Tn - t * AT_TILE + 15) >> 4);
     if (active)
@@ -399,7 +467,8 @@
           }
           const int key0 = t * AT_TILE + fj * 16 + g * 4;
           float ms[4] = {1.f, 1.f, 1.f, 1.f};
-          if (dp > 0.f) attn_drop4_keys(rkey, thr, row0, t * AT_TILE + fj * 16, inv_keep, ms);
+          if constexpr (KEEP) attn_keep4_words(kw[fj], inv_keep, ms);
+          else if (dp > 0.f) attn_drop4_keys(rkey, thr, row0, t * AT_TILE + fj * 16, inv_keep, ms);
           if ((t + 1) * AT_TILE > Tn) {
 #pragma unroll
             for (int j = 0; j < 4; ++j) {
@@ -426,6 +495,10 @@
     if (t + 1 < ntile) {
       tile_store<NT>(rk, Ks[cur ^ 1]);
       tile_store<NT>(rv, Vs[cur ^ 1]);
+      if constexpr (KEEP) {
+#pragma unroll
+        for (int fj = 0; fj < NF; ++fj) kw[fj] = kn[fj];
+      }
     }
     __syncthreads();
   }
@@ -438,9 +511,12 @@
                                                                 const float* __restrict__ lse,
                                                                 const float* __restrict__ delta,
                                                                 bf16_t* __restrict__ dqkv, int Tn, int heads_s,
-                                                                float scale, float dp, float inv_keep, uint64_t seed) {
+                                                                float scale, float dp, float inv_keep, uint64_t seed,
+                                                                const uint64_t* __restrict__ keep) {
   static_assert(KT * 8 == 2 * 64 * NW, "a tile is staged as two 16-byte chunks per thread");
-  constexpr int NT = 64 * NW, RW = 16 * NW, AT_TILE = KT;
+  constexpr int NT = 64 * NW, RW = 16 * NW, AT_TILE = KT, NF = KT / 16;
+  constexpr bool KEEP = std::is_same<IDX, AttnKeep>::value;
+  typedef typename attn_idx_of<IDX>::type HIDX;
   __shared__ __attribute__((aligned(16))) bf16_t Qs[2][AT_TILE * 64];
   __shared__ __attribute__((aligned(16))) bf16_t Os[2][AT_TILE * 64];
   __shared__ __attribute__((aligned(16))) float lse_s[2][AT_TILE];
@@ -462,15 +538,29 @@
   const int ntile = (Tn + AT_TILE - 1) / AT_TILE;
   TileRegs rq, ro;
   float rl = 0.f, rd = 0.f;
+  const int NB = (Tn + 15) >> 4;
+  const int ksh = ((key >> 2) & 1) * 16 + g * 4;
+  const uint32_t* khalf = nullptr;
+  if constexpr (KEEP)
+    khalf = reinterpret_cast<const uint32_t*>(keep + (bh * NB * NB + min(key >> 4, NB - 1)) * 4 + (key & 3)) + ((key >> 3) & 1);
+  uint32_t kwn[NF] = {}, kwc[NF] = {};
   auto row_load = [&](int t) {
     if (threadIdx.x < AT_TILE) {
       const int r = t * AT_TILE + threadIdx.x;
       rl = r < Tn ? lse[bh * Tn + r] * 1.4426950408889634f : (DMA ? INFINITY : 0.f);
       rd = r < Tn ? delta[bh * Tn + r] : 0.f;
     }
+    if constexpr (KEEP) {
+#pragma unroll
+      for (int fq = 0; fq < NF; ++fq) kwn[fq] = khalf[(int64_t)min(t * NF + fq, NB - 1) * NB * 8];
+    }
   };
   auto row_store = [&](int buf) {
     if (threadIdx.x < AT_TILE) { lse_s[buf][threadIdx.x] = rl; del_s[buf][threadIdx.x] = rd; }
+    if constexpr (KEEP) {
+#pragma unroll
+      for (int fq = 0; fq < NF; ++fq) kwc[fq] = kwn[fq];
+    }
   };
   if constexpr (DMA) {
     tile_dma<NW, KT>(qb, gs, 0, Tn, Qs[0], wave, lane);
@@ -492,7 +582,7 @@
   for (int df = 0; df < 4; ++df) { dv[df] = f32x4{0.f, 0.f, 0.f, 0.f}; dk[df] = f32x4{0.f, 0.f, 0.f, 0.f}; }
   const bool active = row_tile * RW + wave * 16 < Tn;
   const uint32_t rkey = rng_key(seed), thr = drop_thr16(dp);
-  const IDX col0 = (IDX)(attn_drop_idx(bh, 0, key, Tn) >> 1);
+  const HIDX col0 = (HIDX)(attn_drop_idx(bh, 0, key, Tn) >> 1);
   const uint32_t Tp2 = (uint32_t)(((Tn + 1) & ~1) >> 1);
   const float scale2 = scale * 1.4426950408889634f;
 #pragma unroll 1
@@ -529,7 +619,8 @@
           const float la[4] = {l4.x, l4.y, l4.z, l4.w}, da[4] = {d4.x, d4.y, d4.z, d4.w};
           const int q0 = t * AT_TILE + fq * 16 + g * 4;
           float ms[4] = {1.f, 1.f, 1.f, 1.f};
-          if (dp > 0.f) attn_drop4_rows(rkey, thr, col0, Tp2, q0, key & 1, inv_keep, ms);
+          if constexpr (KEEP) attn_keep4_bits(kwc[fq], ksh, inv_keep, ms);
+          else if (dp > 0.f) attn_drop4_rows(rkey, thr, col0, Tp2, q0, key & 1, inv_keep, ms);
 #pragma unroll
           for (int j = 0; j < 4; ++j) {
             const float p = key < Tn ? __builtin_amdgcn_exp2f(fmaf(sa[j], scale2, -la[j])) : 0.f;
@@ -582,6 +673,14 @@
   return g == 32 || (g != 64 && T <= ATTN_SMALL_GEOM_MAX_T && ((T + 31) & ~31) < ((T + 63) & ~63));
 }
 
+static bool attn_use_keep(const void* keep, float drop_p) {
+  return keep != nullptr && drop_p > 0.f && getenv("W2V2_ATTN_NO_KEEP") == nullptr;
+}
+static int64_t attn_keep_words(int B, int T, int heads) {
+  const int64_t nb = (T + 15) / 16;
+  return (int64_t)B * heads * nb * nb * 4;
+}
+
 static bool attn_idx32(int B, int T, int heads) {
   if (getenv("W2V2_ATTN_IDX64")) return false;
   return (uint64_t)B * heads * T * (uint64_t)(((T + 1) & ~1) >> 1) < (1ull << 32);
@@ -589,35 +688,44 @@
 
 template <typename TE, int NW, int KT, typename IDX>
 static int attention_fwd_g(const char* name, const void* qkv, void* ctx, float* lse, const int* lens, int B, int T,
-                           int heads, float scale, float drop_p, uint64_t seed, void* stream) {
+                           int heads, float scale, float drop_p, uint64_t seed, uint64_t* keep, void* stream) {
   const float ik = 1.0f / (1.0f - drop_p);
   hipStream_t st = as_stream(stream);
   dim3 grid((unsigned)(cdiv(T, 16 * NW) * heads * B));
   W2V2_DISPATCH_LEN(lens,
     hipLaunchKernelGGL((attn_fwd_tiled_kernel<TE, NW, KT, IDX, LEN>), grid, dim3(64 * NW), 0, st, (const bf16_t*)qkv,
-                       (bf16_t*)ctx, lse, T, g_attn_no_remap ? -heads : heads, scale, drop_p, ik, seed, lens));
+                       (bf16_t*)ctx, lse, T, g_attn_no_remap ? -heads : heads, scale, drop_p, ik, seed, lens, keep));
   W2V2_CHECK_LAUNCH(name);
   return 0;
 }
 template <typename TE>
 static int attention_fwd_t(const char* name, const void* qkv, void* ctx, float* lse, const int* lens, int B, int T,
-                           int heads, float scale, float drop_p, uint64_t seed, void* stream) {
+                           int heads, float scale, float drop_p, uint64_t seed, uint64_t* keep, void* stream) {
   const bool i32 = attn_idx32(B, T, heads);
+  if (!attn_use_keep(keep, drop_p)) keep = nullptr;
   if (attn_small_geom(T))
-    return i32 ? attention_fwd_g<TE, 2, 32, uint32_t>(name, qkv, ctx, lse, lens, B, T, heads, scale, drop_p, seed, stream)
-               : attention_fwd_g<TE, 2, 32, uint64_t>(name, qkv, ctx, lse, lens, B, T, heads, scale, drop_p, seed, stream);
-  return i32 ? attention_fwd_g<TE, 4, 64, uint32_t>(name, qkv, ctx, lse, lens, B, T, heads, scale, drop_p, seed, stream)
-             : attention_fwd_g<TE, 4, 64, uint64_t>(name, qkv, ctx, lse, lens, B, T, heads, scale, drop_p, seed, stream);
-}
-
-extern "C" int w2v2_attention_fwd(const void* qkv, void* ctx, float* lse, int B, int T, int heads, int d, float scale,
-                                  float drop_p, uint64_t seed, int dtype, void* stream) {
+    return i32 ? attention_fwd_g<TE, 2, 32, uint32_t>(name, qkv, ctx, lse, lens, B, T, heads, scale, drop_p, seed, keep, stream)
+               : attention_fwd_g<TE, 2, 32, uint64_t>(name, qkv, ctx, lse, lens, B, T, heads, scale, drop_p, seed, keep, stream);
+  return i32 ? attention_fwd_g<TE, 4, 64, uint32_t>(name, qkv, ctx, lse, lens, B, T, heads, scale, drop_p, seed, keep, stream)
+             : attention_fwd_g<TE, 4, 64, uint64_t>(name, qkv, ctx, lse, lens, B, T, heads, scale, drop_p, seed, keep, stream);
+}
+
+extern "C" int64_t w2v2_attention_keep_words(int B, int T, int heads) {
+  return B > 0 && T > 0 && heads > 0 ? attn_keep_words(B, T, heads) : 0;
+}
+
+extern "C" int w2v2_attention_fwd_keep(const void* qkv, void* ctx, float* lse, uint64_t* keep, int B, int T, int heads,
+                                       int d, float scale, float drop_p, uint64_t seed, int dtype, void* stream) {
   if (attn_check("attention_fwd", B, T, heads, d, dtype, drop_p)) return -1;
   W2V2_REQUIRE(qkv && ctx && lse, "attention_fwd: null pointer");
   W2V2_DISPATCH_16(dtype, "attention_fwd",
                    return attention_fwd_t<AT>("attention_fwd", qkv, ctx, lse, nullptr, B, T, heads, scale, drop_p, seed,
-                                              stream););
+                                              keep, stream););
   return 0;
+}
+extern "C" int w2v2_attention_fwd(const void* qkv, void* ctx, float* lse, int B, int T, int heads, int d, float scale,
+                                  float drop_p, uint64_t seed, int dtype, void* stream) {
+  return w2v2_attention_fwd_keep(qkv, ctx, lse, nullptr, B, T, heads, d, scale, drop_p, seed, dtype, stream);
 }
 
 extern "C" int w2v2_attention_fwd_len(const void* qkv, void* ctx, float* lse, const int* lens, int B, int T, int heads,
@@ -626,49 +734,61 @@
   W2V2_REQUIRE(qkv && ctx && lse && lens, "attention_fwd_len: null pointer");
   W2V2_DISPATCH_16(dtype, "attention_fwd_len",
                    return attention_fwd_t<AT>("attention_fwd_len", qkv, ctx, lse, lens, B, T, heads, scale, 0.f, 0,
-                                              stream););
+                                              nullptr, stream););
   return 0;
 }
 
 template <typename TE, int NW, int KT, typename IDX>
 static int attention_bwd_g(const void* qkv, const void* ctx, const void* dctx, const float* lse, void* dqkv,
                            float* delta, int B, int T, int heads, float scale, float drop_p, uint64_t seed,
-                           void* stream) {
+                           const uint64_t* keep, void* stream) {
   const float ik = 1.0f / (1.0f - drop_p);
   hipStream_t st = as_stream(stream);
   dim3 grid((unsigned)(cdiv(T, 16 * NW) * heads * B));
   hipLaunchKernelGGL((attn_bwd_dq_tiled_kernel<TE, NW, KT, IDX>), grid, dim3(64 * NW), 0, st, (const bf16_t*)qkv, (const bf16_t*)ctx,
                      (const bf16_t*)dctx, lse, (bf16_t*)dqkv, delta, T, g_attn_no_remap ? -heads : heads, scale, drop_p, ik,
-                     seed);
+                     seed, keep);
   if (NW == 2 && getenv("W2V2_ATTN_KV_NO_DMA") == nullptr)
     hipLaunchKernelGGL((attn_bwd_kv_tiled_kernel<TE, NW, KT, IDX, NW == 2>), grid, dim3(64 * NW), 0, st, (const bf16_t*)qkv,
                        (const bf16_t*)dctx, lse, (const float*)delta, (bf16_t*)dqkv, T, g_attn_no_remap ? -heads : heads, scale,
-                       drop_p, ik, seed);
+                       drop_p, ik, seed, keep);
   else
     hipLaunchKernelGGL((attn_bwd_kv_tiled_kernel<TE, NW, KT, IDX, false>), grid, dim3(64 * NW), 0, st, (const bf16_t*)qkv,
                        (const bf16_t*)dctx, lse, (const float*)delta, (bf16_t*)dqkv, T, g_attn_no_remap ? -heads : heads, scale,
-                       drop_p, ik, seed);
+                       drop_p, ik, seed, keep);
   W2V2_CHECK_LAUNCH("attention_bwd");
   return 0;
 }
 template <typename TE>
 static int attention_bwd_t(const void* qkv, const void* ctx, const void* dctx, const float* lse, void* dqkv,
                            float* delta, int B, int T, int heads, float scale, float drop_p, uint64_t seed,
-                           void* stream) {
+                           const uint64_t* keep, void* stream) {
+  if (attn_use_keep(keep, drop_p))
+    return attn_small_geom(T)
+      ? attention_bwd_g<TE, 2, 32, AttnKeep>(qkv, ctx, dctx, lse, dqkv, delta, B, T, heads, scale, drop_p, seed, keep, stream)
+      : attention_bwd_g<TE, 4, 64, AttnKeep>(qkv, ctx, dctx, lse, dqkv, delta, B, T, heads, scale, drop_p, seed, keep, stream);
+  keep = nullptr;
   const bool i32 = attn_idx32(B, T, heads);
   if (attn_small_geom(T))
-    return i32 ? attention_bwd_g<TE, 2, 32, uint32_t>(qkv, ctx, dctx, lse, dqkv, delta, B, T, heads, scale, drop_p, seed, stream)
-               : attention_bwd_g<TE, 2, 32, uint64_t>(qkv, ctx, dctx, lse, dqkv, delta, B, T, heads, scale, drop_p, seed, stream);
-  return i32 ? attention_bwd_g<TE, 4, 64, uint32_t>(qkv, ctx, dctx, lse, dqkv, delta, B, T, heads, scale, drop_p, seed, stream)
-             : attention_bwd_g<TE, 4, 64, uint64_t>(qkv, ctx, dctx, lse, dqkv, delta, B, T, heads, scale, drop_p, seed, stream);
-}
-
+    return i32 ? attention_bwd_g<TE, 2, 32, uint32_t>(qkv, ctx, dctx, lse, dqkv, delta, B, T, heads, scale, drop_p, seed, keep, stream)
+               : attention_bwd_g<TE, 2, 32, uint64_t>(qkv, ctx, dctx, lse, dqkv, delta, B, T, heads, scale, drop_p, seed, keep, stream);
+  return i32 ? attention_bwd_g<TE, 4, 64, uint32_t>(qkv, ctx, dctx, lse, dqkv, delta, B, T, heads, scale, drop_p, seed, keep, stream)
+             : attention_bwd_g<TE, 4, 64, uint64_t>(qkv, ctx, dctx, lse, dqkv, delta, B, T, heads, scale, drop_p, seed, keep, stream);
+}
+
+extern "C" int w2v2_attention_bwd_keep(const void* qkv, const void* ctx, const void* dctx, const float* lse,
+                                       const uint64_t* keep, void* dqkv, float* delta, int B, int T, int heads, int d,
+                                       float scale, float drop_p, uint64_t seed, int dtype, void* stream) {
+  if (attn_check("attention_bwd", B, T, heads, d, dtype, drop_p)) return -1;
+  W2V2_REQUIRE(qkv && ctx && dctx && lse && dqkv && delta, "attention_bwd: null pointer");
+  W2V2_DISPATCH_16(dtype, "attention_bwd",
+                   return attention_bwd_t<AT>(qkv, ctx, dctx, lse, dqkv, delta, B, T, heads, scale, drop_p, seed, keep,
+                                              stream););
+  return 0;
+}
 extern "C" int w2v2_attention_bwd(const void* qkv, const void* ctx, const void* dctx, const float* lse, void* dqkv,
                                   float* delta, int B, int T, int heads, int d, float scale, float drop_p,
                                   uint64_t seed, int dtype, void* stream) {
-  if (attn_check("attention_bwd", B, T, heads, d, dtype, drop_p)) return -1;
-  W2V2_REQUIRE(qkv && ctx && dctx && lse && dqkv && delta, "attention_bwd: null pointer");
-  W2V2_DISPATCH_16(dtype, "attention_bwd",
-                   return attention_bwd_t<AT>(qkv, ctx, dctx, lse, dqkv, delta, B, T, heads, scale, drop_p, seed, stream););
-  return 0;
-}
+  return w2v2_attention_bwd_keep(qkv, ctx, dctx, lse, nullptr, dqkv, delta, B, T, heads, d, scale, drop_p, seed, dtype,
+                                 stream);
+}
diff --git a/w2v2_speaker_amd/engine.py b/w2v2_speaker_amd/engine.py
--- a/w2v2_speaker_amd/engine.py
+++ b/w2v2_speaker_amd/engine.py
@@ -134,6 +134,7 @@
     mean2: torch.Tensor
     rstd2: torch.Tensor
     lse: Optional[torch.Tensor] = None
+    keep: Optional[torch.Tensor] = None
     p: Optional[torch.Tensor] = None
     pd: Optional[torch.Tensor] = None
 
@@ -307,6 +308,8 @@
                            mean2=self._e(M, dtype=f32), rstd2=self._e(M, dtype=f32))
             if self.fused:
                 lb.lse = self._e(B * heads * T, dtype=f32)
+                if self.train and self.reg.attention_dropout > 0:
+                    lb.keep = self._e(ops.attention_keep_words(B, T, heads), dtype=torch.int64)
             else:
                 lb.p = torch.zeros(B * heads * T, self.Tl, dtype=self.adt, device=self.dev)
                 lb.pd = (torch.zeros(B * heads * T, self.Tl, dtype=self.adt, device=self.dev)
@@ -685,7 +688,8 @@
             if lens is not None:
                 ops.attention_fwd_len(lb.qkv, lb.ctx, lb.lse, lens, B, T, heads, d, d ** -0.5)
             else:
-                ops.attention_fwd(lb.qkv, lb.ctx, lb.lse, B, T, heads, d, d ** -0.5, pa, self._sd("attn", l, step))
+                ops.attention_fwd(lb.qkv, lb.ctx, lb.lse, B, T, heads, d, d ** -0.5, pa, self._sd("attn", l, step),
+                                  keep=lb.keep)
             return
         gl["scores"]()
         if lens is not None:
@@ -1048,7 +1052,7 @@
         gl["dctx"]()
         if self.fused:
             ops.attention_bwd(lb.qkv, lb.ctx, self.DC, lb.lse, gs["DQKV"], self.delta, B, T, heads, d, d ** -0.5,
-                              pa, self._sd("attn", l, self._step))
+                              pa, self._sd("attn", l, self._step), keep=lb.keep)
         else:
             gl["dP"]()
             ops.softmax_bwd(self.S, lb.p, self.dS, B * heads * T, T, self.Tl, pa, self._sd("attn", l, self._step))
diff --git a/w2v2_speaker_amd/ops.py b/w2v2_speaker_amd/ops.py
--- a/w2v2_speaker_amd/ops.py
+++ b/w2v2_speaker_amd/ops.py
@@ -576,10 +576,24 @@
                                       dt(p), stream()), "softmax_bwd")
 
 
-def attention_fwd(qkv, ctx, lse, B: int, T: int, heads: int, d: int, scale: float, drop_p: float, seed: int) -> None:
+def attention_keep_words(B: int, T: int, heads: int) -> int:
+    return int(lib().w2v2_attention_keep_words(B, T, heads))
+
+
+def _keep_ptr(keep, B: int, T: int, heads: int):
+    if keep is None:
+        return None
+    _dev(keep)
+    if keep.dtype != torch.int64 or not keep.is_contiguous() or keep.numel() < attention_keep_words(B, T, heads):
+        raise RuntimeError("attention keep buffer: need a contiguous int64 tensor of attention_keep_words(B, T, heads) words")
+    return keep.data_ptr()
+
+
+def attention_fwd(qkv, ctx, lse, B: int, T: int, heads: int, d: int, scale: float, drop_p: float, seed: int, *,
+                  keep=None) -> None:
     _dev(qkv, ctx, lse)
-    _lib.check(lib().w2v2_attention_fwd(qkv.data_ptr(), ctx.data_ptr(), lse.data_ptr(), B, T, heads, d, scale,
-                                        drop_p, seed, dt(qkv), stream()), "attention_fwd")
+    _lib.check(lib().w2v2_attention_fwd_keep(qkv.data_ptr(), ctx.data_ptr(), lse.data_ptr(), _keep_ptr(keep, B, T, heads),
+                                             B, T, heads, d, scale, drop_p, seed, dt(qkv), stream()), "attention_fwd")
 
 
 def attention_fwd_len(qkv, ctx, lse, lens, B: int, T: int, heads: int, d: int, scale: float) -> None:
@@ -589,11 +603,11 @@
 
 
 def attention_bwd(qkv, ctx, dctx, lse, dqkv, delta, B: int, T: int, heads: int, d: int, scale: float,
-                  drop_p: float, seed: int) -> None:
+                  drop_p: float, seed: int, *, keep=None) -> None:
     _dev(qkv, ctx, dctx, lse, dqkv, delta)
-    _lib.check(lib().w2v2_attention_bwd(qkv.data_ptr(), ctx.data_ptr(), dctx.data_ptr(), lse.data_ptr(),
-                                        dqkv.data_ptr(), delta.data_ptr(), B, T, heads, d, scale, drop_p, seed,
-                                        dt(qkv), stream()), "attention_bwd")
+    _lib.check(lib().w2v2_attention_bwd_keep(qkv.data_ptr(), ctx.data_ptr(), dctx.data_ptr(), lse.data_ptr(),
+                                             _keep_ptr(keep, B, T, heads), dqkv.data_ptr(), delta.data_ptr(), B, T, heads,
+                                             d, scale, drop_p, seed, dt(qkv), stream()), "attention_bwd")
 
 
 def pool_fwd(x, out, mode: int) -> None:
```

Result: no change. 6313 utterances/sec (-0.0%).
